# AaltoML/t-SVGP

Measured on AMD Instinct MI355X. Metric: natgrad E-steps/sec, higher is better.
Workload: dtype f64; 1 GPU; gaussian_regression_N1e6_M1024_D8_P1 (north_star target; the metric's N, M); N=1000000, M=1024, D=8, P=1, likelihood=gaussian, rows_per_gpu=1000000, parallelism=N-sharded x1, 1 all-reduce/step, projection=auto

## Files before the change

include/tsvgp_hip.h:

```cpp
#ifndef TSVGP_HIP_H
#define TSVGP_HIP_H

#include <stdint.h>

#ifdef __cplusplus
extern "C" {
#endif

#define TSVGP_OK 0
#define TSVGP_EINVAL 1
#define TSVGP_ELAUNCH 2

#define TSVGP_TILE 128
#define TSVGP_MAX_BATCH 32

#define TSVGP_LIK_NONE 0
#define TSVGP_LIK_GAUSSIAN 1
#define TSVGP_LIK_BERNOULLI 2
#define TSVGP_LIK_HETERO 3
#define TSVGP_LIK_SOFTMAX 4
#define TSVGP_LIK_STUDENT_T 5
#define TSVGP_LIK_POISSON 6
#define TSVGP_LIK_MULTICLASS 7
#define TSVGP_LIK_GAMMA 8
// ... 67 lines not shown
                      int32_t *nonpos_partial, int64_t N, int64_t Np, int Mp, int P, int mode, void *stream);

int tsvgp_lik_map_f64(const double *mean, const double *var, const double *Y, int lik, double lik_param, double *g0, double *g1,
                      double *ve_partial, int32_t *nonpos_partial, int64_t N, int64_t Np, int P, void *stream);
int tsvgp_lik_map_f32(const float *mean, const float *var, const float *Y, int lik, double lik_param, float *g0, float *g1,
                      double *ve_partial, int32_t *nonpos_partial, int64_t N, int64_t Np, int P, void *stream);

int tsvgp_lik_map_hetero_f64(const double *mean, const double *var, const double *Y, int flags, double *g0, double *g1,
                             double *ve_partial, int32_t *nonpos_partial, int64_t N, int64_t Np, void *stream);
int tsvgp_lik_map_hetero_f32(const float *mean, const float *var, const float *Y, int flags, float *g0, float *g1,
                             double *ve_partial, int32_t *nonpos_partial, int64_t N, int64_t Np, void *stream);

int tsvgp_lik_map_robustmax_f64(const double *mean, const double *var, const double *Y, int flags, int C, double epsilon,
                                double *g0, double *g1, double *ve_partial, int32_t *nonpos_partial, int64_t N, int64_t Np,
                                void *stream);
int tsvgp_lik_map_robustmax_f32(const float *mean, const float *var, const float *Y, int flags, int C, double epsilon, float *g0,
                                float *g1, double *ve_partial, int32_t *nonpos_partial, int64_t N, int64_t Np, void *stream);

int tsvgp_lik_map_scalar_f64(const double *mean, const double *var, const double *Y, int64_t in_stride, int lik, double param0,
                             double param1, double *g0, double *g1, int64_t out_stride, double *ve_partial, double *dparam_partial,
                             int32_t *nonpos_partial, int64_t N, int64_t Np, void *stream);
int tsvgp_lik_map_scalar_f32(const float *mean, const float *var, const float *Y, int64_t in_stride, int lik, double param0,
                             double param1, float *g0, float *g1, int64_t out_stride, double *ve_partial, double *dparam_partial,
                             int32_t *nonpos_partial, int64_t N, int64_t Np, void *stream);

#define TSVGP_ORDINAL_MAX_EDGES 255
int tsvgp_lik_map_ordinal_f64(const double *mean, const double *var, const double *Y, int64_t in_stride, int flags,
                              const double *edges, int n_edges, double sigma, double *g0, double *g1, int64_t out_stride,
                              double *ve_partial, double *dparam_partial, int32_t *nonpos_partial, int64_t N, int64_t Np,
                              void *stream);
int tsvgp_lik_map_ordinal_f32(const float *mean, const float *var, const float *Y, int64_t in_stride, int flags,
                              const double *edges, int n_edges, double sigma, float *g0, float *g1, int64_t out_stride,
                              double *ve_partial, double *dparam_partial, int32_t *nonpos_partial, int64_t N, int64_t Np,
                              void *stream);

int tsvgp_lmc_mix_f64(const double *mean_g, const double *var_g, const double *W, double *Fmu, double *Fvar,
                      int32_t *nonpos_partial, int64_t N, int64_t Np, int L, int P, void *stream);
int tsvgp_lmc_mix_f32(const float *mean_g, const float *var_g, const double *W, float *Fmu, float *Fvar, int32_t *nonpos_partial,
                      int64_t N, int64_t Np, int L, int P, void *stream);
int tsvgp_lmc_unmix_f64(const double *g0_f, const double *g1_f, const double *W, int flags, double *g0_g, double *g1_g,
                        const double *mean_g, const double *var_g, double *dW_partial, int64_t N, int64_t Np, int L, int P,
                        void *stream);
int tsvgp_lmc_unmix_f32(const float *g0_f, const float *g1_f, const double *W, int flags, float *g0_g, float *g1_g,
                        const float *mean_g, const float *var_g, double *dW_partial, int64_t N, int64_t Np, int L, int P,
                        void *stream);

int tsvgp_diag_site_step_f64(const double *mean, const double *var, const double *Y, int lik, double lik_param, double lr,
                             double *lambda_1, double *lambda_2, double *ve_partial, int32_t *nonpos_partial, int64_t N, int64_t Np,
                             int P, void *stream);
int tsvgp_diag_site_step_f32(const float *mean, const float *var, const float *Y, int lik, double lik_param, double lr,
                             double *lambda_1, double *lambda_2, float *lambda_1_f32, float *lambda_2_f32, double *ve_partial,
                             int32_t *nonpos_partial, int64_t N, int64_t Np, int P, void *stream);

#define TSVGP_MC_MAX_SAMPLES (1 << 28)
int tsvgp_mc_normals_f64(double *out, int64_t seed, int64_t draw, int64_t row_offset, int64_t S, int64_t N, int C, void *stream);
int tsvgp_mc_normals_f32(float *out, int64_t seed, int64_t draw, int64_t row_offset, int64_t S, int64_t N, int C, void *stream);

int tsvgp_lik_map_softmax_f64(const double *mean, const double *var, const double *Y, int flags, int C, int S,
                              const int64_t *rng_state, int64_t row_offset, const double *epsilon, double *g0, double *g1,
                              double *ve_partial, int32_t *nonpos_partial, int64_t N, int64_t Np, void *stream);
int tsvgp_lik_map_softmax_f32(const float *mean, const float *var, const float *Y, int flags, int C, int S,
                              const int64_t *rng_state, int64_t row_offset, const float *epsilon, float *g0, float *g1,
                              double *ve_partial, int32_t *nonpos_partial, int64_t N, int64_t Np, void *stream);

int tsvgp_moments_batched_f64(const double *A, int64_t strideA, const double *Tm, const double *gamma, const double *Y,
                              const double *kdiag_host, int lik, double lik_param, double *mean, double *var, double *g0,
                              double *g1, double *ve_partial, int32_t *nonpos_partial, int64_t N, int64_t Np, int Mp,
                              int P, int mode, void *stream);
int tsvgp_moments_batched_f32(const float *A, int64_t strideA, const float *Tm, const float *gamma, const float *Y,
                              const double *kdiag_host, int lik, double lik_param, float *mean, float *var, float *g0,
                              float *g1, double *ve_partial, int32_t *nonpos_partial, int64_t N, int64_t Np, int Mp,
                              int P, int mode, void *stream);

int64_t tsvgp_site_accum_work_bytes_f64(int Mp, int P, int nsplit);
int64_t tsvgp_site_accum_work_bytes_f32(int Mp, int P, int nsplit);
int tsvgp_site_accum_f64(const double *B, const double *g0, const double *g1, double *acc2, double *acc1, void *work,
                         int64_t Np, int Mp, int P, int nsplit, void *stream);
int tsvgp_site_accum_f32(const float *B, const float *g0, const float *g1, double *acc2, double *acc1, void *work,
                         int64_t Np, int Mp, int P, int nsplit, void *stream);
int tsvgp_site_accum_batched_f64(const double *B, int64_t strideB, const double *g0, const double *g1, double *acc2,
                                 double *acc1, void *work, int64_t Np, int Mp, int P, int nsplit, void *stream);
int tsvgp_site_accum_batched_f32(const float *B, int64_t strideB, const float *g0, const float *g1, double *acc2,
                                 double *acc1, void *work, int64_t Np, int Mp, int P, int nsplit, void *stream);

#define TSVGP_POTRF_SUBST 1
#define TSVGP_POTRF_DIAG_V1 4
#define TSVGP_POTRF_FUSE 16
int tsvgp_potrf_f64(double *A, int M, int lda, int batch, int64_t stride, int32_t *info, double *work, int flags,
                    void *stream);

#define TSVGP_POTRF_RHS_UPPER 2
int tsvgp_potrf_solve_f64(double *A, int M, int lda, int batch, int64_t stride, int32_t *info, double *work, int rhs_rows,
                          int flags, void *stream);
int tsvgp_flip_transpose_f64(const double *src, int lds, int64_t sstride, double *dst, int ldd, int64_t dstride, int M, int batch,
                             void *stream);

#define TSVGP_VGP_NO_ROWS 1
int tsvgp_vgp_system_f64(int kind, const double *X, const double *inv_ls, double variance, double jitter, const double *lambda_1,
                         const double *lambda_2, double *S, int64_t N, int64_t Np, int D, int64_t lds, int flags, void *stream);
int tsvgp_vgp_rows_f64(const double *C, int64_t ldc, const double *z, const double *Y, double *lambda_1, double *lambda_2,
                       double kdiag, int lik, double lik_param, double beta, double *mean, double *var, double *ve_partial,
                       double *eqt_partial, int32_t *nonpos_partial, int64_t N, int64_t Np, int K, void *stream);

int64_t tsvgp_vgp_kernel_grad_parts(int64_t Np, int D);
int tsvgp_vgp_kernel_grad_f64(int kind, const double *X, const double *inv_ls, double variance, const double *W, int64_t ldw,
                              const double *a, const double *c, int64_t N, int64_t Np, int D, double *part, void *stream);

int tsvgp_potrf_inv_f64(double *A, int M, int lda, int batch, int64_t stride, int32_t *info, double *work, double *X,
                        double *Xt, double *T, int flags, void *stream);

int tsvgp_tri_copy_f64(const double *src, int lds, int64_t sstride, double *dst, int ldd, int64_t dstride, int M, int batch,
                       double scale, int flip, void *stream);
int tsvgp_tri_copy_shift_f64(const double *src, int lds, int64_t sstride, double *dst, int ldd, int64_t dstride, int M, int batch,
                             double scale, double diag_add, int flip, void *stream);

int tsvgp_site_target_f64(const double *G1, const double *LLt, double *target, double *G1s, int M, int P, double c_ll,
                          double c_g, double jitter, const double *rows, double num_data, void *stream);

int tsvgp_site_update_f64(const double *G1, const double *G0, const double *LLt, const double *meanZ, const double *l1_old,
                          double *target, double *l1_new, double *work, int M, int P, double lr, double jitter, const double *rows,
                          double num_data, void *stream);

int tsvgp_site_beta_f64(const double *D, const double *v, const double *l1, double *work, double *beta, int M, int P,
                        void *stream);

int tsvgp_gemv_f64(const double *A, int64_t strideA, const double *v, double *y, int M, int P, void *stream);

int tsvgp_step_status_f64(const int32_t *info_a, int na, const int32_t *info_b, int nb, const double *nonpos, double *flags,
                          void *stream);

int tsvgp_sym_pack_f64(const double *A, int lda, int64_t stride, int M, int P, double *packed, void *stream);
int tsvgp_sym_unpack_f64(const double *packed, double *A, int lda, int64_t stride, int M, int P, void *stream);

int tsvgp_kernel_grad_rows(void);
int tsvgp_kernel_grad_dpad(int D);
int tsvgp_kernel_grad_f64(int kind, const double *X, const double *Z, const double *inv_ls, double variance,
                          const double *U, int64_t ldu, const double *g0, const double *g1, int gstride,
                          const double *beta, int bstride, int64_t N, int M, int D, double *zpart, double *lpart,
                          double *vpart, void *stream);
int tsvgp_kernel_grad_f32(int kind, const float *X, const float *Z, const float *inv_ls, float variance, const float *U,
                          int64_t ldu, const float *g0, const float *g1, int gstride, const float *beta, int bstride,
                          int64_t N, int M, int D, double *zpart, double *lpart, double *vpart, void *stream);

int64_t tsvgp_greedy_select_work_bytes(int64_t N, int M);
int tsvgp_greedy_select_f64(int kind, const double *X, const double *inv_ls, double variance, double floor, double *C, int64_t ldc,
                            double *d, int64_t *indices, double *pivots, int32_t *count, void *work, int64_t N, int M, int D,
                            void *stream);

#define TSVGP_PATHWISE_MAX_S 16
int tsvgp_pathwise_f64(int kind, const double *X, const double *Z, const double *inv_ls, double variance, const double *Omega,
                       const double *W, const double *V, double *out, int64_t N, int M, int L, int D, int S, int64_t ldo,
                       void *stream);

int tsvgp_pathwise_vjp_f64(int kind, const double *X, const double *Z, const double *inv_ls, double variance, const double *Omega,
                           const double *W, const double *V, const double *C, int64_t ldc, double *dX, int64_t N, int M, int L,
                           int D, int S, void *stream);

int tsvgp_moments_vjp_rows(int D);
int tsvgp_moments_vjp_stage_f64(int D);
int tsvgp_moments_vjp_stage_f32(int D);
int tsvgp_moments_vjp_f64(int kind, const double *X, const double *Z, const double *inv_ls, double variance, const double *U,
                          int64_t ldu, const double *cm, const double *cv, int cstride, const double *beta, int bstride, int64_t N,
                          int M, int D, double *dX, int accumulate, void *stream);
int tsvgp_moments_vjp_f32(int kind, const float *X, const float *Z, const float *inv_ls, float variance, const float *U, int64_t ldu,
                          const float *cm, const float *cv, int cstride, const float *beta, int bstride, int64_t N, int M, int D,
                          double *dX, int accumulate, void *stream);
// ... 23 lines not shown
```

t-svgp_amd/_backend.py:

```python
from __future__ import annotations

import ctypes
import os
import subprocess
from ctypes import c_char_p, c_double, c_float, c_int, c_int64, c_void_p

_HERE = os.path.dirname(os.path.abspath(__file__))
_ROOT = os.path.dirname(_HERE)
CSRC = os.path.join(_HERE, "csrc")
LIB_PATH = os.path.join(CSRC, "libtsvgp_hip.so")
HEADER_PATH = os.path.join(_ROOT, "include", "tsvgp_hip.h")
SOURCES = [os.path.join(CSRC, "tsvgp_kernels.hip"), os.path.join(CSRC, "tsvgp_chol.hip"), os.path.join(CSRC, "tsvgp_kmeans.hip")]
HEADERS = [HEADER_PATH, os.path.join(CSRC, "tsvgp_chol.h")]
SOURCE_FLAGS = {"tsvgp_chol.hip": ["-mllvm", "-amdgpu-mfma-vgpr-form=1"]}

TILE = 128
MAX_BATCH = 32
LIK_NONE, LIK_GAUSSIAN, LIK_BERNOULLI = 0, 1, 2
LIK_HETERO = 3
LIK_SOFTMAX = 4
LIK_MULTICLASS = 7
COUPLED_LIKS = (LIK_HETERO, LIK_SOFTMAX, LIK_MULTICLASS)
LIK_STUDENT_T, LIK_POISSON = 5, 6
LIK_GAMMA = 8
# ... 64 lines not shown
    "tsvgp_version": (c_char_p, []),
    "tsvgp_abi_version": (c_int, []),
    "tsvgp_site_accum_slots_f64": (c_int, []),
    "tsvgp_site_accum_slots_f32": (c_int, []),
    "tsvgp_se_fill_f64": (c_int, [c_void_p, c_void_p, c_void_p, c_double, c_void_p, c_int64, c_int, c_int, c_int64, c_void_p]),
    "tsvgp_se_fill_f32": (c_int, [c_void_p, c_void_p, c_void_p, c_float, c_void_p, c_int64, c_int, c_int, c_int64, c_void_p]),
    "tsvgp_kernel_fill_f64": (c_int, [c_int, c_void_p, c_void_p, c_void_p, c_double, c_void_p, c_int64, c_int, c_int, c_int64, c_void_p]),
    "tsvgp_kernel_fill_f32": (c_int, [c_int, c_void_p, c_void_p, c_void_p, c_float, c_void_p, c_int64, c_int, c_int, c_int64, c_void_p]),
    "tsvgp_kernel_fill_batched_f64": (c_int, [c_int, c_void_p, c_void_p, c_void_p, c_void_p, c_void_p, c_int64, c_int64, c_int, c_int,
                                              c_int64, c_int, c_void_p]),
    "tsvgp_kernel_fill_batched_f32": (c_int, [c_int, c_void_p, c_void_p, c_void_p, c_void_p, c_void_p, c_int64, c_int64, c_int, c_int,
                                              c_int64, c_int, c_void_p]),
    "tsvgp_gram_to_kernel_f64": (c_int, [c_int, c_void_p, c_void_p, c_void_p, c_double, c_int64, c_int, c_int64, c_void_p]),
    "tsvgp_gram_to_kernel_f32": (c_int, [c_int, c_void_p, c_void_p, c_void_p, c_float, c_int64, c_int, c_int64, c_void_p]),
    "tsvgp_cov_f64": (c_int, [c_int, c_void_p, c_void_p, c_void_p, c_double, c_double, c_void_p, c_int64, c_int64, c_int, c_int, c_int64,
                              c_int, c_void_p]),
    "tsvgp_cov_f32": (c_int, [c_int, c_void_p, c_void_p, c_void_p, c_float, c_float, c_void_p, c_int64, c_int64, c_int, c_int, c_int64,
                              c_int, c_void_p]),
    "tsvgp_gram_to_gradw_parts": (c_int64, [c_int64, c_int]),
    "tsvgp_gram_to_gradw_f64": (c_int, [c_int, c_void_p, c_void_p, c_void_p, c_double, c_void_p, c_int64, c_void_p, c_void_p, c_int,
                                        c_void_p, c_int, c_int64, c_int, c_int64, c_void_p, c_void_p]),
    "tsvgp_gram_to_gradw_f32": (c_int, [c_int, c_void_p, c_void_p, c_void_p, c_float, c_void_p, c_int64, c_void_p, c_void_p, c_int,
                                        c_void_p, c_int, c_int64, c_int, c_int64, c_void_p, c_void_p]),
    "tsvgp_kernel_grad_rows": (c_int, []),
    "tsvgp_kernel_grad_dpad": (c_int, [c_int]),
    "tsvgp_kernel_grad_f64": (c_int, [c_int, c_void_p, c_void_p, c_void_p, c_double, c_void_p, c_int64, c_void_p, c_void_p, c_int,
                                      c_void_p, c_int, c_int64, c_int, c_int, c_void_p, c_void_p, c_void_p, c_void_p]),
    "tsvgp_kernel_grad_f32": (c_int, [c_int, c_void_p, c_void_p, c_void_p, c_float, c_void_p, c_int64, c_void_p, c_void_p, c_int,
                                      c_void_p, c_int, c_int64, c_int, c_int, c_void_p, c_void_p, c_void_p, c_void_p]),
    "tsvgp_trmm_f64": (c_int, [c_void_p, c_void_p, c_void_p, c_int64, c_int, c_int, c_void_p]),
    "tsvgp_trmm_f32": (c_int, [c_void_p, c_void_p, c_void_p, c_int64, c_int, c_int, c_void_p]),
    "tsvgp_trmm_batched_f64": (c_int, [c_void_p, c_int64, c_void_p, c_int64, c_void_p, c_int64, c_int64, c_int, c_int, c_int, c_void_p]),
    "tsvgp_trmm_batched_f32": (c_int, [c_void_p, c_int64, c_void_p, c_int64, c_void_p, c_int64, c_int64, c_int, c_int, c_int, c_void_p]),
    "tsvgp_moments_batched_f64": (c_int, [c_void_p, c_int64, c_void_p, c_void_p, c_void_p, c_void_p, c_int, c_double, c_void_p, c_void_p,
                                          c_void_p, c_void_p, c_void_p, c_void_p, c_int64, c_int64, c_int, c_int, c_int, c_void_p]),
    "tsvgp_moments_batched_f32": (c_int, [c_void_p, c_int64, c_void_p, c_void_p, c_void_p, c_void_p, c_int, c_double, c_void_p, c_void_p,
                                          c_void_p, c_void_p, c_void_p, c_void_p, c_int64, c_int64, c_int, c_int, c_int, c_void_p]),
    "tsvgp_site_accum_batched_f64": (c_int, [c_void_p, c_int64, c_void_p, c_void_p, c_void_p, c_void_p, c_void_p, c_int64, c_int, c_int, c_int, c_void_p]),
    "tsvgp_site_accum_batched_f32": (c_int, [c_void_p, c_int64, c_void_p, c_void_p, c_void_p, c_void_p, c_void_p, c_int64, c_int, c_int, c_int, c_void_p]),
    "tsvgp_moments_f64": (c_int, [c_void_p, c_void_p, c_void_p, c_void_p, c_double, c_int, c_double, c_void_p, c_void_p,
                                  c_void_p, c_void_p, c_void_p, c_void_p, c_int64, c_int64, c_int, c_int, c_int, c_void_p]),
    "tsvgp_moments_f32": (c_int, [c_void_p, c_void_p, c_void_p, c_void_p, c_double, c_int, c_double, c_void_p, c_void_p,
                                  c_void_p, c_void_p, c_void_p, c_void_p, c_int64, c_int64, c_int, c_int, c_int, c_void_p]),
    "tsvgp_lik_map_f64": (c_int, [c_void_p, c_void_p, c_void_p, c_int, c_double, c_void_p, c_void_p, c_void_p, c_void_p, c_int64, c_int64,
                                  c_int, c_void_p]),
    "tsvgp_lik_map_f32": (c_int, [c_void_p, c_void_p, c_void_p, c_int, c_double, c_void_p, c_void_p, c_void_p, c_void_p, c_int64, c_int64,
                                  c_int, c_void_p]),
    "tsvgp_lik_map_hetero_f64": (c_int, [c_void_p, c_void_p, c_void_p, c_int, c_void_p, c_void_p, c_void_p, c_void_p, c_int64, c_int64,
                                         c_void_p]),
    "tsvgp_lik_map_hetero_f32": (c_int, [c_void_p, c_void_p, c_void_p, c_int, c_void_p, c_void_p, c_void_p, c_void_p, c_int64, c_int64,
                                         c_void_p]),
    "tsvgp_lik_map_scalar_f64": (c_int, [c_void_p, c_void_p, c_void_p, c_int64, c_int, c_double, c_double, c_void_p, c_void_p, c_int64,
                                         c_void_p, c_void_p, c_void_p, c_int64, c_int64, c_void_p]),
    "tsvgp_lik_map_scalar_f32": (c_int, [c_void_p, c_void_p, c_void_p, c_int64, c_int, c_double, c_double, c_void_p, c_void_p, c_int64,
                                         c_void_p, c_void_p, c_void_p, c_int64, c_int64, c_void_p]),
    "tsvgp_lik_map_ordinal_f64": (c_int, [c_void_p, c_void_p, c_void_p, c_int64, c_int, c_void_p, c_int, c_double, c_void_p, c_void_p,
                                          c_int64, c_void_p, c_void_p, c_void_p, c_int64, c_int64, c_void_p]),
    "tsvgp_lik_map_ordinal_f32": (c_int, [c_void_p, c_void_p, c_void_p, c_int64, c_int, c_void_p, c_int, c_double, c_void_p, c_void_p,
                                          c_int64, c_void_p, c_void_p, c_void_p, c_int64, c_int64, c_void_p]),
    "tsvgp_lmc_mix_f64": (c_int, [c_void_p, c_void_p, c_void_p, c_void_p, c_void_p, c_void_p, c_int64, c_int64, c_int, c_int, c_void_p]),
    "tsvgp_lmc_mix_f32": (c_int, [c_void_p, c_void_p, c_void_p, c_void_p, c_void_p, c_void_p, c_int64, c_int64, c_int, c_int, c_void_p]),
    "tsvgp_lmc_unmix_f64": (c_int, [c_void_p, c_void_p, c_void_p, c_int, c_void_p, c_void_p, c_void_p, c_void_p, c_void_p, c_int64,
                                    c_int64, c_int, c_int, c_void_p]),
    "tsvgp_lmc_unmix_f32": (c_int, [c_void_p, c_void_p, c_void_p, c_int, c_void_p, c_void_p, c_void_p, c_void_p, c_void_p, c_int64,
                                    c_int64, c_int, c_int, c_void_p]),
    "tsvgp_diag_site_step_f64": (c_int, [c_void_p, c_void_p, c_void_p, c_int, c_double, c_double, c_void_p, c_void_p, c_void_p,
                                         c_void_p, c_int64, c_int64, c_int, c_void_p]),
    "tsvgp_diag_site_step_f32": (c_int, [c_void_p, c_void_p, c_void_p, c_int, c_double, c_double, c_void_p, c_void_p, c_void_p,
                                         c_void_p, c_void_p, c_void_p, c_int64, c_int64, c_int, c_void_p]),
    "tsvgp_lik_map_softmax_f64": (c_int, [c_void_p, c_void_p, c_void_p, c_int, c_int, c_int, c_void_p, c_int64, c_void_p, c_void_p,
                                          c_void_p, c_void_p, c_void_p, c_int64, c_int64, c_void_p]),
    "tsvgp_lik_map_softmax_f32": (c_int, [c_void_p, c_void_p, c_void_p, c_int, c_int, c_int, c_void_p, c_int64, c_void_p, c_void_p,
                                          c_void_p, c_void_p, c_void_p, c_int64, c_int64, c_void_p]),
    "tsvgp_lik_map_robustmax_f64": (c_int, [c_void_p, c_void_p, c_void_p, c_int, c_int, c_double, c_void_p, c_void_p, c_void_p,
                                            c_void_p, c_int64, c_int64, c_void_p]),
    "tsvgp_lik_map_robustmax_f32": (c_int, [c_void_p, c_void_p, c_void_p, c_int, c_int, c_double, c_void_p, c_void_p, c_void_p,
                                            c_void_p, c_int64, c_int64, c_void_p]),
    "tsvgp_mc_normals_f64": (c_int, [c_void_p, c_int64, c_int64, c_int64, c_int64, c_int64, c_int, c_void_p]),
    "tsvgp_mc_normals_f32": (c_int, [c_void_p, c_int64, c_int64, c_int64, c_int64, c_int64, c_int, c_void_p]),
    "tsvgp_site_accum_work_bytes_f64": (c_int64, [c_int, c_int, c_int]),
    "tsvgp_site_accum_work_bytes_f32": (c_int64, [c_int, c_int, c_int]),
    "tsvgp_site_accum_f64": (c_int, [c_void_p, c_void_p, c_void_p, c_void_p, c_void_p, c_void_p, c_int64, c_int, c_int, c_int, c_void_p]),
    "tsvgp_site_accum_f32": (c_int, [c_void_p, c_void_p, c_void_p, c_void_p, c_void_p, c_void_p, c_int64, c_int, c_int, c_int, c_void_p]),
    "tsvgp_potrf_f64": (c_int, [c_void_p, c_int, c_int, c_int, c_int64, c_void_p, c_void_p, c_int, c_void_p]),
    "tsvgp_potrf_solve_f64": (c_int, [c_void_p, c_int, c_int, c_int, c_int64, c_void_p, c_void_p, c_int, c_int, c_void_p]),
    "tsvgp_vgp_system_f64": (c_int, [c_int, c_void_p, c_void_p, c_double, c_double, c_void_p, c_void_p, c_void_p, c_int64, c_int64, c_int,
                                     c_int64, c_int, c_void_p]),
    "tsvgp_vgp_rows_f64": (c_int, [c_void_p, c_int64, c_void_p, c_void_p, c_void_p, c_void_p, c_double, c_int, c_double, c_double,
                                   c_void_p, c_void_p, c_void_p, c_void_p, c_void_p, c_int64, c_int64, c_int, c_void_p]),
    "tsvgp_vgp_kernel_grad_parts": (c_int64, [c_int64, c_int]),
    "tsvgp_vgp_kernel_grad_f64": (c_int, [c_int, c_void_p, c_void_p, c_double, c_void_p, c_int64, c_void_p, c_void_p, c_int64, c_int64,
                                          c_int, c_void_p, c_void_p]),
    "tsvgp_flip_transpose_f64": (c_int, [c_void_p, c_int, c_int64, c_void_p, c_int, c_int64, c_int, c_int, c_void_p]),
    "tsvgp_potrf_inv_f64": (c_int, [c_void_p, c_int, c_int, c_int, c_int64, c_void_p, c_void_p, c_void_p, c_void_p, c_void_p,
                                    c_int, c_void_p]),
    "tsvgp_tri_copy_f64": (c_int, [c_void_p, c_int, c_int64, c_void_p, c_int, c_int64, c_int, c_int, c_double, c_int, c_void_p]),
    "tsvgp_tri_copy_shift_f64": (c_int, [c_void_p, c_int, c_int64, c_void_p, c_int, c_int64, c_int, c_int, c_double, c_double, c_int,
                                         c_void_p]),
    "tsvgp_site_target_f64": (c_int, [c_void_p, c_void_p, c_void_p, c_void_p, c_int, c_int, c_double, c_double, c_double, c_void_p,
                                      c_double, c_void_p]),
    "tsvgp_site_update_f64": (c_int, [c_void_p, c_void_p, c_void_p, c_void_p, c_void_p, c_void_p, c_void_p, c_void_p, c_int, c_int,
                                      c_double, c_double, c_void_p, c_double, c_void_p]),
    "tsvgp_site_beta_f64": (c_int, [c_void_p, c_void_p, c_void_p, c_void_p, c_void_p, c_int, c_int, c_void_p]),
    "tsvgp_gemv_f64": (c_int, [c_void_p, c_int64, c_void_p, c_void_p, c_int, c_int, c_void_p]),
    "tsvgp_step_status_f64": (c_int, [c_void_p, c_int, c_void_p, c_int, c_void_p, c_void_p, c_void_p]),
    "tsvgp_sym_pack_f64": (c_int, [c_void_p, c_int, c_int64, c_int, c_int, c_void_p, c_void_p]),
    "tsvgp_sym_unpack_f64": (c_int, [c_void_p, c_void_p, c_int, c_int64, c_int, c_int, c_void_p]),
    "tsvgp_greedy_select_work_bytes": (c_int64, [c_int64, c_int]),
    "tsvgp_greedy_select_f64": (c_int, [c_int, c_void_p, c_void_p, c_double, c_double, c_void_p, c_int64, c_void_p, c_void_p, c_void_p,
                                        c_void_p, c_void_p, c_int64, c_int, c_int, c_void_p]),
    "tsvgp_pathwise_f64": (c_int, [c_int, c_void_p, c_void_p, c_void_p, c_double, c_void_p, c_void_p, c_void_p, c_void_p, c_int64, c_int,
                                   c_int, c_int, c_int, c_int64, c_void_p]),
    "tsvgp_pathwise_vjp_f64": (c_int, [c_int, c_void_p, c_void_p, c_void_p, c_double, c_void_p, c_void_p, c_void_p, c_void_p, c_int64,
                                       c_void_p, c_int64, c_int, c_int, c_int, c_int, c_void_p]),
    "tsvgp_moments_vjp_rows": (c_int, [c_int]),
    "tsvgp_moments_vjp_stage_f64": (c_int, [c_int]),
    "tsvgp_moments_vjp_stage_f32": (c_int, [c_int]),
    "tsvgp_moments_vjp_f64": (c_int, [c_int, c_void_p, c_void_p, c_void_p, c_double, c_void_p, c_int64, c_void_p, c_void_p, c_int,
                                      c_void_p, c_int, c_int64, c_int, c_int, c_void_p, c_int, c_void_p]),
    "tsvgp_moments_vjp_f32": (c_int, [c_int, c_void_p, c_void_p, c_void_p, c_float, c_void_p, c_int64, c_void_p, c_void_p, c_int,
                                      c_void_p, c_int, c_int64, c_int, c_int, c_void_p, c_int, c_void_p]),
    "tsvgp_kmeans_assign_rows": (c_int, [c_int]),
    "tsvgp_kmeans_assign_chunk": (c_int, []),
    "tsvgp_kmeans_assign_parts": (c_int64, [c_int64, c_int]),
    "tsvgp_kmeans_assign_f64": (c_int, [c_void_p, c_void_p, c_void_p, c_void_p, c_void_p, c_void_p, c_int64, c_int, c_int, c_void_p]),
    "tsvgp_kmeans_update_f64": (c_int, [c_void_p, c_void_p, c_void_p, c_void_p, c_void_p, c_int64, c_int, c_int, c_void_p]),
    "tsvgp_kmeanspp_rows": (c_int, [c_int]),
    "tsvgp_kmeanspp_work": (c_int64, [c_int64, c_int, c_int]),
    "tsvgp_kmeanspp_f64": (c_int, [c_void_p, c_void_p, c_int64, c_int, c_int, c_void_p, c_void_p, c_void_p, c_void_p, c_void_p, c_void_p,
                                   c_void_p, c_int64, c_int, c_void_p]),
    "tsvgp_selftest_mfma_f64": (c_int, [c_void_p, c_void_p, c_void_p, c_void_p]),
    "tsvgp_selftest_mfma_f32": (c_int, [c_void_p, c_void_p, c_void_p, c_void_p]),
}


def exported_symbols():
    return sorted(_PROTOTYPES)


def lib():
    global _lib
    if _lib is not None:
        return _lib
    path = os.environ.get("TSVGP_HIP_LIB", LIB_PATH)
    if not os.path.exists(path):
        raise HipExtensionError(
            f"HIP extension not built: {path} is missing. Run `python -c 'import __graft_entry__ as g; g.build()'` "
            "(hipcc --offload-arch=gfx950). There is no CPU fallback for the E-step."
        )
    try:
        handle = ctypes.CDLL(path)
    except OSError as e:
        raise HipExtensionError(f"cannot load {path}: {e}") from e
    try:
        handle.tsvgp_abi_version.restype = c_int
        abi = int(handle.tsvgp_abi_version())
    except AttributeError:
        abi = None
    if abi != ABI_VERSION:
        raise HipExtensionError(f"{path}: ABI version {abi}, these bindings are written for {ABI_VERSION} "
                                "(include/tsvgp_hip.h: TSVGP_ABI_VERSION); rebuild the library from this tree")
    missing = [name for name in _PROTOTYPES if not hasattr(handle, name)]
    if missing:
        raise HipExtensionError(f"{path} does not export {missing}: not a build of this tree (include/tsvgp_hip.h); rebuild it")
    for name, (restype, argtypes) in _PROTOTYPES.items():
        fn = getattr(handle, name)
# ... 25 lines not shown
```

t-svgp_amd/csrc/tsvgp_kernels.hip:

```cpp

#include <hip/hip_runtime.h>

#include <atomic>
#include <cmath>
#include <type_traits>
#include <stdint.h>
#include <stdlib.h>

#include "tsvgp_hip.h"
#include "tsvgp_chol.h"

namespace {

constexpr int TILE = TSVGP_TILE;
constexpr int KC = 16;
#define TSVGP_CHOL_PRIO 3
constexpr int LDS_KS = 144;
constexpr int NTHREADS = 256;
constexpr int MODE_STORE = 0;
constexpr int MODE_MOMENTS = 1;

typedef double v4d __attribute__((ext_vector_type(4)));
typedef float v4f __attribute__((ext_vector_type(4)));
typedef double v2d __attribute__((ext_vector_type(2)));
// ... 2178 lines not shown

    if (c_lo < c_hi) {
        load_chunk(c_lo);
        store_chunk(0);
    }
    __syncthreads();
    auto step = [&](const int64_t c, auto buf_tag) {
        constexpr int BUF = decltype(buf_tag)::value;
        const bool has_next = (c + 1 < c_hi);
        if (has_next) load_chunk(c + 1);
        mma_chunk_krow<T, DIAG, W>(acc, lds[BUF][0], lds[BUF][1], w, lane);
        if (DIAG && t < TILE) {
            const T* bcol = &lds[BUF][1][t];
#pragma unroll
            for (int k = 0; k < KC; ++k) acc1 += g0s[BUF][k] * bcol[k * LDS_KS];
        }
        if (has_next) store_chunk(BUF ^ 1);
        __syncthreads();
    };
    {
        int64_t c = c_lo;
        for (; c + 1 < c_hi; c += 2) {
            step(c, std::integral_constant<int, 0>{});
            step(c + 1, std::integral_constant<int, 1>{});
        }
        if (c < c_hi) step(c, std::integral_constant<int, 0>{});
    }

    T* out = a.part2 + ((size_t)p * per_p + slab) * (TILE * TILE) + (lane & 15);
#pragma unroll
    for (int s = 0; s < 2; ++s)
#pragma unroll
        for (int r = 0; r < 4; ++r) {
            T* orow = out + (row_block(w, s) * 16 + Mfma<T>::row(lane, r)) * TILE;
#pragma unroll
            for (int n = 0; n < 8; ++n)
                if (!DIAG || n <= (s == 0 ? W : 7 - W)) orow[n * 16] = acc[s][n][r];
        }
    if (DIAG && t < TILE) a.part1[((size_t)p * a.ns_diag + sidx) * Mp + it * TILE + t] = acc1;
}

template <typename T>
__global__ __launch_bounds__(NTHREADS, 2) void syrk_kernel(SyrkArgs<T> a) {
    __shared__ __attribute__((aligned(16))) T lds[2][2][KC * LDS_KS];
    __shared__ T g0s[2][KC];

    const int w = __builtin_amdgcn_readfirstlane(threadIdx.x >> 6);
    const int nt = a.nt, n_off = nt * (nt - 1) / 2;
    const int per_p = n_off * a.ns_off + nt * a.ns_diag;
    int lin = xcd_remap(blockIdx.x, gridDim.x);
    const int p = lin / per_p;
    lin -= p * per_p;
    int it, jt, sidx;
    if (lin < n_off * a.ns_off) {
        sidx = lin / n_off;
        const int idx = lin - sidx * n_off;
        it = 1;
        while (it * (it + 1) / 2 <= idx) ++it;
        jt = idx - it * (it - 1) / 2;
    } else {
        lin -= n_off * a.ns_off;
        sidx = lin / nt;
        it = jt = lin - sidx * nt;
    }
    const int tri = it * (it + 1) / 2 + jt;
    const int slab = (tri - it) * a.ns_off + it * a.ns_diag + sidx;

    if (it != jt) {
        syrk_body<T, false, 0>(a, lds, g0s, p, it, jt, sidx, slab, per_p, w);
    } else if (w == 0) {
        syrk_body<T, true, 0>(a, lds, g0s, p, it, jt, sidx, slab, per_p, w);
    } else if (w == 1) {
        syrk_body<T, true, 1>(a, lds, g0s, p, it, jt, sidx, slab, per_p, w);
    } else if (w == 2) {
        syrk_body<T, true, 2>(a, lds, g0s, p, it, jt, sidx, slab, per_p, w);
    } else {
        syrk_body<T, true, 3>(a, lds, g0s, p, it, jt, sidx, slab, per_p, w);
    }
}

constexpr int S1_IMG = KC * LDS_KS;
constexpr int S1_BUF = 2 * S1_IMG;

template <bool DIAG, int W>
__device__ __forceinline__ void syrk1_body(const SyrkArgs<double>& a, double* lds, double* wl, int p, int it, int jt, int sidx, int slab,
                                           int per_p, int w) {
    typedef v4d acc_t;
    const int t = threadIdx.x, lane = t & 63;
    const int Mp = a.Mp, P = a.P;
    const int64_t total_chunks = a.Np / KC;
    const int64_t per = DIAG ? a.chunks_diag : a.chunks_off;
    int64_t c_lo = (int64_t)sidx * per;
    int64_t c_hi = c_lo + per;
    if (c_lo > total_chunks) c_lo = total_chunks;
    if (c_hi > total_chunks) c_hi = total_chunks;
    const int nch = (int)(c_hi - c_lo);

    constexpr int MB = DIAG ? 8 - W : 8;
    constexpr int NM = DIAG ? 9 : 16;
    constexpr int NR = 2 + MB;

    const int lr = lane & 15, lk = lane >> 4;
    const int offa0 = lk * LDS_KS + w * 16 + lr;
    const int offa1 = lk * LDS_KS + (7 - w) * 16 + lr;
    const int offb = lk * LDS_KS + lr + (DIAG ? 0 : S1_IMG);
    const int off1 = lk * LDS_KS + w * 32 + lr * 2;

    auto uni64 = [](const void* ptr) TSVGP_AI {
        const uint64_t v = (uint64_t)(uintptr_t)ptr;
        return ((uint64_t)(unsigned)__builtin_amdgcn_readfirstlane((int)(v >> 32)) << 32) |
               (uint64_t)(unsigned)__builtin_amdgcn_readfirstlane((int)(unsigned)v);
    };
    const unsigned lds_u = (unsigned)__builtin_amdgcn_readfirstlane((int)((unsigned)(uintptr_t)(lds_void_t*)lds + (unsigned)(w * LDS_KS * 8)));
    const unsigned dvo = (unsigned)(lane * 16);
    const double* Bp = a.B + (size_t)p * a.strideB + (int64_t)w * Mp;
    const uint64_t bi_u = uni64(Bp + it * TILE), bj_u = uni64(Bp + jt * TILE);
    const uint64_t row4 = (uint64_t)4 * Mp * sizeof(double), chunkb = (uint64_t)KC * Mp * sizeof(double);
    uint64_t ci_u = 0, cj_u = 0;
    auto dma_setup = [&](const int64_t c) TSVGP_AI {
        ci_u = bi_u + (uint64_t)c * chunkb;
        cj_u = bj_u + (uint64_t)c * chunkb;
    };
    auto dma_piece = [&](auto i_tag, const int buf) TSVGP_AI {
        constexpr int I = decltype(i_tag)::value, rq = I >> 1;
        const unsigned la = lds_u + (unsigned)((buf * S1_BUF + (I & 1) * S1_IMG + rq * 4 * LDS_KS) * sizeof(double));
        const uint64_t g = ((I & 1) ? cj_u : ci_u) + rq * row4;
        const unsigned vo_ = dvo;
        asm volatile("s_mov_b32 m0, %0\n\ts_nop 0\n\tglobal_load_lds_dwordx4 %1, %2" ::"s"(la), "v"(vo_), "s"(g) : "memory");
    };
    constexpr int NDMA = DIAG ? 4 : 8;

    const unsigned wl_u = (unsigned)__builtin_amdgcn_readfirstlane((int)(unsigned)(uintptr_t)(lds_void_t*)wl);
    const uint64_t wmask = (P >= 8) ? ~0ull : ((1ull << (8 * P)) - 1);
    const uint64_t g1_u = uni64(a.g1), g0_u = uni64(a.g0);
    const uint64_t wchunk = (uint64_t)KC * P * sizeof(double);
    auto dma_weights = [&](const int64_t c, const int buf) TSVGP_AI {
        if (w == 0 || (DIAG && w == 1)) {
            const unsigned la = wl_u + (unsigned)((buf * 256 + (w == 1 ? 128 : 0)) * sizeof(double));
            const uint64_t g = (w == 1 ? g0_u : g1_u) + (uint64_t)c * wchunk;
            const unsigned vo_ = dvo;
            uint64_t saved;
            asm volatile("s_mov_b64 %0, exec\n\ts_mov_b64 exec, %1\n\ts_mov_b32 m0, %2\n\ts_nop 0\n\t"
                         "global_load_lds_dwordx4 %3, %4\n\ts_mov_b64 exec, %0"
                         : "=&s"(saved)
                         : "s"(wmask), "s"(la), "v"(vo_), "s"(g)
                         : "memory");
        }
    };
    double w1r[4], w0r[4];
    const int woff = lk * P + p;
    auto read_weight = [&](auto i_tag, const int buf) TSVGP_AI {
        constexpr int I = decltype(i_tag)::value;
        if constexpr (I < 4) w1r[I] = wl[buf * 256 + woff + I * 4 * P];
        else w0r[I - 4] = wl[buf * 256 + 128 + woff + (I - 4) * 4 * P];
    };
    constexpr int NW = DIAG ? 8 : 4;

    acc_t acc[2][8];
#pragma unroll
    for (int s = 0; s < 2; ++s)
#pragma unroll
        for (int n = 0; n < 8; ++n) acc[s][n] = acc_t{0, 0, 0, 0};
    double acc1v[2] = {0.0, 0.0};
    Frag1<double> fx, fy;

    auto rd1 = [&](Frag1<double>& f, auto e_tag, auto ks_tag, const int boff) TSVGP_AI {
        constexpr int E = decltype(e_tag)::value, KS_ = decltype(ks_tag)::value;
        if constexpr (E == 0) f.v[0] = lds[offa0 + boff + KS_ * 4 * LDS_KS];
        else if constexpr (E == 1) f.v[1] = lds[offa1 + boff + KS_ * 4 * LDS_KS];
        else f.v[E] = lds[offb + boff + KS_ * 4 * LDS_KS + (E - 2) * 16];
    };
    auto rds = [&](Frag1<double>& f, auto slot_tag, auto ks_tag, const int boff) TSVGP_AI {
        constexpr int S = decltype(slot_tag)::value;
        if constexpr (S < MB) rd1(f, TSVGP_IC(2 + S), ks_tag, boff);
        else rd1(f, TSVGP_IC(S - MB), ks_tag, boff);
    };
    auto keep_set = [&](const Frag1<double>& f) TSVGP_AI {
        cfor<0, NR>([&](auto e) TSVGP_AI {
            const double x = f.v[decltype(e)::value];
            asm volatile("" ::"v"(x));
        });
    };
    auto mf = [&](const Frag1<double>& f, auto i_tag) TSVGP_AI {
        constexpr int I = decltype(i_tag)::value;
        if constexpr (!DIAG) {
            constexpr int n = I >> 1, sblk = I & 1;
            acc[sblk][n] = __builtin_amdgcn_mfma_f64_16x16x4f64(f.v[sblk], f.v[2 + n], acc[sblk][n], 0, 0, 0);
        } else {
            constexpr int n = (I < 2 * (W + 1)) ? (I >> 1) : (I - (W + 1));
            constexpr int sblk = (I < 2 * (W + 1)) ? (I & 1) : 1;
            acc[sblk][n] = __builtin_amdgcn_mfma_f64_16x16x4f64(f.v[sblk], f.v[2 + n], acc[sblk][n], 0, 0, 0);
        }
    };
    v2d f1[4];
    auto chunk = [&](auto buf_tag, auto next_tag, const int64_t c_fetch) TSVGP_AI {
        constexpr int BUF = decltype(buf_tag)::value;
        constexpr bool NEXT = decltype(next_tag)::value;
        constexpr int B0 = BUF * S1_BUF, B1 = (BUF ^ 1) * S1_BUF;
        if constexpr (NEXT) {
            dma_setup(c_fetch);
            TSVGP_SB();
        }
        cfor<0, 3>([&](auto ks) TSVGP_AI {
            constexpr int KS_ = decltype(ks)::value;
            Frag1<double>& cur = (KS_ & 1) ? fy : fx;
            Frag1<double>& nxt = (KS_ & 1) ? fx : fy;
            constexpr int S = NR + ((DIAG && KS_ == 0) ? 4 : 0);
            cfor<0, (NM > S ? NM : S)>([&](auto i) TSVGP_AI {
                constexpr int I = decltype(i)::value;
                if constexpr (I < NM) mf(cur, i);
                if constexpr (I < NR) rds(nxt, i, TSVGP_IC(KS_ + 1), B0);
                else if constexpr (DIAG && KS_ == 0 && I < NR + 4)
                    f1[I - NR] = *reinterpret_cast<const v2d*>(lds + off1 + B0 + (I - NR) * 4 * LDS_KS);
                TSVGP_SB();
            });
            nxt.v[0] *= w1r[KS_ + 1];
            nxt.v[1] *= w1r[KS_ + 1];
            if constexpr (DIAG && KS_ == 1) {
#pragma unroll
                for (int q = 0; q < 4; ++q) {
                    acc1v[0] += w0r[q] * f1[q][0];
                    acc1v[1] += w0r[q] * f1[q][1];
                }
            }
            TSVGP_SB();
            keep_set(cur);
        });
        asm volatile("s_waitcnt vmcnt(0) lgkmcnt(0)" ::: "memory");
        __builtin_amdgcn_s_barrier();
        asm volatile("" ::: "memory");
        TSVGP_SB();
        if constexpr (NEXT) {
            constexpr int S3 = NDMA + NW + NR;
            cfor<0, (NM > S3 ? NM : S3)>([&](auto i) TSVGP_AI {
                constexpr int I = decltype(i)::value;
                if constexpr (I < NM) mf(fy, i);
                if constexpr (I < NDMA) dma_piece(TSVGP_IC(DIAG ? 2 * I : I), BUF);
                else if constexpr (I < NDMA + NW) read_weight(TSVGP_IC(I - NDMA), BUF ^ 1);
                else if constexpr (I < S3) rds(fx, TSVGP_IC(I - NDMA - NW), TSVGP_IC(0), B1);
                TSVGP_SB();
            });
            dma_weights(c_fetch, BUF);
            fx.v[0] *= w1r[0];
            fx.v[1] *= w1r[0];
            TSVGP_SB();
        } else {
            cfor<0, NM>([&](auto i) TSVGP_AI { mf(fy, i); });
        }
        keep_set(fy);
    };

    if (nch > 0) {
        dma_setup(c_lo);
        cfor<0, NDMA>([&](auto i) TSVGP_AI { dma_piece(TSVGP_IC(DIAG ? 2 * decltype(i)::value : decltype(i)::value), 0); });
        dma_weights(c_lo, 0);
        const int64_t c1 = (nch > 1) ? c_lo + 1 : c_lo;
        dma_setup(c1);
        cfor<0, NDMA>([&](auto i) TSVGP_AI { dma_piece(TSVGP_IC(DIAG ? 2 * decltype(i)::value : decltype(i)::value), 1); });
        dma_weights(c1, 1);
        asm volatile("s_waitcnt vmcnt(0) lgkmcnt(0)" ::: "memory");
        __builtin_amdgcn_s_barrier();
        asm volatile("" ::: "memory");
        cfor<0, NW>([&](auto i) TSVGP_AI { read_weight(i, 0); });
        cfor<0, NR>([&](auto i) TSVGP_AI { rds(fx, i, TSVGP_IC(0), 0); });
        fx.v[0] *= w1r[0];
        fx.v[1] *= w1r[0];
        int i = 0;
        const int64_t c_last = c_hi - 1;
        auto fetch_of = [&](int idx) TSVGP_AI { const int64_t c = c_lo + idx + 2; return c < c_last ? c : c_last; };
        if (nch >= 3) {
            chunk(TSVGP_IC(0), TSVGP_BC(true), fetch_of(0));
            chunk(TSVGP_IC(1), TSVGP_BC(true), fetch_of(1));
            for (i = 2; i + 2 < nch; i += 2) {
                chunk(TSVGP_IC(0), TSVGP_BC(true), fetch_of(i));
                chunk(TSVGP_IC(1), TSVGP_BC(true), fetch_of(i + 1));
            }
        }
        if (nch - i == 2) {
            chunk(TSVGP_IC(0), TSVGP_BC(true), fetch_of(i));
            chunk(TSVGP_IC(1), TSVGP_BC(false), 0);
        } else {
            chunk(TSVGP_IC(0), TSVGP_BC(false), 0);
        }
        asm volatile("s_waitcnt vmcnt(0)" ::: "memory");
    }

    double* out = a.part2 + ((size_t)p * per_p + slab) * (TILE * TILE) + (lane & 15);
#pragma unroll
    for (int s = 0; s < 2; ++s)
#pragma unroll
        for (int r = 0; r < 4; ++r) {
            double* orow = out + (row_block(w, s) * 16 + Mfma<double>::row(lane, r)) * TILE;
#pragma unroll
            for (int n = 0; n < 8; ++n)
                if (!DIAG || n <= (s == 0 ? W : 7 - W)) orow[n * 16] = acc[s][n][r];
        }
    if constexpr (DIAG) {
#pragma unroll
        for (int q = 0; q < 2; ++q) {
            acc1v[q] += __shfl_xor(acc1v[q], 16);
            acc1v[q] += __shfl_xor(acc1v[q], 32);
        }
        if (lk == 0) {
            double* o1 = a.part1 + ((size_t)p * a.ns_diag + sidx) * Mp + it * TILE + w * 32 + lr * 2;
            o1[0] = acc1v[0];
            o1[1] = acc1v[1];
        }
    }
}

__global__ __launch_bounds__(NTHREADS, 1) void syrk1_kernel(SyrkArgs<double> a) {
    __shared__ __attribute__((aligned(1024))) double lds[2 * S1_BUF];
    __shared__ __attribute__((aligned(1024))) double wl[2 * 256];

    const int w = __builtin_amdgcn_readfirstlane(threadIdx.x >> 6);
    const int nt = a.nt, n_off = nt * (nt - 1) / 2;
    const int per_p = n_off * a.ns_off + nt * a.ns_diag;
    int lin = xcd_remap(blockIdx.x, gridDim.x);
    const int p = lin / per_p;
    lin -= p * per_p;
    int it, jt, sidx;
    if (lin < n_off * a.ns_off) {
        sidx = lin / n_off;
        const int idx = lin - sidx * n_off;
        it = 1;
        while (it * (it + 1) / 2 <= idx) ++it;
        jt = idx - it * (it - 1) / 2;
    } else {
        lin -= n_off * a.ns_off;
        sidx = lin / nt;
        it = jt = lin - sidx * nt;
    }
    const int tri = it * (it + 1) / 2 + jt;
    const int slab = (tri - it) * a.ns_off + it * a.ns_diag + sidx;
    if (it != jt) {
        syrk1_body<false, 0>(a, lds, wl, p, it, jt, sidx, slab, per_p, w);
    } else if (w == 0) {
        syrk1_body<true, 0>(a, lds, wl, p, it, jt, sidx, slab, per_p, w);
    } else if (w == 1) {
        syrk1_body<true, 1>(a, lds, wl, p, it, jt, sidx, slab, per_p, w);
    } else if (w == 2) {
        syrk1_body<true, 2>(a, lds, wl, p, it, jt, sidx, slab, per_p, w);
    } else {
        syrk1_body<true, 3>(a, lds, wl, p, it, jt, sidx, slab, per_p, w);
    }
}

constexpr int S1F_KC = 32;
constexpr int S1F_IMG = S1F_KC * TILE;
constexpr int S1F_BUF = 2 * S1F_IMG;
constexpr int S1F_WL = 512;

template <bool DIAG, int W>
__device__ __forceinline__ void syrk1f_body(const SyrkArgs<float>& a, float* lds, float* wl, int p, int it, int jt, int sidx,
                                            int slab, int per_p, int w) {
    typedef v4f acc_t;
    typedef Frag1<float> Frag;
    const int t = threadIdx.x, lane = t & 63;
    const int Mp = a.Mp, P = a.P;
    const int64_t total_chunks = a.Np / S1F_KC;
    const int64_t per = DIAG ? a.chunks_diag : a.chunks_off;
    int64_t c_lo = (int64_t)sidx * per;
    int64_t c_hi = c_lo + per;
    if (c_lo > total_chunks) c_lo = total_chunks;
    if (c_hi > total_chunks) c_hi = total_chunks;
    const int nch = (int)(c_hi - c_lo);

    constexpr int MB = DIAG ? 8 - W : 8;
    constexpr int NM = DIAG ? 9 : 16;
    constexpr int NR = 2 + MB;
    constexpr int NKS = S1F_KC / 4;

    const int lr = lane & 15, lk = lane >> 4, odd = lk & 1;
    const int offa0 = lk * TILE + 16 * (w ^ odd) + lr;
    const int offa1 = lk * TILE + 16 * ((7 - w) ^ odd) + lr;
    const int offb_e = lk * TILE + lr + 16 * odd + (DIAG ? 0 : S1F_IMG);
    const int offb_o = lk * TILE + lr - 16 * odd + (DIAG ? 0 : S1F_IMG);
    const int off1 = lk * TILE + 4 * ((8 * w + (lr >> 1)) ^ (4 * odd)) + 2 * (lr & 1);

    auto uni64 = [](const void* ptr) TSVGP_AI {
        const uint64_t v = (uint64_t)(uintptr_t)ptr;
        return ((uint64_t)(unsigned)__builtin_amdgcn_readfirstlane((int)(v >> 32)) << 32) |
               (uint64_t)(unsigned)__builtin_amdgcn_readfirstlane((int)(unsigned)v);
    };
    const unsigned lds_u = (unsigned)__builtin_amdgcn_readfirstlane((int)((unsigned)(uintptr_t)(lds_void_t*)lds + (unsigned)(w * 1024)));
    const unsigned dvo = (unsigned)((lane >> 5) * Mp * (int)sizeof(float) + (((lane & 31) ^ ((lane >> 5) << 2)) << 4));
    const unsigned dvw = (unsigned)(lane * 16);
    const float* Bp = a.B + (size_t)p * a.strideB + (int64_t)(2 * w) * Mp;
    const uint64_t bi_u = uni64(Bp + it * TILE), bj_u = uni64(Bp + jt * TILE);
    const uint64_t row8 = (uint64_t)8 * Mp * sizeof(float), chunkb = (uint64_t)S1F_KC * Mp * sizeof(float);
    uint64_t ci_u = 0, cj_u = 0;
    auto dma_setup = [&](const int64_t c) TSVGP_AI {
        ci_u = bi_u + (uint64_t)c * chunkb;
        cj_u = bj_u + (uint64_t)c * chunkb;
    };
    auto dma_piece = [&](auto i_tag, const int buf) TSVGP_AI {
        constexpr int I = decltype(i_tag)::value, rq = I >> 1;
        const unsigned la = lds_u + (unsigned)((buf * S1F_BUF + (I & 1) * S1F_IMG + rq * 1024) * sizeof(float));
        const uint64_t g = ((I & 1) ? cj_u : ci_u) + rq * row8;
        const unsigned vo_ = dvo;
        asm volatile("s_mov_b32 m0, %0\n\ts_nop 0\n\tglobal_load_lds_dwordx4 %1, %2" ::"s"(la), "v"(vo_), "s"(g) : "memory");
    };
    constexpr int NDMA = DIAG ? 4 : 8;

    const unsigned wl_u = (unsigned)__builtin_amdgcn_readfirstlane((int)(unsigned)(uintptr_t)(lds_void_t*)wl);
    const uint64_t wmask = (P >= 8) ? ~0ull : ((1ull << (8 * P)) - 1);
    const uint64_t g1_u = uni64(a.g1), g0_u = uni64(a.g0);
    const uint64_t wchunk = (uint64_t)S1F_KC * P * sizeof(float);
    auto dma_weights = [&](const int64_t c, const int buf) TSVGP_AI {
        if (w == 0 || (DIAG && w == 1)) {
            const unsigned la = wl_u + (unsigned)((buf * S1F_WL + (w == 1 ? 256 : 0)) * sizeof(float));
            const uint64_t g = (w == 1 ? g0_u : g1_u) + (uint64_t)c * wchunk;
            const unsigned vo_ = dvw;
            uint64_t saved;
            asm volatile("s_mov_b64 %0, exec\n\ts_mov_b64 exec, %1\n\ts_mov_b32 m0, %2\n\ts_nop 0\n\t"
                         "global_load_lds_dwordx4 %3, %4\n\ts_mov_b64 exec, %0"
                         : "=&s"(saved)
                         : "s"(wmask), "s"(la), "v"(vo_), "s"(g)
                         : "memory");
        }
    };
    float w1r[NKS], w0r[NKS];
    const int woff = lk * P + p;
    auto read_weight = [&](auto i_tag, const int buf) TSVGP_AI {
        constexpr int I = decltype(i_tag)::value;
        if constexpr (I < NKS) w1r[I] = wl[buf * S1F_WL + woff + I * 4 * P];
        else w0r[I - NKS] = wl[buf * S1F_WL + 256 + woff + (I - NKS) * 4 * P];
    };
    constexpr int NWH = DIAG ? 8 : 4;
    auto read_weight_half = [&](auto j_tag, auto half_tag, const int buf) TSVGP_AI {
        constexpr int J = decltype(j_tag)::value, H = decltype(half_tag)::value;
        if constexpr (J < 4) read_weight(TSVGP_IC(4 * H + J), buf);
        else read_weight(TSVGP_IC(NKS + 4 * H + J - 4), buf);
    };

    acc_t acc[2][8];
#pragma unroll
    for (int s = 0; s < 2; ++s)
#pragma unroll
        for (int n = 0; n < 8; ++n) acc[s][n] = acc_t{0, 0, 0, 0};
    float acc1v[2] = {0.f, 0.f};
    Frag fx, fy;

    auto rd1 = [&](Frag& f, auto e_tag, auto ks_tag, const int boff) TSVGP_AI {
        constexpr int E = decltype(e_tag)::value, KS_ = decltype(ks_tag)::value;
        if constexpr (E == 0) f.v[0] = lds[offa0 + boff + KS_ * 4 * TILE];
        else if constexpr (E == 1) f.v[1] = lds[offa1 + boff + KS_ * 4 * TILE];
        else f.v[E] = lds[(((E - 2) & 1) ? offb_o : offb_e) + boff + KS_ * 4 * TILE + (E - 2) * 16];
    };
    auto rds = [&](Frag& f, auto slot_tag, auto ks_tag, const int boff) TSVGP_AI {
        constexpr int S = decltype(slot_tag)::value;
        if constexpr (S < MB) rd1(f, TSVGP_IC(2 + S), ks_tag, boff);
        else rd1(f, TSVGP_IC(S - MB), ks_tag, boff);
    };
    auto keep_set = [&](const Frag& f) TSVGP_AI {
        cfor<0, NR>([&](auto e) TSVGP_AI {
            const float x = f.v[decltype(e)::value];
            asm volatile("" ::"v"(x));
        });
    };
    auto mf = [&](const Frag& f, auto i_tag) TSVGP_AI {
        constexpr int I = decltype(i_tag)::value;
        if constexpr (!DIAG) {
            constexpr int n = I >> 1, sblk = I & 1;
            acc[sblk][n] = __builtin_amdgcn_mfma_f32_16x16x4f32(f.v[sblk], f.v[2 + n], acc[sblk][n], 0, 0, 0);
        } else {
            constexpr int n = (I < 2 * (W + 1)) ? (I >> 1) : (I - (W + 1));
            constexpr int sblk = (I < 2 * (W + 1)) ? (I & 1) : 1;
            acc[sblk][n] = __builtin_amdgcn_mfma_f32_16x16x4f32(f.v[sblk], f.v[2 + n], acc[sblk][n], 0, 0, 0);
        }
    };
    v2f f1[NKS];
    auto chunk = [&](auto buf_tag, auto next_tag, const int64_t c_fetch) TSVGP_AI {
        constexpr int BUF = decltype(buf_tag)::value;
        constexpr bool NEXT = decltype(next_tag)::value;
        constexpr int B0 = BUF * S1F_BUF, B1 = (BUF ^ 1) * S1F_BUF;
        if constexpr (NEXT) {
            dma_setup(c_fetch);
            TSVGP_SB();
        }
        cfor<0, NKS - 1>([&](auto ks) TSVGP_AI {
            constexpr int KS_ = decltype(ks)::value;
            Frag& cur = (KS_ & 1) ? fy : fx;
            Frag& nxt = (KS_ & 1) ? fx : fy;
            constexpr int XW = KS_ == 0 ? NWH : 0;
            constexpr int XF = (DIAG && KS_ < 4) ? 2 : 0;
            constexpr int S = NR + XW + XF;
            cfor<0, (NM > S ? NM : S)>([&](auto i) TSVGP_AI {
                constexpr int I = decltype(i)::value;
                if constexpr (I < NM) mf(cur, i);
                if constexpr (I < NR) rds(nxt, i, TSVGP_IC(KS_ + 1), B0);
                else if constexpr (I < NR + XW) read_weight_half(TSVGP_IC(I - NR), TSVGP_IC(1), BUF);
                else if constexpr (I < S)
                    f1[2 * KS_ + I - NR - XW] = *reinterpret_cast<const v2f*>(lds + off1 + B0 + (2 * KS_ + I - NR - XW) * 4 * TILE);
                TSVGP_SB();
            });
            nxt.v[0] *= w1r[KS_ + 1];
            nxt.v[1] *= w1r[KS_ + 1];
            if constexpr (DIAG && (KS_ == 4 || KS_ == 5)) {
#pragma unroll
                for (int q = 4 * (KS_ - 4); q < 4 * (KS_ - 4) + 4; ++q) {
                    acc1v[0] += w0r[q] * f1[q][0];
                    acc1v[1] += w0r[q] * f1[q][1];
                }
            }
            TSVGP_SB();
            keep_set(cur);
        });
        asm volatile("s_waitcnt vmcnt(0) lgkmcnt(0)" ::: "memory");
        __builtin_amdgcn_s_barrier();
        asm volatile("" ::: "memory");
        TSVGP_SB();
        if constexpr (NEXT) {
            constexpr int S3 = NDMA + NWH + NR;
            cfor<0, (NM > S3 ? NM : S3)>([&](auto i) TSVGP_AI {
                constexpr int I = decltype(i)::value;
                if constexpr (I < NM) mf(fy, i);
                if constexpr (I < NDMA) dma_piece(TSVGP_IC(DIAG ? 2 * I : I), BUF);
                else if constexpr (I < NDMA + NWH) read_weight_half(TSVGP_IC(I - NDMA), TSVGP_IC(0), BUF ^ 1);
                else if constexpr (I < S3) rds(fx, TSVGP_IC(I - NDMA - NWH), TSVGP_IC(0), B1);
                TSVGP_SB();
            });
            dma_weights(c_fetch, BUF);
            fx.v[0] *= w1r[0];
            fx.v[1] *= w1r[0];
            TSVGP_SB();
        } else {
            cfor<0, NM>([&](auto i) TSVGP_AI { mf(fy, i); });
        }
        keep_set(fy);
    };

    if (nch > 0) {
        dma_setup(c_lo);
        cfor<0, NDMA>([&](auto i) TSVGP_AI { dma_piece(TSVGP_IC(DIAG ? 2 * decltype(i)::value : decltype(i)::value), 0); });
        dma_weights(c_lo, 0);
        const int64_t c1 = (nch > 1) ? c_lo + 1 : c_lo;
        dma_setup(c1);
        cfor<0, NDMA>([&](auto i) TSVGP_AI { dma_piece(TSVGP_IC(DIAG ? 2 * decltype(i)::value : decltype(i)::value), 1); });
        dma_weights(c1, 1);
        asm volatile("s_waitcnt vmcnt(0) lgkmcnt(0)" ::: "memory");
        __builtin_amdgcn_s_barrier();
        asm volatile("" ::: "memory");
        cfor<0, NWH>([&](auto i) TSVGP_AI { read_weight_half(i, TSVGP_IC(0), 0); });
        cfor<0, NR>([&](auto i) TSVGP_AI { rds(fx, i, TSVGP_IC(0), 0); });
        fx.v[0] *= w1r[0];
        fx.v[1] *= w1r[0];
        int i = 0;
        const int64_t c_last = c_hi - 1;
        auto fetch_of = [&](int idx) TSVGP_AI { const int64_t c = c_lo + idx + 2; return c < c_last ? c : c_last; };
        if (nch >= 3) {
            chunk(TSVGP_IC(0), TSVGP_BC(true), fetch_of(0));
            chunk(TSVGP_IC(1), TSVGP_BC(true), fetch_of(1));
            for (i = 2; i + 2 < nch; i += 2) {
                chunk(TSVGP_IC(0), TSVGP_BC(true), fetch_of(i));
                chunk(TSVGP_IC(1), TSVGP_BC(true), fetch_of(i + 1));
            }
        }
        if (nch - i == 2) {
            chunk(TSVGP_IC(0), TSVGP_BC(true), fetch_of(i));
            chunk(TSVGP_IC(1), TSVGP_BC(false), 0);
        } else {
            chunk(TSVGP_IC(0), TSVGP_BC(false), 0);
        }
        asm volatile("s_waitcnt vmcnt(0)" ::: "memory");
    }

    float* out = a.part2 + ((size_t)p * per_p + slab) * (TILE * TILE) + (lane & 15);
#pragma unroll
    for (int s = 0; s < 2; ++s)
#pragma unroll
        for (int r = 0; r < 4; ++r) {
            float* orow = out + (row_block(w, s) * 16 + Mfma<float>::row(lane, r)) * TILE;
#pragma unroll
            for (int n = 0; n < 8; ++n)
                if (!DIAG || n <= (s == 0 ? W : 7 - W)) orow[n * 16] = acc[s][n][r];
        }
    if constexpr (DIAG) {
#pragma unroll
        for (int q = 0; q < 2; ++q) {
            acc1v[q] += __shfl_xor(acc1v[q], 16);
            acc1v[q] += __shfl_xor(acc1v[q], 32);
        }
        if (lk == 0) {
            float* o1 = a.part1 + ((size_t)p * a.ns_diag + sidx) * Mp + it * TILE + w * 32 + lr * 2;
            o1[0] = acc1v[0];
            o1[1] = acc1v[1];
        }
    }
}

#define TSVGP_S1F_WAVES 2
__global__ __launch_bounds__(NTHREADS, 1) __attribute__((amdgpu_waves_per_eu(1, TSVGP_S1F_WAVES))) void syrk1f_kernel(SyrkArgs<float> a) {
    __shared__ __attribute__((aligned(1024))) float lds[2 * S1F_BUF];
    __shared__ __attribute__((aligned(1024))) float wl[2 * S1F_WL];

    const int w = __builtin_amdgcn_readfirstlane(threadIdx.x >> 6);
    const int nt = a.nt, n_off = nt * (nt - 1) / 2;
    const int per_p = n_off * a.ns_off + nt * a.ns_diag;
    int lin = xcd_remap(blockIdx.x, gridDim.x);
    const int p = lin / per_p;
    lin -= p * per_p;
    int it, jt, sidx;
    if (lin < n_off * a.ns_off) {
        sidx = lin / n_off;
        const int idx = lin - sidx * n_off;
        it = 1;
        while (it * (it + 1) / 2 <= idx) ++it;
        jt = idx - it * (it - 1) / 2;
    } else {
        lin -= n_off * a.ns_off;
        sidx = lin / nt;
        it = jt = lin - sidx * nt;
    }
    const int tri = it * (it + 1) / 2 + jt;
    const int slab = (tri - it) * a.ns_off + it * a.ns_diag + sidx;
    if (it != jt) {
        syrk1f_body<false, 0>(a, lds, wl, p, it, jt, sidx, slab, per_p, w);
    } else if (w == 0) {
        syrk1f_body<true, 0>(a, lds, wl, p, it, jt, sidx, slab, per_p, w);
    } else if (w == 1) {
        syrk1f_body<true, 1>(a, lds, wl, p, it, jt, sidx, slab, per_p, w);
    } else if (w == 2) {
        syrk1f_body<true, 2>(a, lds, wl, p, it, jt, sidx, slab, per_p, w);
    } else {
        syrk1f_body<true, 3>(a, lds, wl, p, it, jt, sidx, slab, per_p, w);
    }
}

constexpr int SR_ROWS = 16;
template <typename T>
__global__ __launch_bounds__(NTHREADS) void syrk_reduce_kernel(const T* __restrict__ part2,
                                                               const T* __restrict__ part1,
                                                               double* __restrict__ acc2, double* __restrict__ acc1,
                                                               int Mp, int P, int nt, int ns_off, int ns_diag) {
    __shared__ double img[SR_ROWS][TILE + 1];
    constexpr int SUBS = TILE / SR_ROWS;
    const int p = blockIdx.y;
    const int ntri = nt * (nt + 1) / 2;
    const int per_p = (ntri - nt) * ns_off + nt * ns_diag;
    const int tri = blockIdx.x / SUBS, sub = blockIdx.x % SUBS;
    const int t = threadIdx.x;
    if (tri < ntri) {
        int it = 0;
        while ((it + 1) * (it + 2) / 2 <= tri) ++it;
        const int jt = tri - it * (it + 1) / 2;
        const int ns = (it == jt) ? ns_diag : ns_off;
        const int slab0 = (tri - it) * ns_off + it * ns_diag;
        const size_t base = (size_t)p * Mp * Mp;
        const int jj = t & 127, rbase = t >> 7;
        constexpr int RPT = SR_ROWS * 128 / NTHREADS;
        double acc[RPT];
#pragma unroll
        for (int q = 0; q < RPT; ++q) acc[q] = 0.0;
        const T* src = part2 + ((size_t)p * per_p + slab0) * (TILE * TILE) + (size_t)(sub * SR_ROWS + rbase) * TILE + jj;
        for (int sp = 0; sp < ns; ++sp) {
#pragma unroll
            for (int q = 0; q < RPT; ++q) acc[q] += (double)src[(size_t)sp * (TILE * TILE) + q * (NTHREADS / 128) * TILE];
        }
#pragma unroll
        for (int q = 0; q < RPT; ++q) {
            const int r = rbase + q * (NTHREADS / 128), ii = sub * SR_ROWS + r;
            if (it == jt && jj > ii) continue;
            acc2[base + (size_t)(it * TILE + ii) * Mp + jt * TILE + jj] = acc[q];
            img[r][jj] = acc[q];
        }
        __syncthreads();
        const int c = t >> 1, r0 = (t & 1) * (SR_ROWS / 2);
        double* out = acc2 + base + (size_t)(jt * TILE + c) * Mp + it * TILE + sub * SR_ROWS + r0;
#pragma unroll
        for (int r = 0; r < SR_ROWS / 2; ++r) {
            if (it == jt && c > sub * SR_ROWS + r0 + r) continue;
            out[r] = img[r0 + r][c];
        }
    } else {
        const int idx = (blockIdx.x - ntri * SUBS) * NTHREADS + t;
        if (idx < Mp) {
            double s = 0.0;
            for (int sp = 0; sp < ns_diag; ++sp) s += (double)part1[((size_t)p * ns_diag + sp) * Mp + idx];
            acc1[(size_t)p * Mp + idx] = s;
        }
    }
}

constexpr int CH_NB = 128;
constexpr int CH_SB = 16;
constexpr int CH_WT = 32;
constexpr int CH_LD = CH_NB + 1;
constexpr int CH_THREADS = 512;

__device__ __forceinline__ double rsqrt_nr(double x) {
    const double y = __builtin_amdgcn_rsq(x);
    const double e = fma(-x * y, y, 1.0);
    return fma(y * e, fma(e, 0.375, 0.5), y);
}

__device__ __forceinline__ double readlane_d(double v, int src) {
    const int lo = __builtin_amdgcn_readlane(__double2loint(v), src);
    const int hi = __builtin_amdgcn_readlane(__double2hiint(v), src);
    return __hiloint2double(hi, lo);
}

struct ChRole {
    int sub, below, ident;
};
__device__ __forceinline__ ChRole chol_factor_rows(double* __restrict__ S, double* __restrict__ dinv, double* __restrict__ xs,
                                                   int s0, int lane, int w, int need_inverse, int* fail, int col_base,
                                                   double (&a)[CH_SB]) {
    const int nbelow = CH_NB - s0 - CH_SB;
    const int idx = (64 - CH_SB) * w + lane - CH_SB;
    ChRole role;
    role.sub = lane < CH_SB;
    role.below = !role.sub && idx < nbelow;
    role.ident = (!role.sub && !role.below && need_inverse && idx < nbelow + CH_SB) ? idx - nbelow : -1;
    double* const row = S + (role.sub ? s0 + lane : s0 + CH_SB + idx) * CH_LD + s0;
    if (role.sub || role.below) {
#pragma unroll
        for (int c = 0; c < CH_SB; ++c) a[c] = row[c];
    } else {
#pragma unroll
        for (int c = 0; c < CH_SB; ++c) a[c] = (c == role.ident) ? 1.0 : 0.0;
    }
    int bad = 0;
#pragma unroll
    for (int j0 = 0; j0 < CH_SB; j0 += 4) {
        const double p00 = readlane_d(a[j0], j0), p10 = readlane_d(a[j0], j0 + 1), p20 = readlane_d(a[j0], j0 + 2),
                     p30 = readlane_d(a[j0], j0 + 3);
        const double p11 = readlane_d(a[j0 + 1], j0 + 1), p21 = readlane_d(a[j0 + 1], j0 + 2),
                     p31 = readlane_d(a[j0 + 1], j0 + 3);
        const double p22 = readlane_d(a[j0 + 2], j0 + 2), p32 = readlane_d(a[j0 + 2], j0 + 3);
        const double p33 = readlane_d(a[j0 + 3], j0 + 3);
        const double i0 = rsqrt_nr(p00);
        const double l10 = p10 * i0, l20 = p20 * i0, l30 = p30 * i0;
        const double d1 = p11 - l10 * l10;
        const double i1 = rsqrt_nr(d1);
        const double l21 = (p21 - l20 * l10) * i1, l31 = (p31 - l30 * l10) * i1;
        const double d2 = p22 - l20 * l20 - l21 * l21;
        const double i2 = rsqrt_nr(d2);
        const double l32 = (p32 - l30 * l20 - l31 * l21) * i2;
        const double d3 = p33 - l30 * l30 - l31 * l31 - l32 * l32;
        const double i3 = rsqrt_nr(d3);
// ... 1784 lines not shown
    if (blocks > 0x7fffffff) return TSVGP_EINVAL;
    hipLaunchKernelGGL(mc_normals_kernel<T>, dim3((unsigned)blocks), dim3(256), 0, (hipStream_t)stream, out, seed, draw, row_offset,
                       S, N, C);
    return launch_status();
}

template <typename T>
int moments(const T* A, int64_t strideA, const T* Tm, const T* gamma, const T* Y, const double* kdiag, bool kdiag_uniform,
            int lik, double lik_param, T* mean, T* var, T* g0, T* g1, double* ve_partial, int32_t* nonpos_partial,
            int64_t N, int64_t Np, int Mp, int P, int mode, void* stream) {
    const bool mean_only = (lik & TSVGP_LIK_MEANONLY) != 0;
    if (!A || !gamma || !kdiag || N <= 0 || Np < N || (Np % TILE) || Mp <= 0 || (Mp % TILE) || P <= 0 || strideA < 0)
        return TSVGP_EINVAL;
    if (!kdiag_uniform && P > TSVGP_MAX_BATCH) return TSVGP_EINVAL;
    if (strideA != 0 && strideA < Np * (int64_t)Mp) return TSVGP_EINVAL;
    if (!mean_only && (!Tm || mode < 0 || mode > 2)) return TSVGP_EINVAL;
    if (lik & ~(0xFF | TSVGP_LIK_NOCROP | TSVGP_LIK_MEANONLY)) return TSVGP_EINVAL;
    const int lik_base = lik & 0xFF;
    if (lik_base != TSVGP_LIK_NONE && lik_base != TSVGP_LIK_GAUSSIAN && lik_base != TSVGP_LIK_BERNOULLI) return TSVGP_EINVAL;
    constexpr size_t MEAN_LDS_MAX = 128 * 1024;
    if (mean_only && (lik_base == TSVGP_LIK_BERNOULLI || var || (size_t)Mp * P * sizeof(T) > MEAN_LDS_MAX)) return TSVGP_EINVAL;
    if (mean_only) {
        static DynLdsOptIn optin;
        if (optin.ensure(reinterpret_cast<const void*>(&mean_lik_kernel<T>), MEAN_LDS_MAX) != TSVGP_OK) return TSVGP_ELAUNCH;
    }
    lik &= ~TSVGP_LIK_MEANONLY;
    if (lik_base == TSVGP_LIK_NONE) lik = TSVGP_LIK_NONE;
    if (lik != TSVGP_LIK_NONE && (!Y || !g0 || !g1)) return TSVGP_EINVAL;
    if (lik_base == TSVGP_LIK_GAUSSIAN && !(lik_param > 0.0)) return TSVGP_EINVAL;
    PanelArgs<T> a{};
    a.A = A;
    a.Tm = Tm;
    a.gamma = gamma;
    a.Y = Y;
    a.mean = mean;
    a.var = var;
    a.g0 = g0;
    a.g1 = g1;
    a.ve_partial = ve_partial;
    a.nonpos_partial = nonpos_partial;
    a.kdiag_uniform = kdiag_uniform ? 1 : 0;
    for (int q = 0; q < (kdiag_uniform ? 1 : P); ++q) a.kdiag[q] = kdiag[q];
    a.strideA = strideA;
    a.lik_param = lik_param;
    a.N = N;
    a.Np = Np;
    a.Mp = Mp;
    a.P = P;
    a.mode = mode;
    a.lik = lik;
    const dim3 grid((unsigned)(Np / TILE)), block(NTHREADS);
    if (mean_only)
        hipLaunchKernelGGL((mean_lik_kernel<T>), grid, block, (size_t)Mp * P * sizeof(T), (hipStream_t)stream, a);
    else if (mode == TSVGP_TRI_LOWER && (size_t)Mp * sizeof(T) <= P1_GAMMA_LDS_MAX) {
        static DynLdsOptIn optin1l;
        if (optin1l.ensure(reinterpret_cast<const void*>(&panel1_kernel<T, MODE_MOMENTS, TSVGP_TRI_LOWER>), P1_GAMMA_LDS_MAX) !=
            TSVGP_OK)
            return TSVGP_ELAUNCH;
        hipLaunchKernelGGL((panel1_kernel<T, MODE_MOMENTS, TSVGP_TRI_LOWER>), grid, block, (size_t)Mp * sizeof(T),
                           (hipStream_t)stream, a);
    } else if (mode == TSVGP_TRI_LOWER)
        hipLaunchKernelGGL((panel_kernel<T, MODE_MOMENTS, TSVGP_TRI_LOWER>), grid, block, 0, (hipStream_t)stream, a);
    else if (mode == TSVGP_TRI_UPPER && (size_t)Mp * sizeof(T) <= P1_GAMMA_LDS_MAX) {
        static DynLdsOptIn optin1;
        if (optin1.ensure(reinterpret_cast<const void*>(&panel1_kernel<T>), P1_GAMMA_LDS_MAX) != TSVGP_OK) return TSVGP_ELAUNCH;
        hipLaunchKernelGGL((panel1_kernel<T>), grid, block, (size_t)Mp * sizeof(T), (hipStream_t)stream, a);
    } else if (mode == TSVGP_TRI_UPPER)
        hipLaunchKernelGGL((panel_kernel<T, MODE_MOMENTS, TSVGP_TRI_UPPER>), grid, block, 0, (hipStream_t)stream, a);
    else
        hipLaunchKernelGGL((panel_kernel<T, MODE_MOMENTS, TSVGP_TRI_DENSE>), grid, block, 0, (hipStream_t)stream, a);
    return launch_status();
}

template <typename T>
int64_t site_accum_work_bytes(int Mp, int P, int nsplit) {
    if (Mp <= 0 || (Mp % TILE) || P <= 0 || nsplit <= 0) return -1;
    const int64_t nt = Mp / TILE, n_off = nt * (nt - 1) / 2;
    const int64_t ns_diag = syrk_ns_diag(nsplit, (int)sizeof(T));
    const int64_t per_p = n_off * nsplit + nt * ns_diag;
    return (int64_t)P * (per_p * TILE * TILE + ns_diag * Mp) * (int64_t)sizeof(T);
}

template <typename T>
int site_accum(const T* B, int64_t strideB, const T* g0, const T* g1, double* acc2, double* acc1, void* work, int64_t Np,
               int Mp, int P, int nsplit, void* stream) {
    if (!B || !g0 || !g1 || !acc2 || !acc1 || !work || Np <= 0 || (Np % TILE) || Mp <= 0 || (Mp % TILE) || P <= 0 ||
        nsplit <= 0 || strideB < 0 || (strideB != 0 && strideB < Np * (int64_t)Mp))
        return TSVGP_EINVAL;
    if (((uintptr_t)B | (uintptr_t)g0 | (uintptr_t)g1 | (uintptr_t)work) & 15 || ((strideB * (int64_t)sizeof(T)) & 15))
        return TSVGP_EINVAL;
    const int nt = Mp / TILE, ntri = nt * (nt + 1) / 2, n_off = ntri - nt;
    const int64_t total_chunks = Np / KC;
    SyrkArgs<T> a{};
    a.B = B;
    a.g0 = g0;
    a.g1 = g1;
    a.Np = Np;
    a.strideB = strideB;
    a.Mp = Mp;
    a.P = P;
    a.nt = nt;
    a.ns_off = nsplit;
    a.ns_diag = syrk_ns_diag(nsplit, (int)sizeof(T));
    a.chunks_off = (total_chunks + a.ns_off - 1) / a.ns_off;
    a.chunks_diag = (total_chunks + a.ns_diag - 1) / a.ns_diag;
    const int64_t per_p = (int64_t)n_off * a.ns_off + (int64_t)nt * a.ns_diag;
    a.part2 = reinterpret_cast<T*>(work);
    a.part1 = a.part2 + (size_t)P * per_p * TILE * TILE;
    const int64_t nwg = (int64_t)P * per_p;
    if (nwg > 0x7fffffff) return TSVGP_EINVAL;
    if (sizeof(T) == 8 && P <= 8) {
      if constexpr (sizeof(T) == 8) {
        static DynLdsOptIn optin_s1;
        if (optin_s1.ensure(reinterpret_cast<const void*>(&syrk1_kernel), 0) != TSVGP_OK) return TSVGP_ELAUNCH;
        hipLaunchKernelGGL(syrk1_kernel, dim3((unsigned)nwg), dim3(NTHREADS), 0, (hipStream_t)stream, a);
      }
    } else if (sizeof(T) == 4 && P <= 8) {
      if constexpr (sizeof(T) == 4) {
        const int64_t total32 = Np / S1F_KC;
        a.chunks_off = (total32 + a.ns_off - 1) / a.ns_off;
        a.chunks_diag = (total32 + a.ns_diag - 1) / a.ns_diag;
        static DynLdsOptIn optin_s1f;
        if (optin_s1f.ensure(reinterpret_cast<const void*>(&syrk1f_kernel), 0) != TSVGP_OK) return TSVGP_ELAUNCH;
        hipLaunchKernelGGL(syrk1f_kernel, dim3((unsigned)nwg), dim3(NTHREADS), 0, (hipStream_t)stream, a);
      }
    } else
        hipLaunchKernelGGL(syrk_kernel<T>, dim3((unsigned)nwg), dim3(NTHREADS), 0, (hipStream_t)stream, a);
    if (launch_status() != TSVGP_OK) return TSVGP_ELAUNCH;
    const int extra = (Mp + NTHREADS - 1) / NTHREADS;
    hipLaunchKernelGGL(syrk_reduce_kernel<T>, dim3((unsigned)(ntri * (TILE / SR_ROWS) + extra), (unsigned)P), dim3(NTHREADS), 0,
                       (hipStream_t)stream, a.part2, a.part1, acc2, acc1, Mp, P, nt, a.ns_off, a.ns_diag);
    return launch_status();
}

template <typename T>
int site_accum_slots() {
    int dev = 0, cus = 0, nb = 0;
    if (hipGetDevice(&dev) != hipSuccess) return -1;
    if (hipDeviceGetAttribute(&cus, hipDeviceAttributeMultiprocessorCount, dev) != hipSuccess) return -1;
    if (sizeof(T) == 8) return cus;
    if (hipOccupancyMaxActiveBlocksPerMultiprocessor(&nb, reinterpret_cast<const void*>(&syrk1f_kernel), NTHREADS, 0) != hipSuccess)
        return -1;
    return cus * (nb > 2 ? 2 : nb < 1 ? 1 : nb);
}

int potrf(double* A, int M, int lda, int batch, int64_t stride, int* info, double* work, int flags, void* stream,
          double* X = nullptr, double* Xt = nullptr, double* T = nullptr, int rhs_rows = 0) {
    if (!A || !info || !work || M <= 0 || (M % CH_NB) || lda < M || batch <= 0 ||
        (flags & ~(TSVGP_POTRF_SUBST | TSVGP_POTRF_RHS_UPPER | TSVGP_POTRF_DIAG_V1 | TSVGP_POTRF_FUSE)) || rhs_rows < 0 || (rhs_rows % CH_NB) ||
        (rhs_rows > 0 && stride < (int64_t)(M + rhs_rows) * lda))
        return TSVGP_EINVAL;
    if ((lda % 2) || ((reinterpret_cast<uintptr_t>(A) | reinterpret_cast<uintptr_t>(work)) & 15) ||
        (batch > 1 && ((stride % 2) || stride < (int64_t)(M + rhs_rows) * lda)))
        return TSVGP_EINVAL;
    const bool rhs_upper = (flags & TSVGP_POTRF_RHS_UPPER) != 0;
    const bool inv = X != nullptr, subst = (flags & TSVGP_POTRF_SUBST) != 0, diag_v1 = (flags & TSVGP_POTRF_DIAG_V1) != 0,
               fuse = (flags & TSVGP_POTRF_FUSE) != 0;
    if (inv && (!Xt || !T || ((reinterpret_cast<uintptr_t>(X) | reinterpret_cast<uintptr_t>(Xt) | reinterpret_cast<uintptr_t>(T)) & 15)))
        return TSVGP_EINVAL;
    const int nt = M / CH_NB;
    const size_t smem = (size_t)CH_NB * CH_LD * sizeof(double);
    static DynLdsOptIn optin;
    if (optin.ensure(reinterpret_cast<const void*>(&potrf_diag_kernel<false>), smem) != TSVGP_OK) return TSVGP_ELAUNCH;
    static DynLdsOptIn optin_fused;
    if (optin_fused.ensure(reinterpret_cast<const void*>(&potrf_diag_kernel<true>), smem) != TSVGP_OK) return TSVGP_ELAUNCH;
    hipStream_t st = (hipStream_t)stream;
    const int64_t xstride = (int64_t)M * M;
    if (inv) {
        zero_fill(X, sizeof(double) * xstride * batch, st);
        zero_fill(Xt, sizeof(double) * xstride * batch, st);
    }
    const int wpb = NTHREADS / 64;
    for (int k = 0; k < nt; ++k) {
        const int ext_rows = rhs_upper ? (rhs_rows < (k + 1) * CH_NB ? rhs_rows : (k + 1) * CH_NB) : rhs_rows;
        const int below = nt - k - 1;
        const bool panel2 = !inv && !diag_v1 && !subst;
        const int need_inverse = inv ? 1 : ((below > 0 || ext_rows > 0) && !subst) ? (panel2 ? 2 : 1) : 0;
        const int nstrips = (below * CH_NB + ext_rows) / 16;
        const bool fused = panel2 && fuse && nstrips > 0;
        if (fused) {
            const int per = CH_THREADS / 64;
            hipLaunchKernelGGL(potrf_diag_kernel<true>, dim3(batch, (nstrips + per - 1) / per), dim3(CH_THREADS), smem, st, A, lda, stride,
                               k, work, info, 2, X, Xt, M, xstride, nstrips);
        } else {
            hipLaunchKernelGGL(potrf_diag_kernel<false>, dim3(batch), dim3(CH_THREADS), smem, st, A, lda, stride, k, work, info,
                               need_inverse, X, Xt, M, xstride, 0);
        }
        if (below > 0 || ext_rows > 0) {
            const int nb32 = below * (CH_NB / CH_WT), ext32 = ext_rows / CH_WT;
            const int ntile = nb32 * (nb32 + 1) / 2 + ext32 * nb32;
            if (subst)
                hipLaunchKernelGGL(chol_panel_subst_kernel, dim3((below * CH_NB + ext_rows) / PS_ROWS, batch), dim3(NTHREADS), 0,
                                   st, A, lda, stride, k);
            else if (fused) {
            } else if (panel2) {
                if (tsvgp_chol::launch_panel2(A, lda, stride, k, work, (below * CH_NB + ext_rows) / 16, batch, st) != hipSuccess)
                    return TSVGP_ELAUNCH;
            } else
                hipLaunchKernelGGL(chol_tile_kernel<0>, dim3(nb32 + ext32, batch), dim3(NTHREADS), 0, st, A, lda, stride, k, nt,
                                   work, ext32);
            if (ntile > 0)
                hipLaunchKernelGGL(chol_tile_kernel<1>, dim3((ntile + wpb - 1) / wpb, batch), dim3(NTHREADS), 0, st, A,
                                   lda, stride, k, nt, work, ext32);
        }
    }
    if (inv) {
        for (int n = CH_NB; n < M; n *= 2) {
            const int npair = (M + 2 * n - 1) / (2 * n);
            const int ntile = (n / CH_WT) * (n / CH_WT);
            const dim3 grid(ntile, npair, batch);
            hipLaunchKernelGGL(trtri_level_kernel<0>, grid, dim3(NTHREADS), 0, st, A, lda, stride, X, Xt, T, M, xstride,
                               M, n);
            hipLaunchKernelGGL(trtri_level_kernel<1>, grid, dim3(NTHREADS), 0, st, A, lda, stride, X, Xt, T, M, xstride,
                               M, n);
// ... 828 lines not shown
    return lmc_mix<double>(mean_g, var_g, W, Fmu, Fvar, nonpos_partial, N, Np, L, P, stream);
}
int tsvgp_lmc_mix_f32(const float* mean_g, const float* var_g, const double* W, float* Fmu, float* Fvar, int32_t* nonpos_partial,
                      int64_t N, int64_t Np, int L, int P, void* stream) {
    return lmc_mix<float>(mean_g, var_g, W, Fmu, Fvar, nonpos_partial, N, Np, L, P, stream);
}
int tsvgp_lmc_unmix_f64(const double* g0_f, const double* g1_f, const double* W, int flags, double* g0_g, double* g1_g,
                        const double* mean_g, const double* var_g, double* dW_partial, int64_t N, int64_t Np, int L, int P,
                        void* stream) {
    return lmc_unmix<double>(g0_f, g1_f, W, flags, g0_g, g1_g, mean_g, var_g, dW_partial, N, Np, L, P, stream);
}
int tsvgp_lmc_unmix_f32(const float* g0_f, const float* g1_f, const double* W, int flags, float* g0_g, float* g1_g,
                        const float* mean_g, const float* var_g, double* dW_partial, int64_t N, int64_t Np, int L, int P,
                        void* stream) {
    return lmc_unmix<float>(g0_f, g1_f, W, flags, g0_g, g1_g, mean_g, var_g, dW_partial, N, Np, L, P, stream);
}
int tsvgp_lik_map_scalar_f32(const float* mean, const float* var, const float* Y, int64_t in_stride, int lik, double param0,
                             double param1, float* g0, float* g1, int64_t out_stride, double* ve_partial, double* dparam_partial,
                             int32_t* nonpos_partial, int64_t N, int64_t Np, void* stream) {
    return lik_map_scalar<float>(mean, var, Y, in_stride, lik, param0, param1, g0, g1, out_stride, ve_partial, dparam_partial,
                                 nonpos_partial, N, Np, stream);
}
int tsvgp_lik_map_softmax_f64(const double* mean, const double* var, const double* Y, int flags, int C, int S,
                              const int64_t* rng_state, int64_t row_offset, const double* epsilon, double* g0, double* g1,
                              double* ve_partial, int32_t* nonpos_partial, int64_t N, int64_t Np, void* stream) {
    return lik_map_softmax<double>(mean, var, Y, flags, C, S, rng_state, row_offset, epsilon, g0, g1, ve_partial, nonpos_partial, N,
                                   Np, stream);
}
int tsvgp_lik_map_softmax_f32(const float* mean, const float* var, const float* Y, int flags, int C, int S,
                              const int64_t* rng_state, int64_t row_offset, const float* epsilon, float* g0, float* g1,
                              double* ve_partial, int32_t* nonpos_partial, int64_t N, int64_t Np, void* stream) {
    return lik_map_softmax<float>(mean, var, Y, flags, C, S, rng_state, row_offset, epsilon, g0, g1, ve_partial, nonpos_partial, N,
                                  Np, stream);
}
int tsvgp_lik_map_robustmax_f64(const double* mean, const double* var, const double* Y, int flags, int C, double epsilon, double* g0,
                                double* g1, double* ve_partial, int32_t* nonpos_partial, int64_t N, int64_t Np, void* stream) {
    return lik_map_robustmax<double>(mean, var, Y, flags, C, epsilon, g0, g1, ve_partial, nonpos_partial, N, Np, stream);
}
int tsvgp_lik_map_robustmax_f32(const float* mean, const float* var, const float* Y, int flags, int C, double epsilon, float* g0,
                                float* g1, double* ve_partial, int32_t* nonpos_partial, int64_t N, int64_t Np, void* stream) {
    return lik_map_robustmax<float>(mean, var, Y, flags, C, epsilon, g0, g1, ve_partial, nonpos_partial, N, Np, stream);
}
int tsvgp_mc_normals_f64(double* out, int64_t seed, int64_t draw, int64_t row_offset, int64_t S, int64_t N, int C, void* stream) {
    return mc_normals<double>(out, seed, draw, row_offset, S, N, C, stream);
}
int tsvgp_mc_normals_f32(float* out, int64_t seed, int64_t draw, int64_t row_offset, int64_t S, int64_t N, int C, void* stream) {
    return mc_normals<float>(out, seed, draw, row_offset, S, N, C, stream);
}
int tsvgp_moments_f64(const double* A, const double* Tm, const double* gamma, const double* Y, double kdiag, int lik,
                      double lik_param, double* mean, double* var, double* g0, double* g1, double* ve_partial,
                      int32_t* nonpos_partial, int64_t N, int64_t Np, int Mp, int P, int mode, void* stream) {
    return moments<double>(A, 0, Tm, gamma, Y, &kdiag, true, lik, lik_param, mean, var, g0, g1, ve_partial,
                           nonpos_partial, N, Np, Mp, P, mode, stream);
}
int tsvgp_moments_batched_f64(const double* A, int64_t strideA, const double* Tm, const double* gamma, const double* Y,
                              const double* kdiag_host, int lik, double lik_param, double* mean, double* var, double* g0,
                              double* g1, double* ve_partial, int32_t* nonpos_partial, int64_t N, int64_t Np, int Mp,
                              int P, int mode, void* stream) {
    return moments<double>(A, strideA, Tm, gamma, Y, kdiag_host, false, lik, lik_param, mean, var, g0, g1, ve_partial,
                           nonpos_partial, N, Np, Mp, P, mode, stream);
}
int tsvgp_moments_batched_f32(const float* A, int64_t strideA, const float* Tm, const float* gamma, const float* Y,
                              const double* kdiag_host, int lik, double lik_param, float* mean, float* var, float* g0,
                              float* g1, double* ve_partial, int32_t* nonpos_partial, int64_t N, int64_t Np, int Mp,
                              int P, int mode, void* stream) {
    return moments<float>(A, strideA, Tm, gamma, Y, kdiag_host, false, lik, lik_param, mean, var, g0, g1, ve_partial,
                          nonpos_partial, N, Np, Mp, P, mode, stream);
}
int tsvgp_moments_f32(const float* A, const float* Tm, const float* gamma, const float* Y, double kdiag, int lik,
                      double lik_param, float* mean, float* var, float* g0, float* g1, double* ve_partial,
                      int32_t* nonpos_partial, int64_t N, int64_t Np, int Mp, int P, int mode, void* stream) {
    return moments<float>(A, 0, Tm, gamma, Y, &kdiag, true, lik, lik_param, mean, var, g0, g1, ve_partial,
                          nonpos_partial, N, Np, Mp, P, mode, stream);
}

int64_t tsvgp_site_accum_work_bytes_f64(int Mp, int P, int nsplit) {
    return site_accum_work_bytes<double>(Mp, P, nsplit);
}
int64_t tsvgp_site_accum_work_bytes_f32(int Mp, int P, int nsplit) {
    return site_accum_work_bytes<float>(Mp, P, nsplit);
}
int tsvgp_site_accum_f64(const double* B, const double* g0, const double* g1, double* acc2, double* acc1, void* work,
                         int64_t Np, int Mp, int P, int nsplit, void* stream) {
    return site_accum<double>(B, 0, g0, g1, acc2, acc1, work, Np, Mp, P, nsplit, stream);
}
int tsvgp_site_accum_batched_f64(const double* B, int64_t strideB, const double* g0, const double* g1, double* acc2,
                                 double* acc1, void* work, int64_t Np, int Mp, int P, int nsplit, void* stream) {
    return site_accum<double>(B, strideB, g0, g1, acc2, acc1, work, Np, Mp, P, nsplit, stream);
}
int tsvgp_site_accum_batched_f32(const float* B, int64_t strideB, const float* g0, const float* g1, double* acc2,
                                 double* acc1, void* work, int64_t Np, int Mp, int P, int nsplit, void* stream) {
    return site_accum<float>(B, strideB, g0, g1, acc2, acc1, work, Np, Mp, P, nsplit, stream);
}
int tsvgp_site_accum_f32(const float* B, const float* g0, const float* g1, double* acc2, double* acc1, void* work,
                         int64_t Np, int Mp, int P, int nsplit, void* stream) {
    return site_accum<float>(B, 0, g0, g1, acc2, acc1, work, Np, Mp, P, nsplit, stream);
}

int tsvgp_potrf_f64(double* A, int M, int lda, int batch, int64_t stride, int* info, double* work, int flags,
                    void* stream) {
    return potrf(A, M, lda, batch, stride, info, work, flags, stream);
}
int tsvgp_potrf_solve_f64(double* A, int M, int lda, int batch, int64_t stride, int* info, double* work, int rhs_rows,
                          int flags, void* stream) {
    if (rhs_rows <= 0) return TSVGP_EINVAL;
    return potrf(A, M, lda, batch, stride, info, work, flags, stream, nullptr, nullptr, nullptr, rhs_rows);
}
int tsvgp_vgp_system_f64(int kind, const double* X, const double* inv_ls, double variance, double jitter, const double* lambda_1,
                         const double* lambda_2, double* S, int64_t N, int64_t Np, int D, int64_t lds, int flags, void* stream) {
    return vgp_system(kind, X, inv_ls, variance, jitter, lambda_1, lambda_2, S, N, Np, D, lds, flags, stream);
}
int tsvgp_vgp_rows_f64(const double* C, int64_t ldc, const double* z, const double* Y, double* lambda_1, double* lambda_2,
                       double kdiag, int lik, double lik_param, double beta, double* mean, double* var, double* ve_partial,
                       double* eqt_partial, int32_t* nonpos_partial, int64_t N, int64_t Np, int K, void* stream) {
    return vgp_rows(C, ldc, z, Y, lambda_1, lambda_2, kdiag, lik, lik_param, beta, mean, var, ve_partial, eqt_partial,
                    nonpos_partial, N, Np, K, stream);
}
int64_t tsvgp_vgp_kernel_grad_parts(int64_t Np, int D) {
    if (Np <= 0 || (Np % TILE) || Np / TILE > 32768 || D <= 0 || D > 32) return -1;
    const int64_t nt = Np / TILE;
    return (nt * (nt + 1) / 2 + 1) * (1 + vgp_kgrad_dpad(D));
}
int tsvgp_vgp_kernel_grad_f64(int kind, const double* X, const double* inv_ls, double variance, const double* W, int64_t ldw,
                              const double* a, const double* c, int64_t N, int64_t Np, int D, double* part, void* stream) {
    return vgp_kernel_grad(kind, X, inv_ls, variance, W, ldw, a, c, N, Np, D, part, stream);
}
int tsvgp_flip_transpose_f64(const double* src, int lds, int64_t sstride, double* dst, int ldd, int64_t dstride, int M, int batch,
                             void* stream) {
    if (!src || !dst || M <= 0 || lds < M || ldd < M || batch <= 0 || batch > 65535) return TSVGP_EINVAL;
    const unsigned nb = (unsigned)((M + 31) / 32);
    hipLaunchKernelGGL(flip_transpose_kernel, dim3(nb, nb, (unsigned)batch), dim3(NTHREADS), 0, (hipStream_t)stream, src, lds,
                       sstride, dst, ldd, dstride, M);
    return launch_status();
}
int tsvgp_potrf_inv_f64(double* A, int M, int lda, int batch, int64_t stride, int* info, double* work, double* X,
                        double* Xt, double* T, int flags, void* stream) {
    if (!X || !Xt || !T) return TSVGP_EINVAL;
    return potrf(A, M, lda, batch, stride, info, work, flags, stream, X, Xt, T);
}

int tsvgp_tri_copy_shift_f64(const double* src, int lds, int64_t sstride, double* dst, int ldd, int64_t dstride, int M, int batch,
                             double scale, double diag_add, int flip, void* stream) {
    if (!src || !dst || M <= 0 || lds < M || ldd < M || batch <= 0 || batch > 65535 || M > 65535 || flip < 0 || flip > 3)
        return TSVGP_EINVAL;
    hipLaunchKernelGGL(tri_copy_kernel, dim3((M + NTHREADS - 1) / NTHREADS, M, batch), dim3(NTHREADS), 0, (hipStream_t)stream,
                       src, lds, sstride, dst, ldd, dstride, M, scale, flip, diag_add);
    return launch_status();
}
int tsvgp_tri_copy_f64(const double* src, int lds, int64_t sstride, double* dst, int ldd, int64_t dstride, int M, int batch,
                       double scale, int flip, void* stream) {
    if (flip > 2) return TSVGP_EINVAL;
    return tsvgp_tri_copy_shift_f64(src, lds, sstride, dst, ldd, dstride, M, batch, scale, 0.0, flip, stream);
}

int tsvgp_site_target_f64(const double* G1, const double* LLt, double* target, double* G1s, int M, int P, double c_ll,
                          double c_g, double jitter, const double* rows, double num_data, void* stream) {
    if (!G1 || !LLt || !target || !G1s || M <= 0 || P <= 0 || P > 65535 || (num_data > 0.0 && !rows)) return TSVGP_EINVAL;
    const unsigned nb = (unsigned)((M + 31) / 32);
    hipLaunchKernelGGL(site_target_kernel, dim3(nb, nb, (unsigned)P), dim3(NTHREADS), 0, (hipStream_t)stream, G1, LLt, target,
                       G1s, M, c_ll, c_g, jitter, rows, num_data);
    return launch_status();
}
int tsvgp_site_update_f64(const double* G1, const double* G0, const double* LLt, const double* meanZ, const double* l1_old,
                          double* target, double* l1_new, double* work, int M, int P, double lr, double jitter,
                          const double* rows, double num_data, void* stream) {
    if (!G1 || !G0 || !LLt || !meanZ || !l1_old || !target || !l1_new || !work || M <= 0 || P <= 0 || P > 65535 ||
        (num_data > 0.0 && !rows))
        return TSVGP_EINVAL;
    const unsigned nb = (unsigned)((M + 31) / 32);
    hipLaunchKernelGGL(site_update_kernel, dim3(nb, nb, (unsigned)P), dim3(NTHREADS), 0, (hipStream_t)stream, G1, LLt, meanZ,
                       target, work, M, P, lr, jitter, rows, num_data);
    hipLaunchKernelGGL(site_update_finish_kernel, dim3((unsigned)((M + NTHREADS - 1) / NTHREADS), (unsigned)P), dim3(NTHREADS), 0,
                       (hipStream_t)stream, work, G0, l1_old, l1_new, M, P, lr, rows, num_data);
    return launch_status();
}
int tsvgp_site_beta_f64(const double* D, const double* v, const double* l1, double* work, double* beta, int M, int P,
                        void* stream) {
    if (!D || !v || !l1 || !work || !beta || M <= 0 || P <= 0 || P > 65535) return TSVGP_EINVAL;
    const int wpb = NTHREADS / 64, nrg = (M + 63) / 64;
// ... 93 lines not shown
```

t-svgp_amd/estep.py:

```python
from __future__ import annotations

import contextlib
import ctypes
import os
from dataclasses import dataclass
from typing import Optional

import torch

from . import _backend as B
from .distributed import world_size
from .kernels import LinearCoregionalization, SeparateIndependent
from .side_branch import SideBranch, SideStream

MAX_INPUT_DIM = 32
MAX_INPUT_DIM_GRAD = 16


@dataclass
class EStepStats:

    n_rows: int
    ve_sum: torch.Tensor
    nonpos: torch.Tensor
    acc2: Optional[torch.Tensor] = None
    acc1: Optional[torch.Tensor] = None
    mean: Optional[torch.Tensor] = None
    var: Optional[torch.Tensor] = None
    g0: Optional[torch.Tensor] = None
    g1: Optional[torch.Tensor] = None
    tile: Optional[torch.Tensor] = None
    dparam: Optional[torch.Tensor] = None
    fmu: Optional[torch.Tensor] = None
    fvar: Optional[torch.Tensor] = None
    g0_f: Optional[torch.Tensor] = None
    g1_f: Optional[torch.Tensor] = None
    dW: Optional[torch.Tensor] = None


@dataclass
class LikMapResult:

    g0: torch.Tensor
    g1: torch.Tensor
    ve_partial: torch.Tensor
    nonpos_partial: torch.Tensor
    dparam: Optional[torch.Tensor] = None
    fmu: Optional[torch.Tensor] = None
    fvar: Optional[torch.Tensor] = None
    g0_f: Optional[torch.Tensor] = None
    g1_f: Optional[torch.Tensor] = None
    dW: Optional[torch.Tensor] = None


def _ptr(t: Optional[torch.Tensor]):
    return None if t is None else t.data_ptr()


def per_latent(t, p):
    if t is None:
        return None
    if isinstance(t, (list, tuple)):
        return t[p]
    return t[p] if t.dim() == 3 else t


def site_sum_chunk_rows(f64: bool, P: int) -> int:
    return 32 if (not f64 and P <= 8) else 16


def site_sum_slices(Mp: int, P: int, Np, slots: int, f64: bool, oversubscribe=None) -> int:
    nt = Mp // B.TILE
    n_off = nt * (nt - 1) // 2
    num = 20 if f64 else 22
    ns_diag = lambda ns: max(1, (num * ns + 31) // 32)
    if Np is None or oversubscribe is not None:
        ns = 1
        while P * (n_off * (ns + 1) + nt * ns_diag(ns + 1)) <= slots:
            ns += 1
        return ns * (oversubscribe if oversubscribe is not None else 8)
    chunks = max(1, Np // site_sum_chunk_rows(f64, P))
    overhead = 14.0
    best, best_t = 1, None
    for ns in range(1, max(1, min(chunks // 32, 1024)) + 1):
        nd = ns_diag(ns)
        rounds = -(-(P * (n_off * ns + nt * nd)) // slots)
        per = max(-(-chunks // ns) if n_off else 0, -(-chunks // nd) * num / 32.0)
        t = rounds * (per + overhead) * (1.02 if rounds == 1 else 1.0)
        if best_t is None or t < best_t * (1.0 - 1e-9):
            best, best_t = ns, t
    return best


class EStepEngine:

    def __init__(self, compute_dtype=torch.float64, device=None):
        self.lib = B.lib()
        if not torch.cuda.is_available():
            raise B.HipExtensionError("no ROCm device visible: the t-SVGP E-step has no CPU fallback")
        self.device = torch.device(device) if device is not None else torch.device("cuda", torch.cuda.current_device())
        if self.device.type != "cuda":
            raise B.HipExtensionError(f"EStepEngine needs a ROCm device, got {self.device}")
        self.dtype = compute_dtype
        self.sfx = B.suffix(compute_dtype)
        self._buf = {}
        self._slots = None
        self.nsplit_override = None
        self.syrk_oversubscribe = None
        self._b_tag = None
        self._side = SideStream(self.device)
        self.last_batched = False
        self.last_trmm_batch = 1
        self.profile = None
        self.profile_only = None
        self.potrf_flags = B.POTRF_DIAG_V1 if os.environ.get("TSVGP_POTRF_DIAG_V1") == "1" else 0

    def _stream(self):
        return torch.cuda.current_stream(self.device).cuda_stream

    def _fn(self, name, dtype=None):
        return getattr(self.lib, f"{name}_{B.suffix(dtype) if dtype is not None else self.sfx}")

    def _get(self, key, shape, dtype):
        t = self._buf.get(key)
        if t is None or tuple(t.shape) != tuple(shape) or t.dtype != dtype:
            t = torch.empty(shape, dtype=dtype, device=self.device)
            self._buf[key] = t
        return t

    def _launch(self, name, status_fn):
        if self.profile is None or (self.profile_only is not None and name not in self.profile_only):
            B.check(status_fn(), name)
            return
        e0, e1 = self._event(), self._event()
        e0.record(torch.cuda.current_stream(self.device))
        B.check(status_fn(), name)
        e1.record(torch.cuda.current_stream(self.device))
        self.profile.setdefault(name, []).append((e0, e1))

    def _event(self):
        pool = self.__dict__.setdefault("_event_pool", [])
        return pool.pop() if pool else torch.cuda.Event(enable_timing=True)

    def reserve_events(self, n: int):
        pool = self.__dict__.setdefault("_event_pool", [])
        while len(pool) < n:
            pool.append(torch.cuda.Event(enable_timing=True))

    def profile_summary(self):
        torch.cuda.synchronize(self.device)
        out = {}
        pool = self.__dict__.setdefault("_event_pool", [])
        for name, evs in (self.profile or {}).items():
            series = [a.elapsed_time(b) for a, b in evs]
            ms = sorted(series)
            n = len(ms)
            med = 0.0 if n == 0 else (ms[n // 2] if n % 2 else 0.5 * (ms[n // 2 - 1] + ms[n // 2]))
            out[name] = (n, sum(ms) / max(n, 1), ms[0] if n else 0.0, med, ms[-1] if n else 0.0, series)
            for a, b in evs:
                pool += [a, b]
        if self.profile is not None:
            self.profile.clear()
        return out

    def release(self):
        self._buf.clear()
        self._b_tag = None

    @contextlib.contextmanager
    def private_buffers(self):
        saved = self._buf, self._b_tag
        self._buf, self._b_tag = {}, None
        try:
            yield self._buf
        finally:
            self._buf, self._b_tag = saved

    def fork(self, reads=(), writes=(), **payload):
        return self._side.fork(reads, writes, **payload)

    @property
    def side_open(self) -> bool:
        return self._side.stream is not None

    def slots(self) -> int:
        if self._slots is None:
            with torch.cuda.device(self.device):
                s = int(self._fn("tsvgp_site_accum_slots")())
            if s <= 0:
                raise B.HipExtensionError("tsvgp_site_accum_slots failed")
            self._slots = s
        return self._slots

    def choose_nsplit(self, Mp: int, P: int, Np: int = None) -> int:
        return site_sum_slices(Mp, P, Np, self.slots(), self.dtype == torch.float64, self.syrk_oversubscribe)

    def _padded_gamma(self, gamma: torch.Tensor, Mp: int, P: int) -> torch.Tensor:
# ... 527 lines not shown
        elif isinstance(kernel, (list, tuple)):
            kernels = list(kernel)
        else:
            kernels = [kernel]
        if len(kernels) not in (1, P):
            raise ValueError(f"predict_vjp: one kernel or one per latent (P = {P}), got {len(kernels)}")
        if len(kernels) == P and all(k is kernels[0] for k in kernels):
            kernels = kernels[:1]
        Np, Mp = B.round_up(N), B.round_up(M)
        self._b_tag = None
        self._side.wait_stale()
        Kfu = self._get("Kfu", (Np, Mp), T)
        Ubuf = self._get("U", (Np, Mp), T)
        dX = torch.empty((N, D), dtype=torch.float64, device=dev)
        for p in range(P):
            kern = kernels[p if len(kernels) > 1 else 0]
            if p == 0 or len(kernels) > 1:
                self.se_fill(X, Z, kern.inv_lengthscales(D, T, dev), kern.variance.item(), Kfu, kern.kind)
            torch.mm(Kfu, self._pad_square(0.5 * (Q[p] + Q[p].T), Mp, "pad_Q"), out=Ubuf)
            self.moments_vjp(X, Z, kern, Ubuf, cm[:, p], cv[:, p], beta[:, p], dX, accumulate=p > 0)
        return dX

    def selftest_mfma(self, dtype=None):
        dtype = dtype or self.dtype
        g = torch.Generator(device="cpu").manual_seed(7)
        a = torch.randn(16, 4, generator=g, dtype=torch.float64).to(dtype).to(self.device)
        b = torch.randn(4, 16, generator=g, dtype=torch.float64).to(dtype).to(self.device)
        c = torch.zeros(16, 16, dtype=dtype, device=self.device)
        with torch.cuda.device(self.device):
            B.check(self._fn("tsvgp_selftest_mfma", dtype)(a.data_ptr(), b.data_ptr(), c.data_ptr(), self._stream()),
                    "tsvgp_selftest_mfma")
        return a, b, c

    batch_separate = True
    batch_mem_fraction = 0.8

    _per_latent = staticmethod(per_latent)

    def _batch_plan(self, N, M, kernel, P, whiten_T, whiten_mode, project_T, moments_on_kfu, D=0):
        if not self.batch_separate or P < 2 or P > B.MAX_BATCH or moments_on_kfu:
            return None
        if len({k.kind for k in kernel.kernels}) != 1:
            return None
        if D > MAX_INPUT_DIM:
            return None
        if any(self._per_latent(project_T, p) is not None for p in range(P)):
            return None
        whitened = [p for p in range(P) if self._per_latent(whiten_T, p) is not None]
        if whitened and whiten_mode != B.TRI_UPPER:
            return None
        Np, Mp = B.round_up(N), B.round_up(M)
        need = P * Np * Mp * torch.empty((), dtype=self.dtype).element_size()
        have = self._buf.get("KfuP")
        if have is None or tuple(have.shape) != (P, Np, Mp) or have.dtype != self.dtype:
            free, _ = torch.cuda.mem_get_info(self.device)
            free += torch.cuda.memory_reserved(self.device) - torch.cuda.memory_allocated(self.device)
            if have is not None:
                free += have.numel() * have.element_size()
            if need > self.batch_mem_fraction * free:
                return None
        return whitened

    def _fill_batched(self, X, Z, kernel, KfuP):
        T, dev = self.dtype, self.device
        N, D = X.shape
        M = Z.shape[0]
        if D > MAX_INPUT_DIM:
            raise ValueError(f"input dimension D = {D} exceeds the HIP fill kernel's limit of {MAX_INPUT_DIM}")
        P = len(kernel.kernels)
        inv_ls = torch.stack([k.inv_lengthscales(D, T, dev) for k in kernel.kernels]).contiguous()
        ctype = ctypes.c_double if T == torch.float64 else ctypes.c_float
        fn = self._fn("tsvgp_kernel_fill_batched", T)
        stride = KfuP.shape[1] * KfuP.shape[2]
        with torch.cuda.device(dev):
            for p0 in range(0, P, B.MAX_BATCH):
                n = min(B.MAX_BATCH, P - p0)
                var = (ctype * n)(*[k.variance.item() for k in kernel.kernels[p0:p0 + n]])
                self._launch("tsvgp_se_fill", lambda: fn(kernel.kernels[0].kind, X.data_ptr(), Z.data_ptr(),
                                                         inv_ls[p0].data_ptr(), var, KfuP[p0].data_ptr(), stride, N, M, D,
                                                         KfuP.shape[2], n, self._stream()))
        return KfuP

    def _run_batched(self, X, Y, Z, kernel, whitened, *, moment_Tm, moment_mode, gamma, lik_id, lik_param, whiten_T,
                     sites, want_moments, want_grads, mean_only, prefill=None, mix=None) -> EStepStats:
        T, dev = self.dtype, self.device
        X = X.to(device=dev, dtype=T).contiguous()
        Z = Z.to(device=dev, dtype=T).contiguous()
        N, M, P = X.shape[0], Z.shape[0], moment_Tm.shape[0]
        Np, Mp = B.round_up(N), B.round_up(M)
        need_g = lik_id != B.LIK_NONE
        mapped = (lik_id & 0xFF) in B.MAPPED_LIKS or (need_g and mix is not None)
        if need_g:
            Y = Y.to(device=dev, dtype=T).contiguous()
        self._b_tag = None
        self._buf.pop("Kfu", None)
        self._buf.pop("B", None)
        KfuP = self._get("KfuP", (P, Np, Mp), T)
        stride = Np * Mp
        if prefill is not None:
            prefill.take("KfuP", KfuP)
        else:
            self._side.wait_stale()
            self._fill_batched(X, Z, kernel, KfuP)
        runs, start = [], None
        for p in range(P + 1):
            on = p < P and p in whitened
            if on and start is None:
                start = p
            if not on and start is not None:
                runs.append((start, p))
                start = None
        fn_trmm = self._fn("tsvgp_trmm_batched")
        self.last_trmm_batch = max([hi - lo for lo, hi in runs], default=1)
        for lo, hi in runs:
            Wt = torch.stack([self._per_latent(whiten_T, p) for p in range(lo, hi)])
            Wp = self._pad_square(Wt, Mp, f"pad_LinvP{hi - lo}")
            with torch.cuda.device(dev):
                self._launch("tsvgp_trmm", lambda: fn_trmm(KfuP[lo].data_ptr(), stride, Wp.data_ptr(), Mp * Mp,
                                                           KfuP[lo].data_ptr(), stride, Np, Mp, B.TRI_UPPER, hi - lo,
                                                           self._stream()))
        Tm = self._pad_square(moment_Tm, Mp, "pad_Tm")
        gam = self._padded_gamma(gamma, Mp, P)
        kdiag = [k.variance.item() for k in kernel.kernels]
        lm = None
        if mapped:
            mean, var, lm = self._moments_then_map(KfuP, Tm, gam, kdiag, Y, lik_id, lik_param, N, Np, moment_mode, mean_only, mix)
            g0, g1, ve_partial, nonpos_partial = lm.g0, lm.g1, lm.ve_partial, lm.nonpos_partial
        else:
            g0 = self._get("g0", (Np, P), T) if need_g else None
            g1 = self._get("g1", (Np, P), T) if need_g else None
            mean = torch.empty((N, P), dtype=T, device=dev) if want_moments else None
            var = torch.empty((N, P), dtype=T, device=dev) if (want_moments and not mean_only) else None
            ve_partial, nonpos_partial = self.moments(KfuP, Tm, gam, kdiag, N, moment_mode, lik_id=lik_id, lik_param=lik_param,
                                                      mean_only=mean_only, Y=Y if need_g else None, mean=mean, var=var, g0=g0, g1=g1)
        stats = EStepStats(n_rows=N, ve_sum=ve_partial.sum(), nonpos=nonpos_partial.sum().to(torch.float64),
                           dparam=None if lm is None else lm.dparam)
        if want_moments:
            stats.mean = mean.to(torch.float64, copy=mapped)
            stats.var = None if var is None else var.to(torch.float64, copy=mapped)
        if want_grads and need_g:
            stats.g0, stats.g1 = g0[:N].to(torch.float64), g1[:N].to(torch.float64)
        self._mixed_stats(stats, lm, N, want_moments, want_grads)
        if sites:
            stats.acc2, stats.acc1 = self._site_sums(KfuP, g0, g1, P, M)
        self.last_batched = True
        return stats

    def _run_separate(self, X, Y, Z, kernel, *, moment_Tm, gamma, whiten_T, project_T, want_grads, prefill=None,
                      **kw) -> EStepStats:
        P = moment_Tm.shape[0]
        if len(kernel.kernels) != P:
            raise ValueError(f"{len(kernel.kernels)} kernels for {P} latent GPs")
        lik_id = kw.get("lik_id", B.LIK_NONE)
        mix = kernel.device_W(self.device) if (isinstance(kernel, LinearCoregionalization) and lik_id != B.LIK_NONE) else None
        if mix is not None:
            kw["mean_only"] = False
        mapped = (lik_id & 0xFF) in B.MAPPED_LIKS or mix is not None
        if mapped or Y is not None:
            self._check_y(Y, X.shape[0], P, lik_id, kw.get("lik_param"), outputs=None if mix is None else mix.shape[0])
        if X.shape[0] > 0:
            if prefill is not None and prefill.name == "KfuP":
                whitened = [p for p in range(P) if self._per_latent(whiten_T, p) is not None]
            else:
                whitened = self._batch_plan(X.shape[0], Z.shape[0], kernel, P, whiten_T,
                                            kw.get("whiten_mode", B.TRI_UPPER), project_T, kw.get("moments_on_kfu", False),
                                            D=X.shape[1])
            if whitened is not None:
                return self._run_batched(X, Y, Z, kernel, whitened, moment_Tm=moment_Tm, moment_mode=kw["moment_mode"],
                                         gamma=gamma, lik_id=kw.get("lik_id", B.LIK_NONE), lik_param=kw.get("lik_param", 0.0),
                                         whiten_T=whiten_T, sites=kw.get("sites", False),
                                         want_moments=kw.get("want_moments", False), want_grads=want_grads,
                                         mean_only=kw.get("mean_only", False), prefill=prefill, mix=mix)
        self.last_batched = False
        if mapped and X.shape[0] > 0:
            return self._run_separate_coupled(X, Y, Z, kernel, moment_Tm=moment_Tm, gamma=gamma, whiten_T=whiten_T,
                                              project_T=project_T, want_grads=want_grads, mix=mix, **kw)
        parts = []
        for p, kp in enumerate(kernel.kernels):
            st = self.run(X, None if (Y is None or mix is not None) else Y[:, p:p + 1], Z, kp, moment_Tm=moment_Tm[p:p + 1], gamma=gamma[:, p:p + 1],
                          whiten_T=per_latent(whiten_T, p), project_T=per_latent(project_T, p), want_grads=want_grads, **kw)
            if want_grads and st.g0 is not None:
                st.g0, st.g1 = st.g0.clone(), st.g1.clone()
            parts.append(st)

        def cat(name, dim):
            vals = [getattr(s, name) for s in parts]
            return None if vals[0] is None else torch.cat(vals, dim=dim)

        out = EStepStats(n_rows=parts[0].n_rows, ve_sum=sum(s.ve_sum for s in parts), nonpos=sum(s.nonpos for s in parts))
        out.mean, out.var, out.g0, out.g1 = cat("mean", 1), cat("var", 1), cat("g0", 1), cat("g1", 1)
        out.acc2, out.acc1 = cat("acc2", 0), cat("acc1", 0)
        return out

    def _run_separate_coupled(self, X, Y, Z, kernel, *, moment_Tm, gamma, whiten_T, project_T, want_grads, lik_id, sites=False,
                              want_moments=False, mean_only=False, mix=None, **kw) -> EStepStats:
        if mean_only:
            raise ValueError("mean_only needs a likelihood whose gradients do not depend on the predictive variance")
        T, dev = self.dtype, self.device
        N, P = X.shape[0], moment_Tm.shape[0]
        Np = B.round_up(N)
        lik_param = kw.pop("lik_param", None)
        per = self._per_latent
        mean = self._get("coupled_mean", (N, P), T)
        var = self._get("coupled_var", (N, P), T)
        for p, kp in enumerate(kernel.kernels):
            st = self.run(X, None, Z, kp, moment_Tm=moment_Tm[p:p + 1], gamma=gamma[:, p:p + 1], whiten_T=per(whiten_T, p),
                          want_moments=True, **kw)
            mean[:, p] = st.mean[:, 0]
            var[:, p] = st.var[:, 0]
        Yc = Y.to(device=dev, dtype=T).contiguous()
        if mix is not None:
            lm = self._mixed_map(mean, var, Yc, mix, lik_id, lik_param, N, Np)
        else:
            lm = self.lik_map(mean, var, Yc, lik_id, lik_param, N, Np)
        g0, g1 = lm.g0, lm.g1
        out = EStepStats(n_rows=N, ve_sum=lm.ve_partial.sum(), nonpos=lm.nonpos_partial.sum().to(torch.float64), dparam=lm.dparam)
        if want_moments:
            out.mean, out.var = mean.to(torch.float64, copy=True), var.to(torch.float64, copy=True)
        if want_grads:
            out.g0, out.g1 = g0[:N].to(torch.float64, copy=True), g1[:N].to(torch.float64, copy=True)
        self._mixed_stats(out, lm, N, want_moments, want_grads)
        if sites:
            acc2, acc1 = [], []
            for p, kp in enumerate(kernel.kernels):
                st = self.run(X, None, Z, kp, moment_Tm=moment_Tm[p:p + 1], gamma=gamma[:, p:p + 1], whiten_T=per(whiten_T, p),
                              project_T=per(project_T, p), sites=True, site_grads=(g0[:, p:p + 1], g1[:, p:p + 1]), **kw)
                acc2.append(st.acc2)
                acc1.append(st.acc1)
            out.acc2, out.acc1 = torch.cat(acc2, dim=0), torch.cat(acc1, dim=0)
        return out

    def start_fill(self, X, Z, kernel, b_tag=None, want="Kfu", routes=None):
        if self.device.type != "cuda" or X.shape[0] == 0:
            return None
        T, dev = self.dtype, self.device
        N, D = X.shape
        M = Z.shape[0]
        Np, Mp = B.round_up(N), B.round_up(M)
        separate = isinstance(kernel, SeparateIndependent)
        if separate:
            P = len(kernel.kernels)
            if routes is None or any(r == "projected" for r in routes):
                return None
            if self._batch_plan(N, M, kernel, P, None, B.TRI_UPPER, None, False, D=D) is None:
                return None
        elif (b_tag is not None and self._b_tag == (want, b_tag) and self._buf.get(want) is not None
                and tuple(self._buf[want].shape) == (Np, Mp)):
            return None
        Xc = X.to(device=dev, dtype=T).contiguous()
        Zc = Z.to(device=dev, dtype=T).contiguous()
        self._b_tag = None
        if separate:
            self._buf.pop("Kfu", None)
            self._buf.pop("B", None)
            buf = self._get("KfuP", (P, Np, Mp), T)
            with self.fork(reads=(Xc, Zc), writes=(buf,), name="KfuP", buf=buf) as branch:
                self._fill_batched(Xc, Zc, kernel, buf)
        else:
            inv_ls = kernel.inv_lengthscales(D, T, dev)
            variance = kernel.variance.item()
            buf = self._get("Kfu", (Np, Mp), T)
            with self.fork(reads=(Xc, Zc, inv_ls), writes=(buf,), name="Kfu", buf=buf,
                           key=(X.data_ptr(), tuple(X.shape), Z.data_ptr(), tuple(Z.shape), id(kernel))) as branch:
                self.se_fill(Xc, Zc, inv_ls, variance, buf, kernel.kind)
        return branch

    def run(self, X, Y, Z, kernel, *, moment_Tm, moment_mode, gamma, lik_id=B.LIK_NONE, lik_param=0.0,
            whiten_T=None, whiten_mode=B.TRI_UPPER, project_T=None, sites=False, want_moments=False, want_grads=False,
            b_tag=None, mean_only=False, prefill=None, moments_on_kfu=False, project_mode=B.TRI_LOWER,
            keep_tile=False, site_grads=None) -> EStepStats:
        if isinstance(kernel, SeparateIndependent):
            return self._run_separate(X, Y, Z, kernel, moment_Tm=moment_Tm, moment_mode=moment_mode, gamma=gamma,
                                      lik_id=lik_id, lik_param=lik_param, whiten_T=whiten_T, whiten_mode=whiten_mode,
                                      project_T=project_T, sites=sites, want_moments=want_moments, want_grads=want_grads,
                                      mean_only=mean_only, moments_on_kfu=moments_on_kfu, project_mode=project_mode,
                                      prefill=prefill)
        if site_grads is not None and lik_id != B.LIK_NONE:
            raise ValueError("site_grads replaces the likelihood: lik_id must be LIK_NONE")
        if mean_only and (lik_id & 0xFF) not in (B.LIK_NONE, B.LIK_GAUSSIAN):
            raise ValueError("mean_only needs a likelihood whose gradients do not depend on the predictive variance")
        T, dev = self.dtype, self.device
        X = X.to(device=dev, dtype=T).contiguous()
        Z = Z.to(device=dev, dtype=T).contiguous()
        N, D = X.shape
        M = Z.shape[0]
        P = moment_Tm.shape[0]
        if N == 0:
            if world_size() == 1:
                raise ValueError("empty data: natgrad_step / elbo need at least one row")
            zero = torch.zeros((), dtype=torch.float64, device=dev)
            st = EStepStats(n_rows=0, ve_sum=zero, nonpos=zero.clone())
            if sites:
                st.acc2 = torch.zeros((P, M, M), dtype=torch.float64, device=dev)
                st.acc1 = torch.zeros((P, M), dtype=torch.float64, device=dev)
            if want_moments:
                st.mean = torch.zeros((0, P), dtype=torch.float64, device=dev)
                st.var = None if mean_only else torch.zeros((0, P), dtype=torch.float64, device=dev)
            return st
        if X.dim() != 2 or Z.dim() != 2 or Z.shape[1] != D:
            raise ValueError(f"X must be [N, D] and Z [M, D] with equal D, got {tuple(X.shape)} and {tuple(Z.shape)}")
        mapped = (lik_id & 0xFF) in B.MAPPED_LIKS
        if lik_id != B.LIK_NONE:
            self._check_y(Y, N, P, lik_id, lik_param)
            Y = Y.to(device=dev, dtype=T).contiguous()
        Np, Mp = B.round_up(N), B.round_up(M)
        inv_ls = kernel.inv_lengthscales(D, T, dev)
        variance = kernel.variance.item()

        want = "B" if whiten_T is not None else "Kfu"
        late_whiten = moments_on_kfu and whiten_T is not None
        if late_whiten:
            b_tag = None
        reuse = (b_tag is not None and self._b_tag == (want, b_tag) and self._buf.get(want) is not None
                 and tuple(self._buf[want].shape) == (Np, Mp))
        if reuse:
            A = self._buf[want]
        else:
            self._b_tag = None
            Kfu = self._get("Kfu", (Np, Mp), T)
            if prefill is not None:
                prefill.take("Kfu", Kfu)
            else:
                self._side.wait_stale()
                self.se_fill(X, Z, inv_ls, variance, Kfu, kernel.kind)
            A = Kfu
            if whiten_T is not None and not late_whiten:
                Bw = self._get("B", (Np, Mp), T)
                self.trmm(Kfu, self._pad_square(whiten_T, Mp, "pad_Linv"), Bw, whiten_mode)
                A = Bw
            if b_tag is not None:
                self._b_tag = (want, b_tag)

        Tm = self._pad_square(moment_Tm, Mp, "pad_Tm")
        gam = self._padded_gamma(gamma, Mp, P)
        need_g = lik_id != B.LIK_NONE or site_grads is not None
        g0 = self._get("g0", (Np, P), T) if need_g else None
        g1 = self._get("g1", (Np, P), T) if need_g else None
        mean = torch.empty((N, P), dtype=T, device=dev) if want_moments else None
        var = torch.empty((N, P), dtype=T, device=dev) if (want_moments and not mean_only) else None
        tile, lm = None, None
        if site_grads is not None:
            g0.copy_(site_grads[0])
            g1.copy_(site_grads[1])
        if keep_tile:
            if P != 1 or mean_only or whiten_T is not None or not need_g:
                raise ValueError("keep_tile: one latent, a likelihood, no whitening")
            if mapped:
                raise ValueError("keep_tile: a likelihood whose map runs behind the moments comes in through site_grads")
            tile = self._get("Tt", (Np, Mp), T)
            self.trmm(A, Tm[0], tile, moment_mode)
            mean = torch.mv(A[:N], gam[:, 0]).reshape(N, 1)
            var = (variance - torch.linalg.vector_norm(tile[:N], dim=1).square()).reshape(N, 1)
            if site_grads is None:
                res = self.lik_map(mean, var, Y, lik_id, lik_param, N, Np, g0=g0, g1=g1)
                ve_partial, nonpos_partial = res.ve_partial, res.nonpos_partial
        elif mapped:
            mean, var, lm = self._moments_then_map(A, Tm, gam, variance, Y, lik_id, lik_param, N, Np, moment_mode, mean_only)
            g0, g1, ve_partial, nonpos_partial = lm.g0, lm.g1, lm.ve_partial, lm.nonpos_partial
            if want_moments:
                mean, var = mean.clone(), var.clone()
        elif site_grads is not None and not want_moments:
            pass
        else:
            own = site_grads is None
            ve_partial, nonpos_partial = self.moments(A, Tm, gam, variance, N, moment_mode, lik_id=lik_id, lik_param=lik_param,
                                                      mean_only=mean_only, Y=Y if lik_id != B.LIK_NONE else None, mean=mean,
                                                      var=var, g0=g0 if own else None, g1=g1 if own else None)
        if site_grads is not None:
            zero = torch.zeros((), dtype=torch.float64, device=dev)
            stats = EStepStats(n_rows=N, ve_sum=zero, nonpos=zero.clone())
        else:
            stats = EStepStats(n_rows=N, ve_sum=ve_partial.sum(), nonpos=nonpos_partial.sum().to(torch.float64),
                               dparam=None if lm is None else lm.dparam)
        stats.tile = tile
        if want_moments:
            stats.mean, stats.var = mean.to(torch.float64), (None if var is None else var.to(torch.float64))
        if want_grads and need_g:
            stats.g0, stats.g1 = g0[:N].to(torch.float64), g1[:N].to(torch.float64)

        if late_whiten and sites:
            Bw = self._get("B", (Np, Mp), T)
            self.trmm(A, self._pad_square(whiten_T, Mp, "pad_Linv"), Bw, whiten_mode)
            A = Bw
        if sites and project_T is not None:
            if whiten_T is None:
                raise ValueError("project_T needs whiten_T")
            Aproj = self._get("Kfu", (Np, Mp), T)
            self.trmm(A, self._pad_square(project_T, Mp, "pad_proj"), Aproj, project_mode)
            A = Aproj
        if sites:
            stats.acc2, stats.acc1 = self._site_sums(A, g0, g1, P, M)
        return stats

    def _site_sums(self, A, g0, g1, P, M):
        dev = self.device
        Np, Mp = A.shape[-2:]
        nsplit = self.nsplit_override or self.choose_nsplit(Mp, P, Np)
        nsplit = max(1, min(nsplit, Np // site_sum_chunk_rows(self.dtype == torch.float64, P)))
        nbytes = int(self._fn("tsvgp_site_accum_work_bytes")(Mp, P, nsplit))
        work = self._get("work", (nbytes,), torch.uint8)
        acc2 = torch.empty((P, Mp, Mp), dtype=torch.float64, device=dev)
        acc1 = torch.empty((P, Mp), dtype=torch.float64, device=dev)
        if A.dim() == 3:
            fn, operand = self._fn("tsvgp_site_accum_batched"), (A.data_ptr(), Np * Mp)
        else:
            fn, operand = self._fn("tsvgp_site_accum"), (A.data_ptr(),)
        with torch.cuda.device(dev):
            self._launch("tsvgp_site_accum", lambda: fn(*operand, g0.data_ptr(), g1.data_ptr(), acc2.data_ptr(), acc1.data_ptr(),
                                                        work.data_ptr(), Np, Mp, P, nsplit, self._stream()))
        return acc2[:, :M, :M], acc1[:, :M]

    def run_two_product(self, X, Y, Z, kernel, *, whiten_T, moment_Tm, gamma, lik_id=B.LIK_NONE, lik_param=0.0, sites=False,
                        want_moments=False, prefill=None) -> EStepStats:
        T, dev = self.dtype, self.device
        st = self.run(X, None, Z, kernel, moment_Tm=moment_Tm, moment_mode=B.TRI_UPPER, gamma=gamma, lik_id=B.LIK_NONE,
                      whiten_T=whiten_T, whiten_mode=B.TRI_UPPER, want_moments=True, prefill=prefill)
        N, M = X.shape[0], Z.shape[0]
        Np, Mp = B.round_up(N), B.round_up(M)
        Bw = self._buf["B"]
        kff = kernel.variance.item()
        bn = torch.linalg.vector_norm(Bw[:N], dim=1).to(torch.float64)
        var = (2.0 * kff - bn * bn)[:, None] - st.var
        stats = EStepStats(n_rows=N, ve_sum=torch.zeros((), dtype=torch.float64, device=dev), nonpos=(~(var > 0)).sum().to(torch.float64))
        if want_moments:
            stats.mean, stats.var = st.mean, var
        if lik_id != B.LIK_NONE:
            Yc = Y.to(device=dev, dtype=T).contiguous()
            self._check_y(Yc, N, 1, lik_id, lik_param)
            lm = self.lik_map(st.mean.to(T).contiguous(), var.to(T).contiguous(), Yc, lik_id, lik_param, N, Np,
                              g0=self._get("g0", (Np, 1), T), g1=self._get("g1", (Np, 1), T))
            stats.ve_sum, stats.nonpos, stats.dparam = lm.ve_partial.sum(), lm.nonpos_partial.sum().to(torch.float64), lm.dparam
            if sites:
                stats.acc2, stats.acc1 = self._site_sums(Bw, lm.g0, lm.g1, 1, M)
        return stats

    def cov(self, tile: torch.Tensor, C: torch.Tensor, N: int, *, sign: float = -1.0, X=None, inv_ls=None, variance: float = 0.0,
            kind: int = B.KERNEL_SE, accumulate: bool = False):
        Np, Mp = tile.shape
        if C.dtype != tile.dtype or C.shape[0] != Np or C.stride(1) != 1 or tile.stride(1) != 1 or tile.stride(0) != Mp:
            raise ValueError("cov: tile [Np, Mp] contiguous and C [Np, >= Np] with unit column stride, in one dtype")
        D = 0 if accumulate else X.shape[1]
        fn = self._fn("tsvgp_cov", tile.dtype)
        with torch.cuda.device(self.device):
            self._launch("tsvgp_cov", lambda: fn(int(kind), tile.data_ptr(), _ptr(None if accumulate else X),
                                                 _ptr(None if accumulate else inv_ls), float(variance), float(sign), C.data_ptr(),
                                                 int(N), Np, Mp, D, C.stride(0), B.COV_ACCUMULATE if accumulate else 0,
                                                 self._stream()))
        return C

    def full_cov(self, X, Z, kernel, *, moment_Tm, moment_mode, gamma, whiten_T=None, whiten_mode=B.TRI_UPPER,
                 two_product=False, padded=False):
        T, dev = self.dtype, self.device
        X = X.to(device=dev, dtype=T).contiguous()
        Z = Z.to(device=dev, dtype=T).contiguous()
        if X.dim() != 2 or Z.dim() != 2 or Z.shape[1] != X.shape[1]:
            raise ValueError(f"X must be [N, D] and Z [M, D] with equal D, got {tuple(X.shape)} and {tuple(Z.shape)}")
        N, D = X.shape
        M = Z.shape[0]
        P = moment_Tm.shape[0]
        if N == 0:
            raise ValueError("full_cov needs at least one test point")
        separate = isinstance(kernel, SeparateIndependent)
        if separate and len(kernel.kernels) != P:
            raise ValueError(f"{len(kernel.kernels)} kernels for {P} latent GPs")
        if two_product and (P != 1 or whiten_T is None or separate):
            raise ValueError("two_product: one latent, one kernel, a whitening factor")
        Np, Mp = B.round_up(N), B.round_up(M)
        esz = 8 if T == torch.float64 else 4
        need = (2 if padded else 1) * P * Np * Np * 8 + (0 if T == torch.float64 else Np * Np * esz) + 3 * Np * Mp * esz
        free, _ = torch.cuda.mem_get_info(dev)
        free += torch.cuda.memory_reserved(dev) - torch.cuda.memory_allocated(dev)
        if need > free:
            raise ValueError(f"full_cov: {P} joint covariance(s) of {N} test points need {need / 2 ** 30:.1f} GiB of device memory "
                             f"({P} x {Np} x {Np} fp64), {free / 2 ** 30:.1f} GiB are free; predict fewer points at a time")
        self._b_tag = None
        cov = torch.empty((P, Np, Np), dtype=torch.float64, device=dev)
        Cw = None if T == torch.float64 else torch.empty((Np, Np), dtype=T, device=dev)
        mean = torch.empty((N, P), dtype=torch.float64, device=dev)
        gam = self._padded_gamma(gamma, Mp, P)
        Kfu = self._get("Kfu", (Np, Mp), T)
        tile = self._get("Tt", (Np, Mp), T)
        self._side.wait_stale()
        for p in range(P):
            kp = kernel.kernels[p] if separate else kernel
            inv_ls, variance = kp.inv_lengthscales(D, T, dev), kp.variance.item()
            if p == 0 or separate:
                self.se_fill(X, Z, inv_ls, variance, Kfu, kp.kind)
            A = Kfu
            wt = self._per_latent(whiten_T, p)
            if wt is not None:
                A = self._get("B", (Np, Mp), T)
# ... 349 lines not shown
```

t-svgp_amd/models/tsvgp.py:

```python
from __future__ import annotations

import abc
import functools
import os
import warnings

import numpy as np
import torch

from .. import _backend as B
from .. import distributed as D_
from ..base import default_device, default_float, default_jitter, to_tensor
from ..estep import EStepStats, per_latent
from ..side_branch import poll_current_stream
from ..inducing_variables import inducingpoint_wrapper
from ..kernels import LinearCoregionalization, SeparateIndependent, latent_kernels
from ..likelihoods import mapped_parameter
from ..sites import DenseSites
from ..util import (
    bmv,
    cholesky_deferred,
    cond2_estimate,
    gradient_transformation_mean_var_to_expectation,
    info_sum,
    kl_from_dense_site,
    posterior_from_dense_site,
    rev_cholesky,
)


def _kmv(K: torch.Tensor, v: torch.Tensor) -> torch.Tensor:
    return bmv(K, v)


def _ktmv(K: torch.Tensor, v: torch.Tensor) -> torch.Tensor:
    return bmv(K, v, transpose=True)


class _PredictF(torch.autograd.Function):

    @staticmethod
    def forward(ctx, X, model):
        from ..pathwise import _private_copy

        mean, var, beta, Q = model._predict_marginal(X.detach(), want_operands=True)
        ctx.engine = model._get_engine()
        if isinstance(model.kernel, SeparateIndependent):
            ctx.kernels = [_private_copy(k) for k in model.kernel.kernels]
        else:
            ctx.kernels = [_private_copy(model.kernel)]
        ctx.save_for_backward(X, model._Z().detach().clone(), beta.detach().clone(), Q.detach().clone())
        return mean, var

    @staticmethod
    @torch.autograd.function.once_differentiable
    def backward(ctx, grad_mean, grad_var):
        X, Z, beta, Q = ctx.saved_tensors
        return ctx.engine.predict_vjp(X, Z, ctx.kernels, beta, Q, grad_mean, grad_var), None


class base_SVGP(abc.ABC):

    def __init__(self, kernel, likelihood, inducing_variable, *, mean_function=None, num_latent_gps=1, num_data=None,
                 compute_dtype=None, device=None):
        if mean_function is not None:
            raise NotImplementedError("only the default Zero mean function is on the hot path")
        self.kernel = kernel
        self.likelihood = likelihood
        self.mean_function = None
        self.num_latent_gps = num_latent_gps
        self.num_data = num_data
        self.inducing_variable = inducingpoint_wrapper(inducing_variable)
        self.compute_dtype = compute_dtype or default_float()
        self.device = torch.device(device) if device is not None else default_device()
        self._engine = None
        self._engine64 = None
        self._sample_draw = 0
        self._function_draw = 0
        self.poll_status = True
        self.data_parallel = None

    def _get_engine(self):
        if self._engine is None:
            from ..estep import EStepEngine

            self._engine = EStepEngine(self.compute_dtype, self.device)
        return self._engine

    def _reduce(self) -> bool:
        return D_.collectives_on() if self.data_parallel is None else bool(self.data_parallel)

    def _read_flags(self, flags: torch.Tensor) -> torch.Tensor:
        if not flags.is_cuda:
            return flags
        host = getattr(self, "_flags_host", None)
        if host is None or host.numel() != flags.numel():
            host = self._flags_host = torch.empty(flags.numel(), dtype=flags.dtype).pin_memory()
        host.copy_(flags, non_blocking=True)
        if not self.poll_status:
            torch.cuda.current_stream(flags.device).synchronize()
            return host.clone()
        poll_current_stream(flags.device)
        return host.clone()

    @abc.abstractmethod
    def get_mean_chol_cov_inducing_posterior(self):
        raise NotImplementedError

    def _lmc(self):
        return self.kernel if isinstance(self.kernel, LinearCoregionalization) else None

    def _refuse_lmc(self, what: str):
        if self._lmc() is not None:
            raise NotImplementedError(f"{what} is not implemented for LinearCoregionalization: the mixed outputs have marginal "
                                      "predictions (predict_f, full_output_cov, predict_y, predict_log_density) only")

    _BOTH_COV = "full_cov and full_output_cov together (the [N, P, N, P] covariance) are not implemented"

    def _joint(self, Xnew, padded=False, engine=None):
        raise NotImplementedError

    def _sample_engine(self):
        if self.compute_dtype == torch.float64:
            return self._get_engine()
        if self._engine64 is None:
            from ..estep import EStepEngine

            self._engine64 = EStepEngine(torch.float64, self.device)
        return self._engine64

    def predict_f_samples(self, Xnew, num_samples=None, full_cov=True, full_output_cov=False, *, seed=0, draw=None,
                          epsilon=None):
        if full_cov and full_output_cov:
            raise NotImplementedError(self._BOTH_COV)
        self._refuse_lmc("predict_f_samples")
        eng = self._sample_engine() if full_cov else self._get_engine()
        S = 1 if num_samples is None else int(num_samples)
        P = int(self.num_latent_gps)
        if not (1 <= P <= B.MAX_BATCH):
            raise ValueError(f"predict_f_samples draws for at most {B.MAX_BATCH} latent GPs (TSVGP_MAX_BATCH), got {P}")
        if not (1 <= S <= B.MC_MAX_SAMPLES):
            raise ValueError(f"num_samples must lie in [1, {B.MC_MAX_SAMPLES}], got {num_samples}")
        if full_cov:
            mean, covp = self._joint(Xnew, padded=True, engine=eng)
        else:
            mean, var = self.predict_f(Xnew)
        N = mean.shape[0]
        if epsilon is None:
            if draw is None:
                draw = self._sample_draw
                self._sample_draw = draw + 1
            eps = eng.mc_normals(S, N, P, seed, draw)
        else:
            eps = torch.as_tensor(epsilon, dtype=torch.float64).to(self.device)
            if tuple(eps.shape) != (S, N, P):
                raise ValueError(f"epsilon must be [S, N, P] = [{S}, {N}, {P}], got {tuple(eps.shape)}")
        if full_cov:
            covp.diagonal(dim1=-2, dim2=-1).add_(default_jitter())
            L, info = eng.cholesky(covp, overwrite=True)
            if float(self._read_flags(info.abs().sum().reshape(1).to(torch.float64))[0]) != 0:
                raise FloatingPointError("Cholesky decomposition was not successful (matrix not positive definite)")
            f = (mean.t()[:, :, None] + torch.matmul(L[:, :N, :N], eps.permute(2, 1, 0))).permute(2, 1, 0).contiguous()
        else:
            f = mean[None] + torch.sqrt(var)[None] * eps
        return f[0] if num_samples is None else f

    def sample_functions(self, num_samples, num_features=1024, *, seed=0, draw=None):
        from ..pathwise import sample_functions

        self._refuse_lmc("sample_functions")
        eng = self._sample_engine()
        P = int(self.num_latent_gps)
        if not (1 <= P <= B.MAX_BATCH):
            raise ValueError(f"sample_functions draws for at most {B.MAX_BATCH} latent GPs (TSVGP_MAX_BATCH), got {P}")
        S, L = int(num_samples), int(num_features)
        if not (1 <= S <= B.MC_MAX_SAMPLES):
            raise ValueError(f"num_samples must lie in [1, {B.MC_MAX_SAMPLES}], got {num_samples}")
        if L < 1:
            raise ValueError(f"num_features must be at least 1, got {num_features}")
        advance = draw is None
        if advance:
            draw = self._function_draw
        fs = sample_functions(self, eng, S, L, int(seed), int(draw))
        if advance:
            self._function_draw = draw + 1
        return fs

    def _predict_marginal(self, Xd, want_operands=False):
        raise NotImplementedError

# ... 587 lines not shown
            if not sep:
                G = G.sum(dim=0, keepdim=True)
            kl = kl_from_dense_site(ops["K6"], l1, Dm, ops["U_W"], beta)
            with torch.enable_grad():
                Kt = torch.stack([k.K_torch(Z_t, v_, l_) for k, v_, l_ in zip(kernels, var_t, ls_t)])
                knn = sum(v_ * s_ for v_, s_ in zip(var_t, sum_g1))
                g_all = torch.autograd.grad(torch.sum(G.detach() * Kt) + scale * knn, var_t + ls_t + [Z_t])
        g_var, g_ls, g_Z = g_all[:nk], g_all[nk:2 * nk], g_all[-1]
        grads = {"Z": g_Z + scale * dZ}
        for ki, k in enumerate(kernels):
            ls_shape = k.lengthscales.value.shape
            n_ls = scale * dls[ki]
            pre = f"kernels.{ki}." if sep else ""
            grads[pre + "variance"] = g_var[ki] + scale * dvar[ki]
            grads[pre + "lengthscales"] = g_ls[ki] + (n_ls.sum() if len(ls_shape) == 0 else n_ls.reshape(ls_shape))
        if gaussian:
            s2 = self.likelihood.lik_param
            grads["likelihood_variance"] = scale * (-0.5 * rows * n_out / s2 + 0.5 * res / (s2 * s2))
        if lik_par is not None:
            grads[lik_par[0]] = scale * res
        if lmc:
            grads["W"] = scale * dW.reshape(n_out, P)
        elbo = ve_sum * scale - kl
        return elbo, grads

    def natgrad_step(self, data, lr=0.1, jitter=1e-9):
        X, Y = self._as_device(data[0]), self._as_device(data[1])
        self._check_targets(X, Y)
        routes = self._routes(jitter)
        draw0 = getattr(self.likelihood, "draw", None)
        if self._wants_graph(X) and self._graph_step(X, Y, lr, jitter, routes):
            return
        old_l1, old_L = self.lambda_1.value, self.lambda_2_sqrt.value
        while True:
            soft = any(r != "projected" for r in routes)
            if draw0 is not None and self.likelihood.draw != draw0:
                self.likelihood.draw = draw0
            try:
                flags = self._step_device(X, Y, lr, jitter, routes)
                verdict = self._judge(self._read_flags(flags), soft_final=soft)
            except FloatingPointError:
                self.lambda_1.assign(old_l1)
                self.sites.assign_lambda_2_sqrt(old_L)
                raise
            if verdict is True:
                return
            self.lambda_1.assign(old_l1)
            self.sites.assign_lambda_2_sqrt(old_L)
            routes = [self._DEMOTE.get(r, r) for r in routes]
            if self.projection == "auto" and self._cond_cache is not None:
                self._cond_cache[2].update({p: r for p, r in enumerate(routes)})

    def _step_front(self, X, Y, lr, jitter, routes):
        warm_key = self._warm_key(X, jitter)
        eng = self._get_engine()
        pre = ops = None
        fork = not (self.device.type == "cuda" and torch.cuda.is_current_stream_capturing()
                    and X.shape[0] * self.num_inducing < self.GRAPH_FORK_MIN_NM)
        Kzz = K6 = None
        if self.overlap_fill and fork and hasattr(eng, "start_fill"):
            if not (warm_key is not None and self._warm is not None and self._warm[0] == warm_key):
                Kzz = eng.kuu(self._Z(), self.kernel)
                K6 = self._k6(Kzz)
            want = "Kfu" if all(r == "direct" for r in routes) else "B"
            if X.shape[0] * self.num_inducing <= self.FILL_INLINE_MAX_NM:
                pass
            elif self._late_fill(X):
                box = {}
                ops = self._site_operands(whiten_jitter=jitter, warm_key=warm_key, routes=routes, fork=fork, Kzz=Kzz, K6=K6,
                                          after_w=lambda: box.update(pre=eng.start_fill(X, self._Z(), self.kernel, b_tag=warm_key,
                                                                                        want=want, routes=routes)),
                                          beside_fill=self._fill_outlasts_factorisation(X))
                pre = box.get("pre")
            else:
                pre = eng.start_fill(X, self._Z(), self.kernel, b_tag=warm_key, want=want, routes=routes)
        if ops is None:
            ops = self._site_operands(whiten_jitter=jitter, warm_key=warm_key, routes=routes, fork=fork, Kzz=Kzz, K6=K6,
                                      beside_fill=pre is not None)
        st = eng.run(X, Y, ops["Z"], self.kernel, moment_Tm=ops["moment_Tm"], prefill=pre,
                     moment_mode=ops["moment_mode"], gamma=ops["gamma"],
                     lik_id=self.likelihood.lik_id, lik_param=self.likelihood.lik_param,
                     whiten_T=ops["whiten_T"], whiten_mode=ops["whiten_mode"], project_T=ops["project_T"],
                     moments_on_kfu=ops["moments_on_kfu"], project_mode=ops["project_mode"],
                     sites=True, b_tag=warm_key,
                     mean_only=self.skip_unused_variance and self.likelihood.lik_id == B.LIK_GAUSSIAN)
        return st, ops

    FILL_INLINE_MAX_NM = int(os.environ.get("TSVGP_FILL_INLINE_MAX_NM", "0"))
    LATE_FILL_MAX_NM = int(os.environ.get("TSVGP_LATE_FILL_MAX_NM", "300000000"))

    def _fill_outlasts_factorisation(self, X) -> bool:
        esize = 8 if self.compute_dtype == torch.float64 else 4
        return X.shape[0] * self.num_inducing * esize >= 1_600_000_000

    def _late_fill(self, X) -> bool:
        return X.shape[0] * self.num_inducing <= self.LATE_FILL_MAX_NM

    def _step_device(self, X, Y, lr, jitter, routes, inplace=False) -> torch.Tensor:
        if not inplace and self._latent_split(routes):
            return self._step_device_split(X, Y, lr, jitter, routes)
        st, ops = self._step_front(X, Y, lr, jitter, routes)
        return self._apply_site_update(st, ops, lr, jitter, inplace=inplace)

    def _latent_split(self, routes) -> bool:
        if self.latent_split is False or not isinstance(self.kernel, SeparateIndependent) or not self._reduce():
            return False
        if self._lmc() is not None:
            return False
        if D_.world_size() < 2 and not D_.FORCE_COLLECTIVES:
            return False
        return self.num_latent_gps >= 2 and all(r in ("direct", "whitened") for r in routes) and not self.cache_whitened

    def _step_device_split(self, X, Y, lr, jitter, routes) -> torch.Tensor:
        eng = self._get_engine()
        P, M = self.num_latent_gps, self.num_inducing
        G, r = max(D_.world_size(), 1), D_.rank()
        own = [p for p in range(P) if p % G == r]
        per = (P + G - 1) // G
        owner_order = [p for q in range(G) for p in range(q, P, G)]
        dev, f64 = self.device, torch.float64
        tri = M * (M + 1) // 2
        pre = None
        if self.overlap_fill and hasattr(eng, "start_fill"):
            pre = eng.start_fill(X, self._Z(), self.kernel, want="B", routes=routes)
        ops = self._site_operands(whiten_jitter=jitter, routes=[routes[p] for p in own], latents=own) if own else None
        slot = 2 * M * M + M
        send = torch.zeros(per * slot, dtype=f64, device=dev)
        for i, p in enumerate(own):
            o = i * slot
            send[o:o + M * M] = ops["moment_Tm"][i].reshape(-1)
            send[o + M * M:o + M * M + M] = ops["gamma"][:, i]
            wt = per_latent(ops["whiten_T"], i)
            if routes[p] != "direct" and wt is not None:
                send[o + M * M + M:o + slot] = wt.reshape(-1)
        allops = D_.all_gather_flat(send).reshape(G, per, slot)
        Tm_full = torch.empty((P, M, M), dtype=f64, device=dev)
        gamma_full = torch.empty((M, P), dtype=f64, device=dev)
        whiten_full = [None] * P
        for p in range(P):
            blk = allops[p % G, p // G]
            Tm_full[p] = blk[:M * M].reshape(M, M)
            gamma_full[:, p] = blk[M * M:M * M + M]
            if routes[p] != "direct":
                whiten_full[p] = blk[M * M + M:].reshape(M, M)
        if all(wt is None for wt in whiten_full):
            whiten_full = None
        st = eng.run(X, Y, self._Z(), self.kernel, moment_Tm=Tm_full, prefill=pre, moment_mode=B.TRI_UPPER, gamma=gamma_full,
                     lik_id=self.likelihood.lik_id, lik_param=self.likelihood.lik_param, whiten_T=whiten_full,
                     whiten_mode=B.TRI_UPPER, project_T=None, sites=True,
                     mean_only=self.skip_unused_variance and self.likelihood.lik_id == B.LIK_GAUSSIAN)
        blk = tri + M
        packed = torch.zeros(G * per * blk, dtype=f64, device=dev)
        acc2, acc1 = st.acc2.to(f64), st.acc1.to(f64)
        i_, j_ = torch.tril_indices(M, M, device=dev)
        for q in range(G):
            for i, p in enumerate(range(q, P, G)):
                o = (q * per + i) * blk
                packed[o:o + tri] = acc2[p][i_, j_]
                packed[o + tri:o + blk] = acc1[p]
        mine = D_.reduce_scatter_sum(packed, G)
        scal = torch.stack([st.ve_sum.reshape(()).to(f64), st.nonpos.reshape(()).to(f64),
                            torch.full((), float(st.n_rows), dtype=f64, device=dev)])
        D_.all_reduce_sum(scal)
        nonpos, rows = scal[1], scal[2]
        state = torch.zeros(per * blk, dtype=f64, device=dev)
        flags = torch.zeros(3, dtype=f64, device=dev)
        if own:
            a2 = torch.zeros((len(own), M, M), dtype=f64, device=dev)
            a1 = torch.empty((len(own), M), dtype=f64, device=dev)
            for i in range(len(own)):
                v = mine[i * blk:i * blk + tri]
                a2[i][i_, j_] = v
                a2[i][j_, i_] = v
                a1[i] = mine[i * blk + tri:(i + 1) * blk]
            flags, l1_new, L_new = self._apply_site_update(None, ops, lr, jitter, reduced=(a2, a1, nonpos, rows), latents=own)
            for i in range(len(own)):
                state[i * blk:i * blk + tri] = L_new[i][i_, j_]
                state[i * blk + tri:(i + 1) * blk] = l1_new[:, i]
        else:
            flags[1] = nonpos
        allstate = D_.all_gather_flat(state).reshape(G, per, blk)
        L_full = torch.zeros((P, M, M), dtype=f64, device=dev)
        l1_full = torch.empty((M, P), dtype=f64, device=dev)
        for p in range(P):
            sb = allstate[p % G, p // G]
            L_full[p][i_, j_] = sb[:tri]
            l1_full[:, p] = sb[tri:]
        self.lambda_1.assign_owned(l1_full)
        self.sites.assign_lambda_2_sqrt(L_full, lower_and_owned=True)
        return D_.all_reduce_max(flags.abs())

    GRAPH_AUTO_MAX_NM = int(os.environ.get("TSVGP_GRAPH_AUTO_MAX_NM", "200000000"))
    GRAPH_FORK_MIN_NM = int(os.environ.get("TSVGP_GRAPH_FORK_MIN_NM", "100000000"))
    GRAPH_SINGLE_MIN_NM = 10_000_000

    def _wants_graph(self, X) -> bool:
        if self.use_graph == "auto":
            return X.shape[0] * self.num_inducing <= self.GRAPH_AUTO_MAX_NM
        return bool(self.use_graph)

    def _graph_step(self, X, Y, lr, jitter, routes) -> bool:
        if self.device.type != "cuda":
            return False
        eng = self._get_engine()
        lmc = self._lmc()
        if self.cache_whitened or eng.profile is not None or (isinstance(self.kernel, SeparateIndependent) and lmc is None):
            return False
        two = self._reduce()
        lik_v = tuple(p.stamp() for p in vars(self.likelihood).values() if hasattr(p, "stamp"))
        if hasattr(self.likelihood, "graph_key"):
            lik_v += self.likelihood.graph_key()
        draw0 = getattr(self.likelihood, "draw", None)
        if lmc is not None:
            lik_v += (lmc.W.stamp(),)
            lmc.device_W(self.device)
        key = (X.data_ptr(), Y.data_ptr(), tuple(X.shape), tuple(Y.shape), X.dtype, Y.dtype, self._kernel_versions(),
               lik_v, self.inducing_variable.Z.stamp(), float(lr), float(jitter), tuple(routes), self.num_data)
        entry = self._graphs.get(key)
        if entry is None:
            if len(self._graphs) >= 64:
                self._graphs = {k: v for k, v in self._graphs.items() if isinstance(v, dict)}
            self._graphs[key] = "seen"
            return False
        l1p, Lp = self.lambda_1, self.sites._lambda_2_sqrt
        if entry == "seen":
            big = X.shape[0] * self.num_inducing > self.GRAPH_SINGLE_MIN_NM
            if len(self._graphs) > 4 or (big and any(isinstance(v, dict) for v in self._graphs.values())):
                self._graphs = {key: "seen"}
            sl1, sL = l1p.value.clone(), Lp.value.clone()
            bl1, bL = torch.empty_like(sl1), torch.empty_like(sL)
            l1p._value, Lp._value = sl1, sL
            graph = torch.cuda.CUDAGraph()
# ... 132 lines not shown
```

t-svgp_amd/models/tsvgp_white.py:

```python
from __future__ import annotations

import functools

import numpy as np
import torch

from .. import _backend as B
from .. import distributed as D_
from ..base import default_jitter, to_tensor
from ..kernels import LinearCoregionalization, SeparateIndependent
from ..sites import DenseSites
from ..util import cholesky_deferred, cond2_estimate, info_sum, rev_cholesky
from .tsvgp import _PredictF, base_SVGP


class _DirectRouteFailed(Exception):
    """The direct projection's own M x M factorisation failed: the caller repeats the call on the whitened route."""


class _SingleProductFailed(Exception):
    """Lambda_2 + 1e-9 I (or I + H^T H built on its factor) is not positive definite while K_uu's factorisations went through:
    the single-product variance does not exist; the caller repeats the call with the reference's own two-product form, which
    only needs K + Lambda_2 + 1e-9 I (src/util.py:73-86)."""

# ... 28 lines not shown
        lambda_1 = np.zeros((num_inducing, self.num_latent_gps)) if lambda_1 is None else lambda_1
        if lambda_2 is None:
            lambda_2 = np.array([np.eye(num_inducing) * 1e-10 for _ in range(self.num_latent_gps)])
        else:
            lambda_2 = lambda_2.value if hasattr(lambda_2, "value") else lambda_2
            assert lambda_2.ndim == 3
            self.num_latent_gps = lambda_2.shape[0]
        self.sites = DenseSites(to_tensor(lambda_1, device=self.device), lambda_2=to_tensor(lambda_2, device=self.device))

    @property
    def lambda_1(self):
        return self.sites.lambda_1

    @property
    def lambda_2(self):
        return self.sites._lambda_2

    def _Z(self):
        return self.inducing_variable.Z.value.to(self.device)

    def _as_device(self, a):
        if isinstance(a, torch.Tensor):
            return a.to(self.device)
        return torch.as_tensor(np.asarray(a)).to(self.device)

    def _operands(self, jitter=None, *, kuu_jitter=None, lambda_1=None, lambda_2=None, direct=False, two_product=False):
        eng = self._get_engine()
        Z = self._Z()
        M = Z.shape[0]
        infos = []
        potrf = getattr(eng, "cholesky", None)
        if potrf is not None and self._cond_k6() > self.ROBUST_MIN_COND:
            potrf = functools.partial(potrf, robust=True)
        Kzz = eng.kuu(Z, self.kernel)
        Id = torch.eye(M, dtype=torch.float64, device=Kzz.device)
        K6 = Kzz + (default_jitter() if kuu_jitter is None else kuu_jitter) * Id
        l1 = self.lambda_1.value if lambda_1 is None else lambda_1
        L2 = self.lambda_2.value if lambda_2 is None else lambda_2
        E = 0.5 * (L2 + L2.transpose(-1, -2)) + 1e-9 * Id
        if two_product:
            mats = [K6[None], (E + K6)[None] if E.dim() == 2 else E + K6] + ([(Kzz + jitter * Id)[None]] if jitter is not None else [])
            U, Uinv = rev_cholesky(torch.cat(mats, dim=0), infos, potrf, inverse=True)
            U6, Uinv6, UinvR = U[0], Uinv[0], Uinv[1]
            T2 = (UinvR @ U6).triu()
            gamma = U6.transpose(-1, -2) @ (UinvR.transpose(-1, -2) @ (UinvR @ l1))
            ops = dict(Z=Z, Kzz=Kzz, K6=K6, Id=Id, infos=infos, e_infos=[], U6=U6, Uinv6=Uinv6, moment_Tm=T2[None], gamma=gamma,
                       moment_mode=B.TRI_UPPER, whiten_T=Uinv6, direct=False, direct_info=None, two_product=True)
            if jitter is not None:
                ops["K9inv"] = Uinv[2].transpose(-1, -2) @ Uinv[2]
            return ops
        mats = [K6[None], E] + ([(Kzz + jitter * Id)[None]] if jitter is not None else [])
        all_infos = []
        U, Uinv = rev_cholesky(torch.cat(mats, dim=0), all_infos, potrf, inverse=True)
        infos = [torch.cat([all_infos[0][:1], all_infos[0][2:]])]
        e_infos = [all_infos[0][1:2]]
        U6, Uinv6, U_E = U[0], Uinv[0], U[1]
        H = (Uinv6 @ U_E).triu()
        Wm = Id + H.transpose(-1, -2) @ H
        _, Cinv = cholesky_deferred(0.5 * (Wm + Wm.transpose(-1, -2))[None], e_infos, potrf, inverse=True, overwrite=True)
        Tm = (Cinv[0] @ H.transpose(-1, -2)).tril()
        v = Uinv6 @ l1
        gamma = v - Tm.transpose(-1, -2) @ (Tm @ v)
        ops = dict(Z=Z, Kzz=Kzz, K6=K6, Id=Id, infos=infos, e_infos=e_infos, U6=U6, Uinv6=Uinv6, moment_Tm=Tm[None], gamma=gamma,
                   moment_mode=B.TRI_LOWER, whiten_T=Uinv6, direct=False, direct_info=None, two_product=False)
        if direct:
            G = Tm @ Uinv6
            Q = G.transpose(-1, -2) @ G
            dinfo = []
            Lq = cholesky_deferred(Q[None], dinfo, potrf, overwrite=True)
            ops.update(moment_Tm=Lq.transpose(-1, -2).contiguous(), moment_mode=B.TRI_UPPER, whiten_T=None, direct=True,
                       gamma=Uinv6.transpose(-1, -2) @ gamma, direct_info=dinfo)
        if jitter is not None:
            ops["K9inv"] = Uinv[2].transpose(-1, -2) @ Uinv[2]
        return ops

    def _run(self, X, Y, ops, lik_id, sites=False, want_moments=False):
        if ops.get("two_product"):
            return self._get_engine().run_two_product(X, Y, ops["Z"], self.kernel, whiten_T=ops["whiten_T"],
                                                      moment_Tm=ops["moment_Tm"], gamma=ops["gamma"], lik_id=lik_id,
                                                      lik_param=self.likelihood.lik_param, sites=sites, want_moments=want_moments)
        return self._get_engine().run(X, Y, ops["Z"], self.kernel, moment_Tm=ops["moment_Tm"], moment_mode=ops["moment_mode"],
                                      gamma=ops["gamma"], lik_id=lik_id, lik_param=self.likelihood.lik_param,
                                      whiten_T=ops["whiten_T"], whiten_mode=B.TRI_UPPER, sites=sites,
                                      want_moments=want_moments)

    def _check(self, ops, nonpos):
        zero = torch.zeros(1, dtype=torch.float64, device=self.device)
        parts = [info_sum(ops["infos"]), nonpos.reshape(1).to(torch.float64),
                 info_sum(ops["direct_info"]) if ops.get("direct_info") else zero,
                 info_sum(ops["e_infos"]) if ops.get("e_infos") else zero]
        flags = self._read_flags(torch.cat(parts))
        if float(flags[0]) != 0:
            raise FloatingPointError("Cholesky decomposition was not successful (matrix not positive definite)")
        if float(flags[3]) != 0:
            raise _SingleProductFailed()
        if float(flags[2]) != 0:
            raise _DirectRouteFailed()
        if not (float(flags[1]) == 0):
            if ops.get("direct") and self.projection == "auto":
                raise _DirectRouteFailed()
            raise FloatingPointError(f"non-positive predictive variance at {float(flags[1]):.0f} point(s)")

    DIRECT_MAX_COND = {torch.float64: 1.0e3, torch.float32: 30.0}

    ROBUST_MIN_COND = 1.0e6

    def _cond_k6(self) -> float:
        k, Zp = self.kernel, self.inducing_variable.Z
        key = (id(k), k.variance.stamp(), k.lengthscales.stamp(), Zp.stamp())
        if self._cond_cache is None or self._cond_cache[0] != key:
            eng = self._get_engine()
            Kzz = eng.kuu(self._Z(), k)
            Kzz.diagonal(dim1=-2, dim2=-1).add_(default_jitter())
            cond = cond2_estimate(Kzz, getattr(eng, "cholesky", None)).reshape(1)
            self._cond_cache = (key, float(D_.broadcast_from_rank0(cond.contiguous())))
            self._direct_failed = False
        return self._cond_cache[1]

    def _use_direct(self) -> bool:
        if self.projection != "auto":
            return self.projection == "direct"
        return self._cond_k6() <= self.DIRECT_MAX_COND[self.compute_dtype] and not self._direct_failed

    def _routed(self, fn):
        if not self._two_product and self._use_direct():
            try:
                return fn(direct=True, two_product=False)
            except _DirectRouteFailed:
                if self.projection != "auto":
                    raise FloatingPointError("the direct projection lost definiteness; use projection='whitened'")
                self._direct_failed = True
            except _SingleProductFailed:
                self._two_product = True
        if not self._two_product:
            try:
                return fn(direct=False, two_product=False)
            except _SingleProductFailed:
                self._two_product = True
        return fn(direct=False, two_product=True)

    def get_mean_chol_cov_inducing_posterior(self):
        ops = self._operands()
        K6 = ops["K6"]
        R = K6 + self.lambda_2.value[0] + 1e-9 * ops["Id"]
        LR = torch.linalg.cholesky(R)
        iLRK = torch.linalg.solve_triangular(LR, K6, upper=False)
        S_q = iLRK.transpose(-1, -2) @ iLRK
        Rl = torch.linalg.solve_triangular(LR.transpose(-1, -2), torch.linalg.solve_triangular(
            LR, self.lambda_1.value, upper=False), upper=True)
        m_q = K6 @ Rl
        return m_q, torch.linalg.cholesky(S_q)[None]

    def prior_kl(self):
        eng = self._get_engine()
        Kzz = eng.kuu(self._Z(), self.kernel)
        Id = torch.eye(Kzz.shape[0], dtype=torch.float64, device=Kzz.device)
        A = Kzz + default_jitter() * Id
        R = self.lambda_2.value[0] + A
        LR, LA = torch.linalg.cholesky(R), torch.linalg.cholesky(A)
        log_det = 2.0 * (torch.sum(torch.log(torch.diagonal(LR))) - torch.sum(torch.log(torch.diagonal(LA))))
        tmp = torch.linalg.solve_triangular(LR, LA, upper=False)
        Rl = torch.linalg.solve_triangular(LR.transpose(-1, -2), torch.linalg.solve_triangular(
            LR, self.lambda_1.value, upper=False), upper=True)
        return 0.5 * (log_det + torch.sum(tmp * tmp) - float(A.shape[0]) + torch.sum(torch.square(LA.transpose(-1, -2) @ Rl)))

    def predict_f(self, Xnew, full_cov=False, full_output_cov=False):
        if full_cov and full_output_cov:
# ... 152 lines not shown
```

Measured before the change: 29.91 E-steps/s.

## Add constant-weight SYRK site accumulation path for homoskedastic Gaussian likelihood

```diff
diff --git a/include/tsvgp_hip.h b/include/tsvgp_hip.h
--- a/include/tsvgp_hip.h
+++ b/include/tsvgp_hip.h
@@ -173,6 +173,14 @@
                                  double *acc1, void *work, int64_t Np, int Mp, int P, int nsplit, void *stream);
 int tsvgp_site_accum_batched_f32(const float *B, int64_t strideB, const float *g0, const float *g1, double *acc2,
                                  double *acc1, void *work, int64_t Np, int Mp, int P, int nsplit, void *stream);
+int tsvgp_site_accum_cw_f64(const double *B, const double *g0, const double *g1_const, double *acc2, double *acc1, void *work,
+                            int64_t Np, int Mp, int P, int nsplit, void *stream);
+int tsvgp_site_accum_cw_f32(const float *B, const float *g0, const double *g1_const, double *acc2, double *acc1, void *work,
+                            int64_t Np, int Mp, int P, int nsplit, void *stream);
+int tsvgp_site_accum_cw_batched_f64(const double *B, int64_t strideB, const double *g0, const double *g1_const, double *acc2,
+                                    double *acc1, void *work, int64_t Np, int Mp, int P, int nsplit, void *stream);
+int tsvgp_site_accum_cw_batched_f32(const float *B, int64_t strideB, const float *g0, const double *g1_const, double *acc2,
+                                    double *acc1, void *work, int64_t Np, int Mp, int P, int nsplit, void *stream);
 
 #define TSVGP_POTRF_SUBST 1
 #define TSVGP_POTRF_DIAG_V1 4
diff --git a/t-svgp_amd/_backend.py b/t-svgp_amd/_backend.py
--- a/t-svgp_amd/_backend.py
+++ b/t-svgp_amd/_backend.py
@@ -170,6 +170,10 @@
     "tsvgp_site_accum_work_bytes_f32": (c_int64, [c_int, c_int, c_int]),
     "tsvgp_site_accum_f64": (c_int, [c_void_p, c_void_p, c_void_p, c_void_p, c_void_p, c_void_p, c_int64, c_int, c_int, c_int, c_void_p]),
     "tsvgp_site_accum_f32": (c_int, [c_void_p, c_void_p, c_void_p, c_void_p, c_void_p, c_void_p, c_int64, c_int, c_int, c_int, c_void_p]),
+    "tsvgp_site_accum_cw_f64": (c_int, [c_void_p, c_void_p, c_void_p, c_void_p, c_void_p, c_void_p, c_int64, c_int, c_int, c_int, c_void_p]),
+    "tsvgp_site_accum_cw_f32": (c_int, [c_void_p, c_void_p, c_void_p, c_void_p, c_void_p, c_void_p, c_int64, c_int, c_int, c_int, c_void_p]),
+    "tsvgp_site_accum_cw_batched_f64": (c_int, [c_void_p, c_int64, c_void_p, c_void_p, c_void_p, c_void_p, c_void_p, c_int64, c_int, c_int, c_int, c_void_p]),
+    "tsvgp_site_accum_cw_batched_f32": (c_int, [c_void_p, c_int64, c_void_p, c_void_p, c_void_p, c_void_p, c_void_p, c_int64, c_int, c_int, c_int, c_void_p]),
     "tsvgp_potrf_f64": (c_int, [c_void_p, c_int, c_int, c_int, c_int64, c_void_p, c_void_p, c_int, c_void_p]),
     "tsvgp_potrf_solve_f64": (c_int, [c_void_p, c_int, c_int, c_int, c_int64, c_void_p, c_void_p, c_int, c_int, c_void_p]),
     "tsvgp_vgp_system_f64": (c_int, [c_int, c_void_p, c_void_p, c_double, c_double, c_void_p, c_void_p, c_void_p, c_int64, c_int64, c_int,
diff --git a/t-svgp_amd/csrc/tsvgp_kernels.hip b/t-svgp_amd/csrc/tsvgp_kernels.hip
--- a/t-svgp_amd/csrc/tsvgp_kernels.hip
+++ b/t-svgp_amd/csrc/tsvgp_kernels.hip
@@ -2284,7 +2284,7 @@
 constexpr int S1_IMG = KC * LDS_KS;
 constexpr int S1_BUF = 2 * S1_IMG;
 
-template <bool DIAG, int W>
+template <bool DIAG, int W, bool CW>
 __device__ __forceinline__ void syrk1_body(const SyrkArgs<double>& a, double* lds, double* wl, int p, int it, int jt, int sidx, int slab,
                                            int per_p, int w) {
     typedef v4d acc_t;
@@ -2300,7 +2300,8 @@
 
     constexpr int MB = DIAG ? 8 - W : 8;
     constexpr int NM = DIAG ? 9 : 16;
-    constexpr int NR = 2 + MB;
+    constexpr int NR = DIAG ? MB : 2 + MB;
+    constexpr int F0 = (DIAG && CW) ? 2 : 0;
 
     const int lr = lane & 15, lk = lane >> 4;
     const int offa0 = lk * LDS_KS + w * 16 + lr;
@@ -2337,7 +2338,7 @@
     const uint64_t g1_u = uni64(a.g1), g0_u = uni64(a.g0);
     const uint64_t wchunk = (uint64_t)KC * P * sizeof(double);
     auto dma_weights = [&](const int64_t c, const int buf) TSVGP_AI {
-        if (w == 0 || (DIAG && w == 1)) {
+        if ((!CW && w == 0) || (DIAG && w == 1)) {
             const unsigned la = wl_u + (unsigned)((buf * 256 + (w == 1 ? 128 : 0)) * sizeof(double));
             const uint64_t g = (w == 1 ? g0_u : g1_u) + (uint64_t)c * wchunk;
             const unsigned vo_ = dvo;
@@ -2356,7 +2357,8 @@
         if constexpr (I < 4) w1r[I] = wl[buf * 256 + woff + I * 4 * P];
         else w0r[I - 4] = wl[buf * 256 + 128 + woff + (I - 4) * 4 * P];
     };
-    constexpr int NW = DIAG ? 8 : 4;
+    constexpr int NW = (CW ? 0 : 4) + (DIAG ? 4 : 0);
+    constexpr int W0 = CW ? 4 : 0;
 
     acc_t acc[2][8];
 #pragma unroll
@@ -2374,11 +2376,24 @@
     };
     auto rds = [&](Frag1<double>& f, auto slot_tag, auto ks_tag, const int boff) TSVGP_AI {
         constexpr int S = decltype(slot_tag)::value;
-        if constexpr (S < MB) rd1(f, TSVGP_IC(2 + S), ks_tag, boff);
+        if constexpr (DIAG) {
+            constexpr int blk = S == 0 ? 7 - W : S == 1 ? W : (S - 2 < W ? S - 2 : S - 1);
+            rd1(f, TSVGP_IC(2 + blk), ks_tag, boff);
+        } else if constexpr (S < MB) rd1(f, TSVGP_IC(2 + S), ks_tag, boff);
         else rd1(f, TSVGP_IC(S - MB), ks_tag, boff);
     };
+    auto weigh = [&](auto& f, auto ks_tag) TSVGP_AI {
+        constexpr int KW = decltype(ks_tag)::value;
+        if constexpr (!CW && DIAG) {
+            f.v[0] = f.v[2 + W] * w1r[KW];
+            f.v[1] = f.v[2 + 7 - W] * w1r[KW];
+        } else if constexpr (!CW) {
+            f.v[0] *= w1r[KW];
+            f.v[1] *= w1r[KW];
+        }
+    };
     auto keep_set = [&](const Frag1<double>& f) TSVGP_AI {
-        cfor<0, NR>([&](auto e) TSVGP_AI {
+        cfor<F0, 2 + MB>([&](auto e) TSVGP_AI {
             const double x = f.v[decltype(e)::value];
             asm volatile("" ::"v"(x));
         });
@@ -2391,7 +2406,8 @@
         } else {
             constexpr int n = (I < 2 * (W + 1)) ? (I >> 1) : (I - (W + 1));
             constexpr int sblk = (I < 2 * (W + 1)) ? (I & 1) : 1;
-            acc[sblk][n] = __builtin_amdgcn_mfma_f64_16x16x4f64(f.v[sblk], f.v[2 + n], acc[sblk][n], 0, 0, 0);
+            constexpr int ea = CW ? 2 + (sblk ? 7 - W : W) : sblk;
+            acc[sblk][n] = __builtin_amdgcn_mfma_f64_16x16x4f64(f.v[ea], f.v[2 + n], acc[sblk][n], 0, 0, 0);
         }
     };
     v2d f1[4];
@@ -2416,8 +2432,7 @@
                     f1[I - NR] = *reinterpret_cast<const v2d*>(lds + off1 + B0 + (I - NR) * 4 * LDS_KS);
                 TSVGP_SB();
             });
-            nxt.v[0] *= w1r[KS_ + 1];
-            nxt.v[1] *= w1r[KS_ + 1];
+            weigh(nxt, TSVGP_IC(KS_ + 1));
             if constexpr (DIAG && KS_ == 1) {
 #pragma unroll
                 for (int q = 0; q < 4; ++q) {
@@ -2438,13 +2453,12 @@
                 constexpr int I = decltype(i)::value;
                 if constexpr (I < NM) mf(fy, i);
                 if constexpr (I < NDMA) dma_piece(TSVGP_IC(DIAG ? 2 * I : I), BUF);
-                else if constexpr (I < NDMA + NW) read_weight(TSVGP_IC(I - NDMA), BUF ^ 1);
+                else if constexpr (I < NDMA + NW) read_weight(TSVGP_IC(W0 + I - NDMA), BUF ^ 1);
                 else if constexpr (I < S3) rds(fx, TSVGP_IC(I - NDMA - NW), TSVGP_IC(0), B1);
                 TSVGP_SB();
             });
             dma_weights(c_fetch, BUF);
-            fx.v[0] *= w1r[0];
-            fx.v[1] *= w1r[0];
+            weigh(fx, TSVGP_IC(0));
             TSVGP_SB();
         } else {
             cfor<0, NM>([&](auto i) TSVGP_AI { mf(fy, i); });
@@ -2463,10 +2477,9 @@
         asm volatile("s_waitcnt vmcnt(0) lgkmcnt(0)" ::: "memory");
         __builtin_amdgcn_s_barrier();
         asm volatile("" ::: "memory");
-        cfor<0, NW>([&](auto i) TSVGP_AI { read_weight(i, 0); });
+        cfor<0, NW>([&](auto i) TSVGP_AI { read_weight(TSVGP_IC(W0 + decltype(i)::value), 0); });
         cfor<0, NR>([&](auto i) TSVGP_AI { rds(fx, i, TSVGP_IC(0), 0); });
-        fx.v[0] *= w1r[0];
-        fx.v[1] *= w1r[0];
+        weigh(fx, TSVGP_IC(0));
         int i = 0;
         const int64_t c_last = c_hi - 1;
         auto fetch_of = [&](int idx) TSVGP_AI { const int64_t c = c_lo + idx + 2; return c < c_last ? c : c_last; };
@@ -2511,10 +2524,8 @@
     }
 }
 
-__global__ __launch_bounds__(NTHREADS, 1) void syrk1_kernel(SyrkArgs<double> a) {
-    __shared__ __attribute__((aligned(1024))) double lds[2 * S1_BUF];
-    __shared__ __attribute__((aligned(1024))) double wl[2 * 256];
-
+template <bool CW>
+__device__ __forceinline__ void syrk1_main(const SyrkArgs<double>& a, double* lds, double* wl) {
     const int w = __builtin_amdgcn_readfirstlane(threadIdx.x >> 6);
     const int nt = a.nt, n_off = nt * (nt - 1) / 2;
     const int per_p = n_off * a.ns_off + nt * a.ns_diag;
@@ -2536,16 +2547,28 @@
     const int tri = it * (it + 1) / 2 + jt;
     const int slab = (tri - it) * a.ns_off + it * a.ns_diag + sidx;
     if (it != jt) {
-        syrk1_body<false, 0>(a, lds, wl, p, it, jt, sidx, slab, per_p, w);
+        syrk1_body<false, 0, CW>(a, lds, wl, p, it, jt, sidx, slab, per_p, w);
     } else if (w == 0) {
-        syrk1_body<true, 0>(a, lds, wl, p, it, jt, sidx, slab, per_p, w);
+        syrk1_body<true, 0, CW>(a, lds, wl, p, it, jt, sidx, slab, per_p, w);
     } else if (w == 1) {
-        syrk1_body<true, 1>(a, lds, wl, p, it, jt, sidx, slab, per_p, w);
+        syrk1_body<true, 1, CW>(a, lds, wl, p, it, jt, sidx, slab, per_p, w);
     } else if (w == 2) {
-        syrk1_body<true, 2>(a, lds, wl, p, it, jt, sidx, slab, per_p, w);
+        syrk1_body<true, 2, CW>(a, lds, wl, p, it, jt, sidx, slab, per_p, w);
     } else {
-        syrk1_body<true, 3>(a, lds, wl, p, it, jt, sidx, slab, per_p, w);
-    }
+        syrk1_body<true, 3, CW>(a, lds, wl, p, it, jt, sidx, slab, per_p, w);
+    }
+}
+
+__global__ __launch_bounds__(NTHREADS, 1) void syrk1_kernel(SyrkArgs<double> a) {
+    __shared__ __attribute__((aligned(1024))) double lds[2 * S1_BUF];
+    __shared__ __attribute__((aligned(1024))) double wl[2 * 256];
+    syrk1_main<false>(a, lds, wl);
+}
+
+__global__ __launch_bounds__(NTHREADS, 1) void syrk1_kernel_cw(SyrkArgs<double> a) {
+    __shared__ __attribute__((aligned(1024))) double lds[2 * S1_BUF];
+    __shared__ __attribute__((aligned(1024))) double wl[2 * 256];
+    syrk1_main<true>(a, lds, wl);
 }
 
 constexpr int S1F_KC = 32;
@@ -2553,7 +2576,7 @@
 constexpr int S1F_BUF = 2 * S1F_IMG;
 constexpr int S1F_WL = 512;
 
-template <bool DIAG, int W>
+template <bool DIAG, int W, bool CW>
 __device__ __forceinline__ void syrk1f_body(const SyrkArgs<float>& a, float* lds, float* wl, int p, int it, int jt, int sidx,
                                             int slab, int per_p, int w) {
     typedef v4f acc_t;
@@ -2570,7 +2593,8 @@
 
     constexpr int MB = DIAG ? 8 - W : 8;
     constexpr int NM = DIAG ? 9 : 16;
-    constexpr int NR = 2 + MB;
+    constexpr int NR = DIAG ? MB : 2 + MB;
+    constexpr int F0 = (DIAG && CW) ? 2 : 0;
     constexpr int NKS = S1F_KC / 4;
 
     const int lr = lane & 15, lk = lane >> 4, odd = lk & 1;
@@ -2610,7 +2634,7 @@
     const uint64_t g1_u = uni64(a.g1), g0_u = uni64(a.g0);
     const uint64_t wchunk = (uint64_t)S1F_KC * P * sizeof(float);
     auto dma_weights = [&](const int64_t c, const int buf) TSVGP_AI {
-        if (w == 0 || (DIAG && w == 1)) {
+        if ((!CW && w == 0) || (DIAG && w == 1)) {
             const unsigned la = wl_u + (unsigned)((buf * S1F_WL + (w == 1 ? 256 : 0)) * sizeof(float));
             const uint64_t g = (w == 1 ? g0_u : g1_u) + (uint64_t)c * wchunk;
             const unsigned vo_ = dvw;
@@ -2629,7 +2653,8 @@
         if constexpr (I < NKS) w1r[I] = wl[buf * S1F_WL + woff + I * 4 * P];
         else w0r[I - NKS] = wl[buf * S1F_WL + 256 + woff + (I - NKS) * 4 * P];
     };
-    constexpr int NWH = DIAG ? 8 : 4;
+    constexpr int NWH = (CW ? 0 : 4) + (DIAG ? 4 : 0);
+    constexpr int WH0 = CW ? 4 : 0;
     auto read_weight_half = [&](auto j_tag, auto half_tag, const int buf) TSVGP_AI {
         constexpr int J = decltype(j_tag)::value, H = decltype(half_tag)::value;
         if constexpr (J < 4) read_weight(TSVGP_IC(4 * H + J), buf);
@@ -2652,11 +2677,24 @@
     };
     auto rds = [&](Frag& f, auto slot_tag, auto ks_tag, const int boff) TSVGP_AI {
         constexpr int S = decltype(slot_tag)::value;
-        if constexpr (S < MB) rd1(f, TSVGP_IC(2 + S), ks_tag, boff);
+        if constexpr (DIAG) {
+            constexpr int blk = S == 0 ? 7 - W : S == 1 ? W : (S - 2 < W ? S - 2 : S - 1);
+            rd1(f, TSVGP_IC(2 + blk), ks_tag, boff);
+        } else if constexpr (S < MB) rd1(f, TSVGP_IC(2 + S), ks_tag, boff);
         else rd1(f, TSVGP_IC(S - MB), ks_tag, boff);
     };
+    auto weigh = [&](auto& f, auto ks_tag) TSVGP_AI {
+        constexpr int KW = decltype(ks_tag)::value;
+        if constexpr (!CW && DIAG) {
+            f.v[0] = f.v[2 + W] * w1r[KW];
+            f.v[1] = f.v[2 + 7 - W] * w1r[KW];
+        } else if constexpr (!CW) {
+            f.v[0] *= w1r[KW];
+            f.v[1] *= w1r[KW];
+        }
+    };
     auto keep_set = [&](const Frag& f) TSVGP_AI {
-        cfor<0, NR>([&](auto e) TSVGP_AI {
+        cfor<F0, 2 + MB>([&](auto e) TSVGP_AI {
             const float x = f.v[decltype(e)::value];
             asm volatile("" ::"v"(x));
         });
@@ -2669,7 +2707,8 @@
         } else {
             constexpr int n = (I < 2 * (W + 1)) ? (I >> 1) : (I - (W + 1));
             constexpr int sblk = (I < 2 * (W + 1)) ? (I & 1) : 1;
-            acc[sblk][n] = __builtin_amdgcn_mfma_f32_16x16x4f32(f.v[sblk], f.v[2 + n], acc[sblk][n], 0, 0, 0);
+            constexpr int ea = CW ? 2 + (sblk ? 7 - W : W) : sblk;
+            acc[sblk][n] = __builtin_amdgcn_mfma_f32_16x16x4f32(f.v[ea], f.v[2 + n], acc[sblk][n], 0, 0, 0);
         }
     };
     v2f f1[NKS];
@@ -2692,13 +2731,12 @@
                 constexpr int I = decltype(i)::value;
                 if constexpr (I < NM) mf(cur, i);
                 if constexpr (I < NR) rds(nxt, i, TSVGP_IC(KS_ + 1), B0);
-                else if constexpr (I < NR + XW) read_weight_half(TSVGP_IC(I - NR), TSVGP_IC(1), BUF);
+                else if constexpr (I < NR + XW) read_weight_half(TSVGP_IC(WH0 + I - NR), TSVGP_IC(1), BUF);
                 else if constexpr (I < S)
                     f1[2 * KS_ + I - NR - XW] = *reinterpret_cast<const v2f*>(lds + off1 + B0 + (2 * KS_ + I - NR - XW) * 4 * TILE);
                 TSVGP_SB();
             });
-            nxt.v[0] *= w1r[KS_ + 1];
-            nxt.v[1] *= w1r[KS_ + 1];
+            weigh(nxt, TSVGP_IC(KS_ + 1));
             if constexpr (DIAG && (KS_ == 4 || KS_ == 5)) {
 #pragma unroll
                 for (int q = 4 * (KS_ - 4); q < 4 * (KS_ - 4) + 4; ++q) {
@@ -2719,13 +2757,12 @@
                 constexpr int I = decltype(i)::value;
                 if constexpr (I < NM) mf(fy, i);
                 if constexpr (I < NDMA) dma_piece(TSVGP_IC(DIAG ? 2 * I : I), BUF);
-                else if constexpr (I < NDMA + NWH) read_weight_half(TSVGP_IC(I - NDMA), TSVGP_IC(0), BUF ^ 1);
+                else if constexpr (I < NDMA + NWH) read_weight_half(TSVGP_IC(WH0 + I - NDMA), TSVGP_IC(0), BUF ^ 1);
                 else if constexpr (I < S3) rds(fx, TSVGP_IC(I - NDMA - NWH), TSVGP_IC(0), B1);
                 TSVGP_SB();
             });
             dma_weights(c_fetch, BUF);
-            fx.v[0] *= w1r[0];
-            fx.v[1] *= w1r[0];
+            weigh(fx, TSVGP_IC(0));
             TSVGP_SB();
         } else {
             cfor<0, NM>([&](auto i) TSVGP_AI { mf(fy, i); });
@@ -2744,10 +2781,9 @@
         asm volatile("s_waitcnt vmcnt(0) lgkmcnt(0)" ::: "memory");
         __builtin_amdgcn_s_barrier();
         asm volatile("" ::: "memory");
-        cfor<0, NWH>([&](auto i) TSVGP_AI { read_weight_half(i, TSVGP_IC(0), 0); });
+        cfor<0, NWH>([&](auto i) TSVGP_AI { read_weight_half(TSVGP_IC(WH0 + decltype(i)::value), TSVGP_IC(0), 0); });
         cfor<0, NR>([&](auto i) TSVGP_AI { rds(fx, i, TSVGP_IC(0), 0); });
-        fx.v[0] *= w1r[0];
-        fx.v[1] *= w1r[0];
+        weigh(fx, TSVGP_IC(0));
         int i = 0;
         const int64_t c_last = c_hi - 1;
         auto fetch_of = [&](int idx) TSVGP_AI { const int64_t c = c_lo + idx + 2; return c < c_last ? c : c_last; };
@@ -2792,11 +2828,8 @@
     }
 }
 
-#define TSVGP_S1F_WAVES 2
-__global__ __launch_bounds__(NTHREADS, 1) __attribute__((amdgpu_waves_per_eu(1, TSVGP_S1F_WAVES))) void syrk1f_kernel(SyrkArgs<float> a) {
-    __shared__ __attribute__((aligned(1024))) float lds[2 * S1F_BUF];
-    __shared__ __attribute__((aligned(1024))) float wl[2 * S1F_WL];
-
+template <bool CW>
+__device__ __forceinline__ void syrk1f_main(const SyrkArgs<float>& a, float* lds, float* wl) {
     const int w = __builtin_amdgcn_readfirstlane(threadIdx.x >> 6);
     const int nt = a.nt, n_off = nt * (nt - 1) / 2;
     const int per_p = n_off * a.ns_off + nt * a.ns_diag;
@@ -2818,16 +2851,29 @@
     const int tri = it * (it + 1) / 2 + jt;
     const int slab = (tri - it) * a.ns_off + it * a.ns_diag + sidx;
     if (it != jt) {
-        syrk1f_body<false, 0>(a, lds, wl, p, it, jt, sidx, slab, per_p, w);
+        syrk1f_body<false, 0, CW>(a, lds, wl, p, it, jt, sidx, slab, per_p, w);
     } else if (w == 0) {
-        syrk1f_body<true, 0>(a, lds, wl, p, it, jt, sidx, slab, per_p, w);
+        syrk1f_body<true, 0, CW>(a, lds, wl, p, it, jt, sidx, slab, per_p, w);
     } else if (w == 1) {
-        syrk1f_body<true, 1>(a, lds, wl, p, it, jt, sidx, slab, per_p, w);
+        syrk1f_body<true, 1, CW>(a, lds, wl, p, it, jt, sidx, slab, per_p, w);
     } else if (w == 2) {
-        syrk1f_body<true, 2>(a, lds, wl, p, it, jt, sidx, slab, per_p, w);
+        syrk1f_body<true, 2, CW>(a, lds, wl, p, it, jt, sidx, slab, per_p, w);
     } else {
-        syrk1f_body<true, 3>(a, lds, wl, p, it, jt, sidx, slab, per_p, w);
-    }
+        syrk1f_body<true, 3, CW>(a, lds, wl, p, it, jt, sidx, slab, per_p, w);
+    }
+}
+
+#define TSVGP_S1F_WAVES 2
+__global__ __launch_bounds__(NTHREADS, 1) __attribute__((amdgpu_waves_per_eu(1, TSVGP_S1F_WAVES))) void syrk1f_kernel(SyrkArgs<float> a) {
+    __shared__ __attribute__((aligned(1024))) float lds[2 * S1F_BUF];
+    __shared__ __attribute__((aligned(1024))) float wl[2 * S1F_WL];
+    syrk1f_main<false>(a, lds, wl);
+}
+
+__global__ __launch_bounds__(NTHREADS, 1) __attribute__((amdgpu_waves_per_eu(1, TSVGP_S1F_WAVES))) void syrk1f_kernel_cw(SyrkArgs<float> a) {
+    __shared__ __attribute__((aligned(1024))) float lds[2 * S1F_BUF];
+    __shared__ __attribute__((aligned(1024))) float wl[2 * S1F_WL];
+    syrk1f_main<true>(a, lds, wl);
 }
 
 constexpr int SR_ROWS = 16;
@@ -2835,6 +2881,7 @@
 __global__ __launch_bounds__(NTHREADS) void syrk_reduce_kernel(const T* __restrict__ part2,
                                                                const T* __restrict__ part1,
                                                                double* __restrict__ acc2, double* __restrict__ acc1,
+                                                               const double* __restrict__ scale,
                                                                int Mp, int P, int nt, int ns_off, int ns_diag) {
     __shared__ double img[SR_ROWS][TILE + 1];
     constexpr int SUBS = TILE / SR_ROWS;
@@ -2859,6 +2906,11 @@
         for (int sp = 0; sp < ns; ++sp) {
 #pragma unroll
             for (int q = 0; q < RPT; ++q) acc[q] += (double)src[(size_t)sp * (TILE * TILE) + q * (NTHREADS / 128) * TILE];
+        }
+        if (scale) {
+            const double c = scale[p];
+#pragma unroll
+            for (int q = 0; q < RPT; ++q) acc[q] = __builtin_fma(acc[q], c, 0.0);
         }
 #pragma unroll
         for (int q = 0; q < RPT; ++q) {
@@ -4809,12 +4861,15 @@
 }
 
 template <typename T>
-int site_accum(const T* B, int64_t strideB, const T* g0, const T* g1, double* acc2, double* acc1, void* work, int64_t Np,
-               int Mp, int P, int nsplit, void* stream) {
-    if (!B || !g0 || !g1 || !acc2 || !acc1 || !work || Np <= 0 || (Np % TILE) || Mp <= 0 || (Mp % TILE) || P <= 0 ||
+int site_accum(const T* B, int64_t strideB, const T* g0, const T* g1, const double* g1_const, double* acc2, double* acc1,
+               void* work, int64_t Np, int Mp, int P, int nsplit, void* stream) {
+    const bool cw = g1_const != nullptr;
+    if (cw ? (g1 != nullptr || P > 8) : !g1) return TSVGP_EINVAL;
+    if (!B || !g0 || !acc2 || !acc1 || !work || Np <= 0 || (Np % TILE) || Mp <= 0 || (Mp % TILE) || P <= 0 ||
         nsplit <= 0 || strideB < 0 || (strideB != 0 && strideB < Np * (int64_t)Mp))
         return TSVGP_EINVAL;
-    if (((uintptr_t)B | (uintptr_t)g0 | (uintptr_t)g1 | (uintptr_t)work) & 15 || ((strideB * (int64_t)sizeof(T)) & 15))
+    if (((uintptr_t)B | (uintptr_t)g0 | (uintptr_t)g1 | (uintptr_t)work) & 15 || ((strideB * (int64_t)sizeof(T)) & 15) ||
+        ((uintptr_t)g1_const & 7))
         return TSVGP_EINVAL;
     const int nt = Mp / TILE, ntri = nt * (nt + 1) / 2, n_off = ntri - nt;
     const int64_t total_chunks = Np / KC;
@@ -4839,8 +4894,14 @@
     if (sizeof(T) == 8 && P <= 8) {
       if constexpr (sizeof(T) == 8) {
         static DynLdsOptIn optin_s1;
-        if (optin_s1.ensure(reinterpret_cast<const void*>(&syrk1_kernel), 0) != TSVGP_OK) return TSVGP_ELAUNCH;
-        hipLaunchKernelGGL(syrk1_kernel, dim3((unsigned)nwg), dim3(NTHREADS), 0, (hipStream_t)stream, a);
+        static DynLdsOptIn optin_s1c;
+        if (cw) {
+            if (optin_s1c.ensure(reinterpret_cast<const void*>(&syrk1_kernel_cw), 0) != TSVGP_OK) return TSVGP_ELAUNCH;
+            hipLaunchKernelGGL(syrk1_kernel_cw, dim3((unsigned)nwg), dim3(NTHREADS), 0, (hipStream_t)stream, a);
+        } else {
+            if (optin_s1.ensure(reinterpret_cast<const void*>(&syrk1_kernel), 0) != TSVGP_OK) return TSVGP_ELAUNCH;
+            hipLaunchKernelGGL(syrk1_kernel, dim3((unsigned)nwg), dim3(NTHREADS), 0, (hipStream_t)stream, a);
+        }
       }
     } else if (sizeof(T) == 4 && P <= 8) {
       if constexpr (sizeof(T) == 4) {
@@ -4848,15 +4909,21 @@
         a.chunks_off = (total32 + a.ns_off - 1) / a.ns_off;
         a.chunks_diag = (total32 + a.ns_diag - 1) / a.ns_diag;
         static DynLdsOptIn optin_s1f;
-        if (optin_s1f.ensure(reinterpret_cast<const void*>(&syrk1f_kernel), 0) != TSVGP_OK) return TSVGP_ELAUNCH;
-        hipLaunchKernelGGL(syrk1f_kernel, dim3((unsigned)nwg), dim3(NTHREADS), 0, (hipStream_t)stream, a);
+        static DynLdsOptIn optin_s1fc;
+        if (cw) {
+            if (optin_s1fc.ensure(reinterpret_cast<const void*>(&syrk1f_kernel_cw), 0) != TSVGP_OK) return TSVGP_ELAUNCH;
+            hipLaunchKernelGGL(syrk1f_kernel_cw, dim3((unsigned)nwg), dim3(NTHREADS), 0, (hipStream_t)stream, a);
+        } else {
+            if (optin_s1f.ensure(reinterpret_cast<const void*>(&syrk1f_kernel), 0) != TSVGP_OK) return TSVGP_ELAUNCH;
+            hipLaunchKernelGGL(syrk1f_kernel, dim3((unsigned)nwg), dim3(NTHREADS), 0, (hipStream_t)stream, a);
+        }
       }
     } else
         hipLaunchKernelGGL(syrk_kernel<T>, dim3((unsigned)nwg), dim3(NTHREADS), 0, (hipStream_t)stream, a);
     if (launch_status() != TSVGP_OK) return TSVGP_ELAUNCH;
     const int extra = (Mp + NTHREADS - 1) / NTHREADS;
     hipLaunchKernelGGL(syrk_reduce_kernel<T>, dim3((unsigned)(ntri * (TILE / SR_ROWS) + extra), (unsigned)P), dim3(NTHREADS), 0,
-                       (hipStream_t)stream, a.part2, a.part1, acc2, acc1, Mp, P, nt, a.ns_off, a.ns_diag);
+                       (hipStream_t)stream, a.part2, a.part1, acc2, acc1, g1_const, Mp, P, nt, a.ns_off, a.ns_diag);
     return launch_status();
 }
 
@@ -5851,19 +5918,39 @@
 }
 int tsvgp_site_accum_f64(const double* B, const double* g0, const double* g1, double* acc2, double* acc1, void* work,
                          int64_t Np, int Mp, int P, int nsplit, void* stream) {
-    return site_accum<double>(B, 0, g0, g1, acc2, acc1, work, Np, Mp, P, nsplit, stream);
+    return site_accum<double>(B, 0, g0, g1, nullptr, acc2, acc1, work, Np, Mp, P, nsplit, stream);
 }
 int tsvgp_site_accum_batched_f64(const double* B, int64_t strideB, const double* g0, const double* g1, double* acc2,
                                  double* acc1, void* work, int64_t Np, int Mp, int P, int nsplit, void* stream) {
-    return site_accum<double>(B, strideB, g0, g1, acc2, acc1, work, Np, Mp, P, nsplit, stream);
+    return site_accum<double>(B, strideB, g0, g1, nullptr, acc2, acc1, work, Np, Mp, P, nsplit, stream);
 }
 int tsvgp_site_accum_batched_f32(const float* B, int64_t strideB, const float* g0, const float* g1, double* acc2,
                                  double* acc1, void* work, int64_t Np, int Mp, int P, int nsplit, void* stream) {
-    return site_accum<float>(B, strideB, g0, g1, acc2, acc1, work, Np, Mp, P, nsplit, stream);
+    return site_accum<float>(B, strideB, g0, g1, nullptr, acc2, acc1, work, Np, Mp, P, nsplit, stream);
 }
 int tsvgp_site_accum_f32(const float* B, const float* g0, const float* g1, double* acc2, double* acc1, void* work,
                          int64_t Np, int Mp, int P, int nsplit, void* stream) {
-    return site_accum<float>(B, 0, g0, g1, acc2, acc1, work, Np, Mp, P, nsplit, stream);
+    return site_accum<float>(B, 0, g0, g1, nullptr, acc2, acc1, work, Np, Mp, P, nsplit, stream);
+}
+int tsvgp_site_accum_cw_f64(const double* B, const double* g0, const double* g1_const, double* acc2, double* acc1, void* work,
+                            int64_t Np, int Mp, int P, int nsplit, void* stream) {
+    if (!g1_const) return TSVGP_EINVAL;
+    return site_accum<double>(B, 0, g0, nullptr, g1_const, acc2, acc1, work, Np, Mp, P, nsplit, stream);
+}
+int tsvgp_site_accum_cw_f32(const float* B, const float* g0, const double* g1_const, double* acc2, double* acc1, void* work,
+                            int64_t Np, int Mp, int P, int nsplit, void* stream) {
+    if (!g1_const) return TSVGP_EINVAL;
+    return site_accum<float>(B, 0, g0, nullptr, g1_const, acc2, acc1, work, Np, Mp, P, nsplit, stream);
+}
+int tsvgp_site_accum_cw_batched_f64(const double* B, int64_t strideB, const double* g0, const double* g1_const, double* acc2,
+                                    double* acc1, void* work, int64_t Np, int Mp, int P, int nsplit, void* stream) {
+    if (!g1_const) return TSVGP_EINVAL;
+    return site_accum<double>(B, strideB, g0, nullptr, g1_const, acc2, acc1, work, Np, Mp, P, nsplit, stream);
+}
+int tsvgp_site_accum_cw_batched_f32(const float* B, int64_t strideB, const float* g0, const double* g1_const, double* acc2,
+                                    double* acc1, void* work, int64_t Np, int Mp, int P, int nsplit, void* stream) {
+    if (!g1_const) return TSVGP_EINVAL;
+    return site_accum<float>(B, strideB, g0, nullptr, g1_const, acc2, acc1, work, Np, Mp, P, nsplit, stream);
 }
 
 int tsvgp_potrf_f64(double* A, int M, int lda, int batch, int64_t stride, int* info, double* work, int flags,
diff --git a/t-svgp_amd/estep.py b/t-svgp_amd/estep.py
--- a/t-svgp_amd/estep.py
+++ b/t-svgp_amd/estep.py
@@ -2,6 +2,7 @@
 
 import contextlib
 import ctypes
+import math
 import os
 from dataclasses import dataclass
 from typing import Optional
@@ -92,6 +93,15 @@
     return best
 
 
+def gaussian_g1_const(lik_id, lik_param, dtype=torch.float64):
+    if (lik_id & 0xFF) != B.LIK_GAUSSIAN or not isinstance(lik_param, (int, float)) or not (0.0 < lik_param < math.inf):
+        return None
+    c = -0.5 / float(lik_param)
+    if not (lik_id & B.LIK_NOCROP):
+        c = min(c, -1e-8)
+    return float(torch.tensor(c, dtype=torch.float64).to(dtype))
+
+
 class EStepEngine:
 
     def __init__(self, compute_dtype=torch.float64, device=None):
@@ -113,6 +123,9 @@
         self.last_trmm_batch = 1
         self.profile = None
         self.profile_only = None
+        self.constant_weight_sites = True
+        self.site_sum_calls = {"general": 0, "constant_weight": 0}
+        self._g1c = None
         self.potrf_flags = B.POTRF_DIAG_V1 if os.environ.get("TSVGP_POTRF_DIAG_V1") == "1" else 0
 
     def _stream(self):
@@ -806,7 +819,7 @@
         return KfuP
 
     def _run_batched(self, X, Y, Z, kernel, whitened, *, moment_Tm, moment_mode, gamma, lik_id, lik_param, whiten_T,
-                     sites, want_moments, want_grads, mean_only, prefill=None, mix=None) -> EStepStats:
+                     sites, want_moments, want_grads, mean_only, prefill=None, mix=None, g1_const=None) -> EStepStats:
         T, dev = self.dtype, self.device
         X = X.to(device=dev, dtype=T).contiguous()
         Z = Z.to(device=dev, dtype=T).contiguous()
@@ -866,7 +879,7 @@
             stats.g0, stats.g1 = g0[:N].to(torch.float64), g1[:N].to(torch.float64)
         self._mixed_stats(stats, lm, N, want_moments, want_grads)
         if sites:
-            stats.acc2, stats.acc1 = self._site_sums(KfuP, g0, g1, P, M)
+            stats.acc2, stats.acc1 = self._site_sums(KfuP, g0, g1, P, M, g1_const=None if mapped else g1_const)
         self.last_batched = True
         return stats
 
@@ -880,6 +893,9 @@
         if mix is not None:
             kw["mean_only"] = False
         mapped = (lik_id & 0xFF) in B.MAPPED_LIKS or mix is not None
+        g1_const = kw.pop("g1_const", None)
+        if not mapped:
+            kw["g1_const"] = g1_const
         if mapped or Y is not None:
             self._check_y(Y, X.shape[0], P, lik_id, kw.get("lik_param"), outputs=None if mix is None else mix.shape[0])
         if X.shape[0] > 0:
@@ -894,7 +910,8 @@
                                          gamma=gamma, lik_id=kw.get("lik_id", B.LIK_NONE), lik_param=kw.get("lik_param", 0.0),
                                          whiten_T=whiten_T, sites=kw.get("sites", False),
                                          want_moments=kw.get("want_moments", False), want_grads=want_grads,
-                                         mean_only=kw.get("mean_only", False), prefill=prefill, mix=mix)
+                                         mean_only=kw.get("mean_only", False), prefill=prefill, mix=mix,
+                                         g1_const=kw.get("g1_const"))
         self.last_batched = False
         if mapped and X.shape[0] > 0:
             return self._run_separate_coupled(X, Y, Z, kernel, moment_Tm=moment_Tm, gamma=gamma, whiten_T=whiten_T,
@@ -992,15 +1009,17 @@
     def run(self, X, Y, Z, kernel, *, moment_Tm, moment_mode, gamma, lik_id=B.LIK_NONE, lik_param=0.0,
             whiten_T=None, whiten_mode=B.TRI_UPPER, project_T=None, sites=False, want_moments=False, want_grads=False,
             b_tag=None, mean_only=False, prefill=None, moments_on_kfu=False, project_mode=B.TRI_LOWER,
-            keep_tile=False, site_grads=None) -> EStepStats:
+            keep_tile=False, site_grads=None, g1_const=None) -> EStepStats:
         if isinstance(kernel, SeparateIndependent):
             return self._run_separate(X, Y, Z, kernel, moment_Tm=moment_Tm, moment_mode=moment_mode, gamma=gamma,
                                       lik_id=lik_id, lik_param=lik_param, whiten_T=whiten_T, whiten_mode=whiten_mode,
                                       project_T=project_T, sites=sites, want_moments=want_moments, want_grads=want_grads,
                                       mean_only=mean_only, moments_on_kfu=moments_on_kfu, project_mode=project_mode,
-                                      prefill=prefill)
+                                      prefill=prefill, g1_const=g1_const)
         if site_grads is not None and lik_id != B.LIK_NONE:
             raise ValueError("site_grads replaces the likelihood: lik_id must be LIK_NONE")
+        if g1_const is not None and (lik_id & 0xFF) != B.LIK_GAUSSIAN:
+            raise ValueError("g1_const: only a homoskedastic Gaussian likelihood has one g1 for every row")
         if mean_only and (lik_id & 0xFF) not in (B.LIK_NONE, B.LIK_GAUSSIAN):
             raise ValueError("mean_only needs a likelihood whose gradients do not depend on the predictive variance")
         T, dev = self.dtype, self.device
@@ -1113,11 +1132,12 @@
             self.trmm(A, self._pad_square(project_T, Mp, "pad_proj"), Aproj, project_mode)
             A = Aproj
         if sites:
-            stats.acc2, stats.acc1 = self._site_sums(A, g0, g1, P, M)
+            stats.acc2, stats.acc1 = self._site_sums(A, g0, g1, P, M, g1_const=None if mapped else g1_const)
         return stats
 
-    def _site_sums(self, A, g0, g1, P, M):
+    def _site_sums(self, A, g0, g1, P, M, g1_const=None):
         dev = self.device
+        cw = g1_const is not None and P <= 8
         Np, Mp = A.shape[-2:]
         nsplit = self.nsplit_override or self.choose_nsplit(Mp, P, Np)
         nsplit = max(1, min(nsplit, Np // site_sum_chunk_rows(self.dtype == torch.float64, P)))
@@ -1125,12 +1145,20 @@
         work = self._get("work", (nbytes,), torch.uint8)
         acc2 = torch.empty((P, Mp, Mp), dtype=torch.float64, device=dev)
         acc1 = torch.empty((P, Mp), dtype=torch.float64, device=dev)
+        name = "tsvgp_site_accum_cw" if cw else "tsvgp_site_accum"
         if A.dim() == 3:
-            fn, operand = self._fn("tsvgp_site_accum_batched"), (A.data_ptr(), Np * Mp)
+            fn, operand = self._fn(name + "_batched"), (A.data_ptr(), Np * Mp)
         else:
-            fn, operand = self._fn("tsvgp_site_accum"), (A.data_ptr(),)
+            fn, operand = self._fn(name), (A.data_ptr(),)
+        if cw:
+            if self._g1c is None or self._g1c[:2] != (float(g1_const), P):
+                self._g1c = (float(g1_const), P, torch.full((P,), float(g1_const), dtype=torch.float64, device=dev))
+            weights = self._g1c[2]
+        else:
+            weights = g1
+        self.site_sum_calls["constant_weight" if cw else "general"] += 1
         with torch.cuda.device(dev):
-            self._launch("tsvgp_site_accum", lambda: fn(*operand, g0.data_ptr(), g1.data_ptr(), acc2.data_ptr(), acc1.data_ptr(),
+            self._launch("tsvgp_site_accum", lambda: fn(*operand, g0.data_ptr(), weights.data_ptr(), acc2.data_ptr(), acc1.data_ptr(),
                                                         work.data_ptr(), Np, Mp, P, nsplit, self._stream()))
         return acc2[:, :M, :M], acc1[:, :M]
 
diff --git a/t-svgp_amd/models/tsvgp.py b/t-svgp_amd/models/tsvgp.py
--- a/t-svgp_amd/models/tsvgp.py
+++ b/t-svgp_amd/models/tsvgp.py
@@ -11,7 +11,7 @@
 from .. import _backend as B
 from .. import distributed as D_
 from ..base import default_device, default_float, default_jitter, to_tensor
-from ..estep import EStepStats, per_latent
+from ..estep import EStepStats, gaussian_g1_const, per_latent
 from ..side_branch import poll_current_stream
 from ..inducing_variables import inducingpoint_wrapper
 from ..kernels import LinearCoregionalization, SeparateIndependent, latent_kernels
@@ -106,6 +106,12 @@
     @abc.abstractmethod
     def get_mean_chol_cov_inducing_posterior(self):
         raise NotImplementedError
+
+    def _site_form(self, lik_id) -> dict:
+        if not getattr(self._get_engine(), "constant_weight_sites", False) or self._lmc() is not None:
+            return {}
+        c = gaussian_g1_const(lik_id, self.likelihood.lik_param, self.compute_dtype)
+        return {} if c is None else {"g1_const": c}
 
     def _lmc(self):
         return self.kernel if isinstance(self.kernel, LinearCoregionalization) else None
@@ -859,7 +865,7 @@
                      lik_id=self.likelihood.lik_id, lik_param=self.likelihood.lik_param,
                      whiten_T=ops["whiten_T"], whiten_mode=ops["whiten_mode"], project_T=ops["project_T"],
                      moments_on_kfu=ops["moments_on_kfu"], project_mode=ops["project_mode"],
-                     sites=True, b_tag=warm_key,
+                     sites=True, b_tag=warm_key, **self._site_form(self.likelihood.lik_id),
                      mean_only=self.skip_unused_variance and self.likelihood.lik_id == B.LIK_GAUSSIAN)
         return st, ops
 
@@ -924,7 +930,7 @@
             whiten_full = None
         st = eng.run(X, Y, self._Z(), self.kernel, moment_Tm=Tm_full, prefill=pre, moment_mode=B.TRI_UPPER, gamma=gamma_full,
                      lik_id=self.likelihood.lik_id, lik_param=self.likelihood.lik_param, whiten_T=whiten_full,
-                     whiten_mode=B.TRI_UPPER, project_T=None, sites=True,
+                     whiten_mode=B.TRI_UPPER, project_T=None, sites=True, **self._site_form(self.likelihood.lik_id),
                      mean_only=self.skip_unused_variance and self.likelihood.lik_id == B.LIK_GAUSSIAN)
         blk = tri + M
         packed = torch.zeros(G * per * blk, dtype=f64, device=dev)
diff --git a/t-svgp_amd/models/tsvgp_white.py b/t-svgp_amd/models/tsvgp_white.py
--- a/t-svgp_amd/models/tsvgp_white.py
+++ b/t-svgp_amd/models/tsvgp_white.py
@@ -134,7 +134,7 @@
         return self._get_engine().run(X, Y, ops["Z"], self.kernel, moment_Tm=ops["moment_Tm"], moment_mode=ops["moment_mode"],
                                       gamma=ops["gamma"], lik_id=lik_id, lik_param=self.likelihood.lik_param,
                                       whiten_T=ops["whiten_T"], whiten_mode=B.TRI_UPPER, sites=sites,
-                                      want_moments=want_moments)
+                                      want_moments=want_moments, **(self._site_form(lik_id) if sites else {}))
 
     def _check(self, ops, nonpos):
         zero = torch.zeros(1, dtype=torch.float64, device=self.device)
```

After: 30.55 E-steps/s, median of 6. 2.1% higher.
